# decisiongraph/duckdb-annsearch

Hardware: AMD Instinct MI355X
Metric: queries/sec @ recall@10>=0.95, 10Mx768 fp32, batch=1024 (higher is better)
Workload: dtype f32 results (fp16-image certified filter + exact fp32 rerank); 1 GPU; FAISS IVFFlat nlist=1024 nprobe=32, 10000000x768 fp32 (low-rank gaussian, intrinsic dim 16, noise 0.02), batch=1024, k=10; global_batch=1024, n=10000000, d=768, k=10, parallelism=shard1

## Files before the change

### duckdb-annsearch_amd/csrc/common.hpp

```cpp
#pragma once
#include <hip/hip_runtime.h>
#include <stdint.h>
#include <stdexcept>
#include <string>
#include <cstdio>

namespace hipann {

constexpr int kPlanCopies = 8;
struct IvfPlanHook {
    const int *list_len;
    int nlist, chunk_rows;
    int *ccnt, *slot_off, *qtot;
    bool done;
};

struct HipError : std::runtime_error {
    using std::runtime_error::runtime_error;
};

#define HIPANN_CHECK(expr)                                                                             \
    do {                                                                                               \
        hipError_t _e = (expr);                                                                        \
        if (_e != hipSuccess) {                                                                        \
            throw ::hipann::HipError(std::string(#expr) + " failed: " + hipGetErrorString(_e) + " (" + \
                                     __FILE__ + ":" + std::to_string(__LINE__) + ")");                 \
        }                                                                                              \
    } while (0)

#define HIPANN_REQUIRE(cond, msg)                                        \
    do {                                                                 \
        if (!(cond)) throw ::hipann::HipError(std::string("hipann: ") + (msg)); \
    } while (0)

__host__ __device__ inline int64_t ceil_div(int64_t a, int64_t b) { return (a + b - 1) / b; }

enum Metric : int { kL2 = 0, kIP = 1 };
enum IvfForm : int {
    kFormDecomposed = 0,
    kFormDirect = 1,
    kFormDecomposedValu = 2,
    kFormSplit3 = 3,
    kFormSplit2 = 4,
    kFormSplit2Exact = 5,
    kFormHalfExact = 6,
    kFormI8Exact = 7
};
constexpr int kRerankK = 16, kRerankMaxK = 12;
constexpr int kIvfSubMaxK = 60;
constexpr int kFlatRerankKIP = 32;
enum FlatForm : int {
    kFlatFp32 = 0,
    kFlatSplit3 = 1,
    kFlatSplit2 = 2,
    kFlatSplit2Exact = 3,
    kFlatBf16Exact = 4,
    kFlatI8Exact = 5
};
constexpr float kSplit2Eps = 0x1p-12f;
__host__ __device__ inline bool ivf_form_split(int f) { return f == kFormSplit3 || f == kFormSplit2; }
__host__ __device__ inline int ivf_form_terms(int f) { return f == kFormSplit3 ? 3 : 2; }

__host__ __device__ inline int ivf_group_narrow(int group) { return group & 0xff; }
__host__ __device__ inline int ivf_group_wide(int group) { return (group >> 8) & 0xff; }
__host__ __device__ inline int ivf_ngroups(int c, int group) {
    if (c <= 0) return 0;
    const int n = ivf_group_narrow(group), w = ivf_group_wide(group);
    const int g = w > 0 && c > n ? w : n;
    return (c + g - 1) / g;
}
__host__ __device__ inline int ivf_group_min(int group) {
    return ivf_group_narrow(group) > 0 ? ivf_group_narrow(group) : ivf_group_wide(group);
}

__device__ __forceinline__ int xcd_remap(int bid, int nblocks) {
    const int q = nblocks >> 3, r = nblocks & 7;
    const int xcd = bid & 7, j = bid >> 3;
    return (xcd < r ? xcd * (q + 1) : r * (q + 1) + (xcd - r) * q) + j;
}

}
```

### duckdb-annsearch_amd/csrc/ivf.cpp

```cpp
#include "../../include/hip_ann.h"
#include "ivf.hpp"

#include <algorithm>
#include <chrono>
#include <cstdio>
#include <cstdlib>
#include <cstring>
#include <exception>
#include <numeric>

using namespace hipann;

namespace {

void set_err(char *buf, int len, const char *msg) {
    if (!buf || len <= 0) return;
    std::strncpy(buf, msg, (size_t)len - 1);
    buf[len - 1] = '\0';
}

template <typename F>
int guard_int(char *eb, int el, F &&f) {
    try {
        return f();
// ... 293 lines not shown
    sh.coarse_d.ensure((size_t)nq * np * sizeof(float), sh.device);
    sh.coarse_i.ensure((size_t)nq * np * sizeof(int64_t), sh.device);
    HIPANN_REQUIRE((int64_t)nq * np < (int64_t)0x7fffffff, "nq * nprobe too large");
    sh.slot_off.ensure(sizeof(int) * ((size_t)nq * np + 1), sh.device);
    if (!sh.ccnt.p || !sh.cursor2.p || sh.plan_nlist != nlist) {
        sh.ccnt.ensure(sizeof(int) * 2 * kPlanCopies * (size_t)nlist, sh.device);
        sh.cursor2.ensure(sizeof(int) * 2 * kPlanCopies * (size_t)nlist, sh.device);
        HIPANN_CHECK(hipMemsetAsync(sh.ccnt.p, 0, sizeof(int) * 2 * kPlanCopies * (size_t)nlist, st));
        HIPANN_CHECK(hipMemsetAsync(sh.cursor2.p, 0, sizeof(int) * 2 * kPlanCopies * (size_t)nlist, st));
        sh.plan_nlist = nlist;
        sh.plan_batch = 0;
    }
    const int par = (int)(sh.plan_batch & 1u);
    const size_t pstride = (size_t)kPlanCopies * nlist;
    int *ccnt_cur = sh.ccnt.get<int>() + par * pstride, *ccnt_next = sh.ccnt.get<int>() + (1 - par) * pstride;
    int *cur_cur = sh.cursor2.get<int>() + par * pstride, *cur_next = sh.cursor2.get<int>() + (1 - par) * pstride;
    sh.qtot.ensure(sizeof(int) * (size_t)nq, sh.device);
    struct CcntReset {
        int *p;
        int nlist;
        hipStream_t st;
        bool armed;
        ~CcntReset() {
            if (armed && std::uncaught_exceptions() > 0)
                (void)hipMemsetAsync(p, 0, sizeof(int) * kPlanCopies * (size_t)nlist, st);
        }
    } ccnt_reset{ccnt_cur, nlist, st, true};
    int req = form_override >= 0 ? form_override : ix.form;
    bool as_half = false, probation = false;
    if (form_override < 0 && req == kFormHalfExact && metric == kL2 && kout <= kRerankMaxK && !bigk && !host_fallback() &&
        ivf_mfma_i8_supported(d, kRerankK) && sh.n > 0 && sh.i8_state >= 0) {
        const int mode = filter_image_mode(ix);
        if (mode == 1) {
            as_half = true;
        } else if (mode == 2 && nq >= kAutoI8MinBatch) {
            if (sh.auto8 == 1 && sh.fb_host.p) {
                const uint64_t w = __atomic_load_n(sh.fb_host.get<uint64_t>(), __ATOMIC_RELAXED);
                if (w != sh.fb_seen) {
                    sh.fb_seen = w;
                    sh.auto8_over = auto8_over_rule((int64_t)(w & 0xffffffffu), np, nlist, sh.live, d) ? sh.auto8_over + 1 : 0;
                    if (sh.auto8_over >= 2) sh.auto8 = -1;
                }
            }
            if (sh.auto8 != 0 && sh.live >= sh.auto8_live + sh.auto8_live / 4 + 1) sh.auto8 = 0;
            as_half = sh.auto8 == 1;
            probation = sh.auto8 == 0;
        }
        if (as_half && !ensure_i8_codes(sh, d, nlist, st)) as_half = false;
        if (as_half) req = kFormI8Exact;
    }
    if (form_override < 0) ix.last_filter_image = 0;
    const bool sub_req = (((req == kFormHalfExact || req == kFormSplit2Exact) && kout > kRerankMaxK) ||
                          req == kFormI8Exact) && kout <= kIvfSubMaxK && !bigk;
    bool half = false, i8 = false;
    if (req == kFormHalfExact) {
        half = (kout <= kRerankMaxK || sub_req) && !bigk && ivf_mfma_h_supported(d, kRerankK) &&
               ensure_half_codes(sh, d, nlist, st);
        req = kFormSplit2Exact;
    } else if (req == kFormI8Exact) {
        i8 = sub_req && ivf_mfma_i8_supported(d, kRerankK) && ensure_i8_codes(sh, d, nlist, st);
        req = kFormSplit2Exact;
    }
    const bool img = half || i8;
    const bool want_exact = req == kFormSplit2Exact;
    if (want_exact) req = kout <= kRerankMaxK || sub_req ? kFormSplit2 : kFormSplit3;
    const int k_user = k;
    const int kscan = want_exact && req == kFormSplit2 ? kRerankK : k;
    int form = req != kFormDirect && !bigk && ivf_dot_supported(xq, d, sh.codes) ? req : kFormDirect;
    if (img) form = kFormSplit2;
    if (!img && ivf_form_split(form) && !ivf_mfma_bf_supported(xq, d, sh.codes, kscan, ivf_form_terms(form)))
        form = kFormDecomposed;
    if (form == kFormDecomposed && !ivf_mfma_supported(xq, d, sh.codes, kscan)) form = kFormDecomposedValu;
    const bool exact = want_exact && form == kFormSplit2;
    const bool sub = exact && sub_req;
    k = kscan;
    const int kslot = sub ? ivf_scan_sublists() * k : k;
    const int kfilt = sub ? (i8 ? 64 : std::min(64, std::max(kout + 4, 2 * kout))) : k;
    if (form_override < 0) {
        ix.last_form = exact ? (i8 ? (as_half ? kFormHalfExact : kFormI8Exact) : half ? kFormHalfExact : kFormSplit2Exact) : form;
        ix.last_filter_image = exact && i8 ? 1 : 0;
        ix.last_kfilt = exact ? kfilt : 0;
        ix.last_sublists = sub ? ivf_scan_sublists() : 0;
    }
    const bool tiled = form == kFormDecomposed || ivf_form_split(form);
    const int group = i8 ? ivf_mfma_i8_group(d) : half ? ivf_mfma_h_group(d) : ivf_group_size(form, d);
    float xmax2 = 0.f;
    const bool cert8 = i8 && metric == kL2;
    float rxmax8 = -1.f;
    if (exact) {
        xmax2 = shard_xmax2(sh, d, st);
        if (i8 && !cert8) rxmax8 = shard_i8_rxmax(sh, st);
        sh.nflag.ensure(sizeof(int), sh.device);
        sh.flagged.ensure(sizeof(int) * (size_t)nq, sh.device);
    }
    unsigned *qbound = nullptr;
    if (tiled) {
        sh.qbound.ensure(sizeof(unsigned) * (size_t)nq, sh.device);
        qbound = sh.qbound.get<unsigned>();
    }
    FlatShard &qsh0 = *sh.quant->shards[0];
    if (half) {
        sh.hsplit.ensure((size_t)ivf_half_qsplit_bytes(nq, d), sh.device);
        sh.hits.ensure(sizeof(float) * (size_t)nq, sh.device);
        sh.hres.ensure(sizeof(float) * 2 * (size_t)nq, sh.device);
        float *qn_out = nullptr;
        if (metric == kL2) {
            qsh0.qn.ensure(sizeof(float) * (size_t)nq, sh.device);
            qn_out = qsh0.qn.get<float>();
        }
        RoctxRange rr("hipann.ivf.prepare");
        launch_ivf_split_queries_h(xq, nq, d, sh.half_es, sh.hsplit.p, sh.hits.get<float>(), sh.hres.get<float>(), qn_out,
                                   st);
        qsh0.qn_given = qn_out ? xq : nullptr;
        qsh0.qn_given_nq = nq;
    } else if (i8) {
        sh.qi8.ensure((size_t)ivf_i8_qimg_bytes(nq, d), sh.device);
        sh.qs8.ensure(sizeof(float) * (size_t)nq, sh.device);
        sh.qres8.ensure(sizeof(float) * (size_t)nq, sh.device);
        sh.qhn2.ensure(sizeof(float) * (size_t)nq, sh.device);
        sh.qhn.ensure(sizeof(float) * (size_t)nq, sh.device);
        float *qn_out = nullptr;
        if (metric == kL2) {
            qsh0.qn.ensure(sizeof(float) * (size_t)nq, sh.device);
            qn_out = qsh0.qn.get<float>();
            launch_row_norms(xq, nq, d, qn_out, st);
        }
        RoctxRange rr("hipann.ivf.prepare");
        launch_ivf_split_queries_i8(xq, nq, d, sh.qi8.p, sh.qs8.get<float>(), sh.qres8.get<float>(),
                                    sh.qhn2.get<float>(), sh.qhn.get<float>(), st);
        qsh0.qn_given = qn_out ? xq : nullptr;
        qsh0.qn_given_nq = nq;
    }
    IvfPlanHook hook{sh.list_len.get<int>(), nlist, ivf_chunk_rows(), ccnt_cur, sh.slot_off.get<int>(),
                     sh.qtot.get<int>(), false};
    FlatShard &qsh = *sh.quant->shards[0];
    static const bool hook_env = [] { const char *e = std::getenv("HIPANN_IVF_SELECT_HOOK"); return !e || std::atoi(e); }();
    if (probes_in) {
        HIPANN_CHECK(hipMemcpyAsync(sh.coarse_i.p, probes_in, sizeof(int64_t) * (size_t)nq * np, hipMemcpyDeviceToDevice,
                                    st));
    } else {
        RoctxRange rr("hipann.ivf.coarse");
        qsh.plan_hook = ivf_plan_query_major() && hook_env ? &hook : nullptr;
        CoarseKeysScope ck(qsh);
        try {
            flat_shard_search(*sh.quant, qsh, nq, xq, np, np, sh.coarse_d.get<float>(), sh.coarse_i.get<int64_t>(), st);
        } catch (...) {
            qsh.plan_hook = nullptr;
            qsh.qn_given = nullptr;
            throw;
        }
    }
    qsh.plan_hook = nullptr;
    qsh.qn_given = nullptr;
    sh.cnt.ensure(sizeof(int) * (nlist + 1), sh.device);
    sh.bucket_off.ensure(sizeof(int) * (nlist + 1), sh.device);
    sh.item_off.ensure(sizeof(int) * (nlist + 1), sh.device);
    sh.bucket.ensure(sizeof(int) * (size_t)nq * np, sh.device);
    HIPANN_REQUIRE((int64_t)nq * np < (int64_t)0x7fffffff, "nq * nprobe too large");
    sh.slot_off.ensure(sizeof(int) * ((size_t)nq * np + 1), sh.device);
    {
    RoctxRange rr("hipann.ivf.plan");
    launch_ivf_plan(sh.coarse_i.get<int64_t>(), nq, np, sh.list_len.get<int>(), nlist, group, sh.cnt.get<int>(),
                    sh.bucket_off.get<int>(), sh.item_off.get<int>(), cur_cur, sh.bucket.get<int>(),
                    sh.slot_off.get<int>(), st, exact ? sh.nflag.get<int>() : nullptr, qbound, ccnt_cur,
                    sh.qtot.get<int>(), hook.done, ccnt_next, cur_next);
    }
    sh.plan_batch++;
    ccnt_reset.armed = false;
    const size_t parts = (size_t)np * nq * sh.max_nch * kslot;
    HIPANN_REQUIRE((int64_t)np * nq * sh.max_nch < (int64_t)0x7fffffff, "too many partial lists");
    sh.part_d.ensure(parts * sizeof(float), sh.device);
    sh.part_i.ensure(parts * sizeof(int), sh.device);
    const int64_t max_items = ivf_max_items(nq, np, nlist, sh.max_nch, sh.n, group);
    const float *qn = nullptr;
    if (form != kFormDirect && metric == kL2) {
        const FlatShard &qs = *sh.quant->shards[0];
        if (probes_in && img) {
            qn = qsh0.qn.get<float>();
        } else if (!probes_in && qs.qn_of == xq && qs.qn_nq == nq) {
            qn = qs.qn.get<float>();
        } else {
            sh.qn.ensure(sizeof(float) * (size_t)nq, sh.device);
            launch_row_norms(xq, nq, d, sh.qn.get<float>(), st);
            qn = sh.qn.get<float>();
        }
    }
    if (tiled && !img) ensure_tiled_codes(sh, d, nlist, st);
    if (img) {
    } else if (ivf_form_split(form)) {
        sh.qsplit.ensure((size_t)ivf_mfma_bf_qsplit_bytes(nq, d, ivf_form_terms(form)), sh.device);
    }
    {
        RoctxRange rr("hipann.ivf.scan");
        ScopedTiming t(ix.timer_main, st);
        if (img) {
            launch_ivf_scan_mfma_h(nq, i8 ? sh.qi8.p : sh.hsplit.p, i8 ? sh.qs8.get<float>() : sh.hits.get<float>(),
                                   i8 ? sh.qres8.get<float>() : sh.hres.get<float>(), cert8 ? sh.qhn2.get<float>() : qn, d,
                                   metric, i8 ? sh.codes_i8.p : sh.codes_h.p, sh.tpass_off.get<int64_t>(), sh.xnorm.get<float>(),
                                   sh.list_off.get<int64_t>(), sh.list_len.get<int>(), sh.cnt.get<int>(), sh.bucket_off.get<int>(),
                                   sh.item_off.get<int>(), sh.bucket.get<int>(), sh.slot_off.get<int>(), nlist, np, k,
                                   max_items, qbound, sh.part_d.get<float>(), sh.part_i.get<int>(), st, sub ? 1 : 0,
                                   i8 ? 1 : 0, i8 ? sh.xs8.get<float>() : nullptr,
                                   cert8 ? sh.xr8.get<float>() : nullptr, cert8 ? sh.qhn.get<float>() : nullptr);
        }
        else if (bigk)
            launch_ivf_scan_bigk(xq, d, metric, sh.codes, sh.list_off.get<int64_t>(), sh.list_len.get<int>(),
                                 sh.coarse_i.get<int64_t>(),
                                 nq * np, np, sh.slot_off.get<int>(), nq * np * std::max(sh.max_nch, 1), k,
                                 sh.part_d.get<float>(), sh.part_i.get<int>(), st);
        else if (ivf_form_split(form))
            launch_ivf_scan_mfma_bf(ivf_form_terms(form), xq, nq, sh.qsplit.p, qn, d, metric, sh.codes_t.get<float>(),
                                    sh.tpass_off.get<int64_t>(), sh.xnorm.get<float>(), sh.list_off.get<int64_t>(),
                                    sh.list_len.get<int>(), sh.cnt.get<int>(), sh.bucket_off.get<int>(), sh.item_off.get<int>(),
                                    sh.bucket.get<int>(), sh.slot_off.get<int>(), nlist, np, k, max_items, qbound,
                                    sh.part_d.get<float>(), sh.part_i.get<int>(), st, sub ? 1 : 0);
        else if (form == kFormDecomposed)
            launch_ivf_scan_mfma(xq, qn, d, metric, sh.codes_t.get<float>(), sh.tpass_off.get<int64_t>(),
                                 sh.xnorm.get<float>(), sh.list_off.get<int64_t>(), sh.list_len.get<int>(),
                                 sh.cnt.get<int>(),
                                 sh.bucket_off.get<int>(), sh.item_off.get<int>(), sh.bucket.get<int>(),
                                 sh.slot_off.get<int>(), nlist, np, k, max_items, qbound, sh.part_d.get<float>(),
                                 sh.part_i.get<int>(), st);
        else
            launch_ivf_scan(xq, qn, d, metric, form, sh.codes, sh.xnorm.get<float>(), sh.list_off.get<int64_t>(),
                            sh.list_len.get<int>(), sh.cnt.get<int>(), sh.bucket_off.get<int>(), sh.item_off.get<int>(), sh.bucket.get<int>(),
                            sh.slot_off.get<int>(), nlist, np, nq, k, max_items, qbound, sh.part_d.get<float>(),
                            sh.part_i.get<int>(), st);
    }
    if (!exact) {
        ScopedTiming t(ix.timer_merge, st);
        launch_ivf_merge(sh.part_d.get<float>(), sh.part_i.get<int>(), sh.ids, sh.n, sh.slot_off.get<int>(), np, nq, k,
                         kout, out_sign, D, I, st);
        return;
    }
    const bool inline_fb = !host_fallback() && !sh.count_only;
    int fb_cap = 0, fb_maxch = 1;
    if (inline_fb) {
        if (!sh.fb_total.p) {
            sh.fb_total.ensure(sizeof(unsigned long long), sh.device);
            HIPANN_CHECK(hipMemsetAsync(sh.fb_total.p, 0, sizeof(unsigned long long), st));
        }
        sh.fpd.ensure(sizeof(float) * (size_t)nq * np * kout, sh.device);
        sh.fpi.ensure(sizeof(long long) * (size_t)nq * np * kout, sh.device);
        fb_maxch = sh.max_nch;
        const size_t per_f = (size_t)np * fb_maxch * kout * (sizeof(float) + sizeof(long long));
        fb_cap = (int)std::min<int64_t>({nq, 64, std::max<int64_t>(1, (int64_t)(((size_t)64 << 20) / per_f))});
        sh.fbc_d.ensure(sizeof(float) * (size_t)fb_cap * np * fb_maxch * kout, sh.device);
        sh.fbc_i.ensure(sizeof(long long) * (size_t)fb_cap * np * fb_maxch * kout, sh.device);
        if (sh.fbc_cap < fb_cap || !sh.fbc_done.p) {
            sh.fbc_done.ensure(sizeof(unsigned) * (size_t)std::max(fb_cap, 64), sh.device);
            HIPANN_CHECK(hipMemsetAsync(sh.fbc_done.p, 0, sh.fbc_done.bytes, st));
            sh.fbc_cap = (int)(sh.fbc_done.bytes / sizeof(unsigned));
        }
    }
    {
        RoctxRange rr("hipann.ivf.rerank");
        ScopedTiming t(ix.timer_merge, st);
        launch_ivf_rerank(sh.part_d.get<float>(), sh.part_i.get<int>(), sh.slot_off.get<int>(), np, nq, kfilt, kout,
                          metric, xq, sh.codes, d, sh.ids, sh.n, 0, xmax2, D, I, sh.nflag.get<int>(),
                          sh.flagged.get<int>(), st, kSplit2Eps, i8 ? rxmax8 : half ? sh.half_rxmax : -1.f,
                          i8 ? sh.qres8.get<float>() : half ? sh.hres.get<float>() : nullptr, sh.coarse_i.get<int64_t>(),
                          sh.list_off.get<int64_t>(), nlist, qbound, img && metric == kL2 ? qn : nullptr, kslot,
                          sub ? 1 : 0, inline_fb ? sh.list_len.get<int>() : nullptr,
                          inline_fb ? sh.fpd.get<float>() : nullptr, inline_fb ? sh.fpi.get<long long>() : nullptr,
                          inline_fb ? sh.fb_total.get<unsigned long long>() : nullptr, fb_cap, cert8 ? 1 : 0);
        if (fb_cap > 0)
            launch_ivf_fallback_chunks(sh.nflag.get<int>(), sh.flagged.get<int>(), fb_cap, np, fb_maxch, ivf_chunk_rows(),
                                       kout, metric, xq, sh.codes, d, sh.ids, 0, sh.coarse_i.get<int64_t>(),
                                       sh.list_off.get<int64_t>(), sh.list_len.get<int>(), nlist, sh.fbc_d.get<float>(),
                                       sh.fbc_i.get<long long>(), sh.fbc_done.get<unsigned>(), D, I,
                                       sh.fb_total.get<unsigned long long>(), st,
                                       as_half && !probation ? auto8_host_word(sh) : nullptr, (unsigned)++sh.fb_seq);
    }
    if (sh.count_only) return;
    if (probation) auto8_probation(ix, sh, nq, xq, k_user, kout, st, probes_in);
    if (inline_fb) return;
    int nf = 0;
    HIPANN_CHECK(hipMemcpyAsync(&nf, sh.nflag.p, sizeof(int), hipMemcpyDeviceToHost, st));
    HIPANN_CHECK(hipStreamSynchronize(st));
    if (nf <= 0) return;
    ix.rerank_fallbacks += nf;
    const size_t pbytes = sizeof(int64_t) * (size_t)nq * np;
    sh.coarse_save.ensure(pbytes, sh.device);
    HIPANN_CHECK(hipMemcpyAsync(sh.coarse_save.p, sh.coarse_i.p, pbytes, hipMemcpyDeviceToDevice, st));
    sh.fq.ensure(sizeof(float) * (size_t)nf * d, sh.device);
    sh.fD.ensure(sizeof(float) * (size_t)nf * kout, sh.device);
    sh.fI.ensure(sizeof(int64_t) * (size_t)nf * kout, sh.device);
    launch_ivf_gather_queries(xq, sh.flagged.get<int>(), nf, d, sh.fq.get<float>(), st);
    {
        TimerPause p0(ix.timer_main), p1(ix.timer_merge);
        ivf_shard_search(ix, sh, nf, sh.fq.get<float>(), k_user, kout, sh.fD.get<float>(), sh.fI.get<int64_t>(), st,
                         kFormSplit3);
    }
    launch_ivf_scatter_results(sh.fD.get<float>(), sh.fI.get<int64_t>(), sh.flagged.get<int>(), nf, kout, D, I, st);
    HIPANN_CHECK(hipMemcpyAsync(sh.coarse_i.p, sh.coarse_save.p, pbytes, hipMemcpyDeviceToDevice, st));
}


static void ivf_relayout(IvfIndex &ix, IvfShard &sh, const std::vector<int64_t> &add) {
    const int nlist = ix.nlist, d = ix.d;
    hipStream_t st = sh.stream;
    std::vector<int64_t> off(nlist + 1, 0);
    for (int l = 0; l < nlist; ++l) {
        const int64_t cap = sh.h_off[l + 1] - sh.h_off[l], need = sh.h_len[l] + add[l];
        const int64_t ncap = std::max(cap, need + std::max<int64_t>(need / 4, 64));
        off[l + 1] = off[l] + ncap;
    }
    const int64_t N = off[nlist];
    std::vector<int64_t> tp_old(nlist + 1, 0), tp(nlist + 1, 0);
    for (int l = 0; l < nlist; ++l) {
        tp_old[l + 1] = tp_old[l] + ceil_div(sh.h_off[l + 1] - sh.h_off[l], 32);
        tp[l + 1] = tp[l] + ceil_div(off[l + 1] - off[l], 32);
    }
    auto take = [](DevBuf &dst, DevBuf &src) {
        std::swap(dst.p, src.p);
        std::swap(dst.bytes, src.bytes);
        std::swap(dst.device, src.device);
    };
    auto move_array = [&](DevBuf &cur, const void *src_base, size_t unit, bool pass, size_t count) {
        auto nb = std::make_unique<DevBuf>();
        nb->ensure(unit * std::max<size_t>(count, 1), sh.device);
        HIPANN_CHECK(hipMemsetAsync(nb->p, 0, nb->bytes, st));
        for (int l = 0; l < nlist; ++l) {
            const int64_t len = sh.h_len[l];
            if (!len) continue;
            const int64_t o0 = pass ? tp_old[l] : sh.h_off[l], o1 = pass ? tp[l] : off[l];
            const int64_t cnt = pass ? ceil_div(len, 32) : len;
            HIPANN_CHECK(hipMemcpyAsync(static_cast<char *>(nb->p) + unit * (size_t)o1,
                                        static_cast<const char *>(src_base) + unit * (size_t)o0, unit * (size_t)cnt,
                                        hipMemcpyDeviceToDevice, st));
        }
        HIPANN_CHECK(hipStreamSynchronize(st));
        take(cur, *nb);
    };
    move_array(sh.codes_buf, sh.codes, sizeof(float) * (size_t)d, false, (size_t)N);
    sh.codes = sh.codes_buf.get<float>();
    move_array(sh.ids_buf, sh.ids, sizeof(int64_t), false, (size_t)N);
    sh.ids = sh.ids_buf.get<int64_t>();
    sh.owns_codes = true;
    if (ix.metric == kL2) {
        if (sh.xnorm.p) {
            move_array(sh.xnorm, sh.xnorm.p, sizeof(float), false, (size_t)N);
        } else {
            sh.xnorm.ensure(sizeof(float) * (size_t)std::max<int64_t>(N, 1), sh.device);
            HIPANN_CHECK(hipMemsetAsync(sh.xnorm.p, 0, sh.xnorm.bytes, st));
        }
    }
    const bool img_h = sh.half_state > 0 && sh.codes_h.p, img_t = sh.codes_t.p != nullptr;
// ... 664 lines not shown
}

int hipann_ivf_last_probes(void *h, int64_t *probes, int64_t cap, char *eb, int el) {
    return guard_int(eb, el, [&]() -> int {
        HIPANN_REQUIRE(h && probes, "null argument");
        auto *ix = static_cast<IndexBase *>(h);
        HIPANN_REQUIRE(ix->kind == Kind::IVF, "not an IVFFlat index");
        auto *vx = static_cast<IvfIndex *>(ix);
        std::lock_guard<std::mutex> lk(vx->mu);
        const int64_t m = vx->last_nq * vx->last_np;
        HIPANN_REQUIRE(cap >= m, "probe buffer too small");
        if (m == 0) return 0;
        IvfShard &sh = *vx->shards[0];
        DeviceGuard g(sh.device);
        HIPANN_CHECK(hipStreamSynchronize(sh.stream));
        HIPANN_CHECK(hipDeviceSynchronize());
        HIPANN_CHECK(hipMemcpy(probes, sh.coarse_i.p, sizeof(int64_t) * (size_t)m, hipMemcpyDeviceToHost));
        return 0;
    });
}

int hipann_ivf_set_nprobe(void *h, int nprobe) {
    if (!h || nprobe < 1) return -1;
    auto *ix = static_cast<IndexBase *>(h);
    if (ix->kind != Kind::IVF) return -1;
    auto *vx = static_cast<IvfIndex *>(ix);
    std::lock_guard<std::mutex> lk(vx->mu);
    vx->nprobe = nprobe;
    return 0;
}

int hipann_ivf_set_form(void *h, int form) {
    if (!h || form < kFormDecomposed || form > kFormI8Exact) return -1;
    auto *ix = static_cast<IndexBase *>(h);
    if (ix->kind != Kind::IVF) return -1;
    auto *vx = static_cast<IvfIndex *>(ix);
    std::lock_guard<std::mutex> lk(vx->mu);
    vx->form = form;
    return 0;
}

int64_t hipann_ivf_rerank_fallbacks(void *h) {
    if (!h) return -1;
    auto *ix = static_cast<IndexBase *>(h);
    if (ix->kind != Kind::IVF) return -1;
    auto *vx = static_cast<IvfIndex *>(ix);
    std::lock_guard<std::mutex> lk(vx->mu);
    int64_t t = vx->rerank_fallbacks;
    for (auto &sh : vx->shards) {
        if (!sh->fb_total.p) continue;
        DeviceGuard g(sh->device);
        unsigned long long v = 0;
        if (hipDeviceSynchronize() != hipSuccess) return -1;
        if (hipMemcpy(&v, sh->fb_total.p, sizeof(v), hipMemcpyDeviceToHost) != hipSuccess) return -1;
        t += (int64_t)v;
    }
    return t;
}

int hipann_ivf_set_filter_image(void *h, int mode) {
    if (!h || mode < 0 || mode > 2) return -1;
    auto *ix = static_cast<IndexBase *>(h);
    if (ix->kind != Kind::IVF) return -1;
    auto *vx = static_cast<IvfIndex *>(ix);
    std::lock_guard<std::mutex> lk(vx->mu);
    vx->filter_image = mode;
    return 0;
}

int hipann_ivf_get_filter_image(void *h) {
    if (!h) return -1;
    auto *ix = static_cast<IndexBase *>(h);
    if (ix->kind != Kind::IVF) return -1;
    return static_cast<IvfIndex *>(ix)->filter_image;
}

int hipann_ivf_last_filter_image(void *h) {
    if (!h) return -1;
    auto *ix = static_cast<IndexBase *>(h);
    if (ix->kind != Kind::IVF) return -1;
    return static_cast<IvfIndex *>(ix)->last_filter_image;
}

int64_t hipann_ivf_i8_passes_tiled(void *h) {
    if (!h) return -1;
    auto *ix = static_cast<IndexBase *>(h);
    if (ix->kind != Kind::IVF) return -1;
    auto *vx = static_cast<IvfIndex *>(ix);
    std::lock_guard<std::mutex> lk(vx->mu);
    int64_t t = 0;
    for (auto &sh : vx->shards) t += sh->i8_tiled;
    return t;
}

int hipann_ivf_get_form(void *h) {
    if (!h) return -1;
    auto *ix = static_cast<IndexBase *>(h);
    if (ix->kind != Kind::IVF) return -1;
    return static_cast<IvfIndex *>(ix)->form;
}

}
```

### duckdb-annsearch_amd/csrc/ivf_kernels.hip

```cpp
#include "common.hpp"
#include "wave_topk.hpp"

#include <algorithm>
#include <cstdlib>
#include <utility>

namespace hipann {

constexpr int IVF_WAVES = 8;
constexpr int IVF_THREADS = 64 * IVF_WAVES;
constexpr int IVF_G = 32;
constexpr int IVF_QW = IVF_G / IVF_WAVES;
constexpr int IVF_TR = 256;
constexpr int IVF_BK = 24;
constexpr int IVF_LD = IVF_BK + 4;
#ifndef HIPANN_IVF_CH
#define HIPANN_IVF_CH 2048
#endif
constexpr int IVF_CH = HIPANN_IVF_CH;

__device__ __forceinline__ int ivf_nch(int len) { return (len + IVF_CH - 1) / IVF_CH; }

__global__ void ivf_count(const int64_t *__restrict__ probes, int64_t npairs, const int *__restrict__ list_len,
                          int nlist, int *__restrict__ cnt) {
    const int64_t i = (int64_t)blockIdx.x * blockDim.x + threadIdx.x;
    if (i >= npairs) return;
    const int64_t l = probes[i];
    if (l < 0 || l >= nlist) return;
    if (list_len[l] <= 0) return;
    atomicAdd(cnt + l, 1);
}

__global__ void __launch_bounds__(1024) ivf_plan(const int *__restrict__ cnt, const int *__restrict__ list_len,
                                                 int nlist, int group, int *__restrict__ bucket_off,
                                                 int *__restrict__ item_off, int *__restrict__ cursor) {
    __shared__ int sb[1024], si[1024];
    __shared__ int carry_b, carry_i;
    if (threadIdx.x == 0) { carry_b = 0; carry_i = 0; }
    __syncthreads();
    for (int base = 0; base < nlist; base += 1024) {
        const int l = base + threadIdx.x;
        const int c = l < nlist ? cnt[l] : 0;
        const int items = l < nlist ? ivf_ngroups(c, group) * ivf_nch(list_len[l]) : 0;
        sb[threadIdx.x] = c;
        si[threadIdx.x] = items;
        __syncthreads();
        for (int o = 1; o < 1024; o <<= 1) {
            int vb = 0, vi = 0;
            if ((int)threadIdx.x >= o) { vb = sb[threadIdx.x - o]; vi = si[threadIdx.x - o]; }
            __syncthreads();
            sb[threadIdx.x] += vb;
            si[threadIdx.x] += vi;
            __syncthreads();
        }
        if (l < nlist) {
            bucket_off[l] = carry_b + sb[threadIdx.x] - c;
            item_off[l] = carry_i + si[threadIdx.x] - items;
            cursor[l] = 0;
        }
        __syncthreads();
        if (threadIdx.x == 1023) { carry_b += sb[1023]; carry_i += si[1023]; }
        __syncthreads();
    }
    if (threadIdx.x == 0) { bucket_off[nlist] = carry_b; item_off[nlist] = carry_i; }
}

__global__ void ivf_fill(const int64_t *__restrict__ probes, int64_t npairs, const int *__restrict__ list_len,
                         int nlist, const int *__restrict__ bucket_off, int *__restrict__ cursor,
                         int *__restrict__ bucket) {
    const int64_t i = (int64_t)blockIdx.x * blockDim.x + threadIdx.x;
    if (i >= npairs) return;
    const int64_t l = probes[i];
    if (l < 0 || l >= nlist) return;
    if (list_len[l] <= 0) return;
    const int pos = atomicAdd(cursor + l, 1);
    bucket[bucket_off[l] + pos] = (int)i;
}

__device__ __forceinline__ void slot_scan_block(const int64_t *__restrict__ probes, int64_t npairs,
                                                const int *__restrict__ list_len, int nlist, int *__restrict__ slot_off,
                                                int *wsum) {
    constexpr int J = 16;
    const int lane = threadIdx.x & 63, wave = threadIdx.x >> 6;
    int carry = 0;
    for (int64_t base = 0; base < npairs; base += 16 * 64 * J) {
        const int64_t seg = base + (int64_t)wave * 64 * J;
        int l[J];
#pragma unroll
        for (int j = 0; j < J; ++j) {
            const int64_t i = seg + 64 * j + lane;
            const int64_t pv = i < npairs ? probes[i] : -1;
            l[j] = pv >= 0 && pv < nlist ? (int)pv : -1;
        }
        int v[J];
#pragma unroll
        for (int j = 0; j < J; ++j) v[j] = l[j] >= 0 ? ivf_nch(list_len[l[j]]) : 0;
        int run = 0;
#pragma unroll
        for (int j = 0; j < J; ++j) {
            int x = v[j];
#pragma unroll
            for (int o = 1; o < 64; o <<= 1) {
                const int t = __shfl_up(x, o);
                if (lane >= o) x += t;
            }
            const int tot = __shfl(x, 63);
            v[j] = run + x - v[j];
            run += tot;
        }
        if (lane == 0) wsum[wave] = run;
        __syncthreads();
        int off = carry, total = 0;
        for (int w2 = 0; w2 < 16; ++w2) {
            const int t = wsum[w2];
            off += w2 < wave ? t : 0;
            total += t;
        }
#pragma unroll
        for (int j = 0; j < J; ++j) {
            const int64_t i = seg + 64 * j + lane;
            if (i < npairs) slot_off[i] = off + v[j];
        }
        carry += total;
        __syncthreads();
    }
    if (threadIdx.x == 0) slot_off[npairs] = carry;
}

__global__ void __launch_bounds__(1024) ivf_slot_scan(const int64_t *__restrict__ probes, int64_t npairs,
                                                      const int *__restrict__ list_len, int nlist,
                                                      int *__restrict__ slot_off) {
    __shared__ int wsum[16];
    slot_scan_block(probes, npairs, list_len, nlist, slot_off, wsum);
}

__global__ void __launch_bounds__(256) ivf_count_q(const int64_t *__restrict__ probes, int64_t nq, int nprobe,
                                                   const int *__restrict__ list_len, int nlist, int *__restrict__ ccnt,
                                                   int *__restrict__ slot_off, int *__restrict__ qtot) {
    const int64_t q = (int64_t)blockIdx.x * 4 + (threadIdx.x >> 6);
    if (q >= nq) return;
    const int lane = threadIdx.x & 63;
    int carry = 0;
    for (int p0 = 0; p0 < nprobe; p0 += 64) {
        const int p = p0 + lane;
        const int64_t i = q * nprobe + p;
        const int64_t l = p < nprobe ? probes[i] : -1;
        const bool ok = l >= 0 && l < nlist;
        const int len = ok ? list_len[l] : 0;
        if (len > 0) atomicAdd(ccnt + (int64_t)(q % kPlanCopies) * nlist + l, 1);
        const int v = len > 0 ? ivf_nch(len) : 0;
        int x = v;
#pragma unroll
        for (int o = 1; o < 64; o <<= 1) {
            const int t = __shfl_up(x, o);
            if (lane >= o) x += t;
        }
        if (p < nprobe) slot_off[i] = carry + x - v;
        carry += __shfl(x, 63);
    }
    if (lane == 0) qtot[q] = carry;
}

__global__ void __launch_bounds__(1024) ivf_plan_q(int *__restrict__ ccnt, const int *__restrict__ list_len, int nlist,
                                                   int group, int *__restrict__ cnt, int *__restrict__ bucket_off,
                                                   int *__restrict__ item_off, int *__restrict__ cursor,
                                                   int *__restrict__ qtot, int64_t nq, int64_t npairs,
                                                   int *__restrict__ slot_off, int *__restrict__ nflag_reset,
                                                   unsigned *__restrict__ qbound) {
    __shared__ int sb[1024], si[1024];
    __shared__ int carry_b, carry_i;
    const int tid = threadIdx.x;
    if (tid == 0) { carry_b = 0; carry_i = 0; }
    if (nflag_reset && tid == 0) *nflag_reset = 0;
    if (qbound)
        for (int64_t q = tid; q < nq; q += 1024) qbound[q] = 0xff800000u;
    __syncthreads();
    for (int base = 0; base < nlist; base += 1024) {
        const int l = base + tid;
        int c = 0;
        if (l < nlist)
            for (int cp = 0; cp < kPlanCopies; ++cp) c += ccnt[(int64_t)cp * nlist + l];
        const int items = l < nlist ? ivf_ngroups(c, group) * ivf_nch(list_len[l]) : 0;
        sb[tid] = c;
        si[tid] = items;
        __syncthreads();
        for (int o = 1; o < 1024; o <<= 1) {
            int vb = 0, vi = 0;
            if (tid >= o) { vb = sb[tid - o]; vi = si[tid - o]; }
            __syncthreads();
            sb[tid] += vb;
            si[tid] += vi;
            __syncthreads();
        }
        if (l < nlist) {
            cnt[l] = c;
            bucket_off[l] = carry_b + sb[tid] - c;
            item_off[l] = carry_i + si[tid] - items;
            int pre = 0;
            for (int cp = 0; cp < kPlanCopies; ++cp) {
                const int64_t e = (int64_t)cp * nlist + l;
                const int n = ccnt[e];
                cursor[e] = pre;
                ccnt[e] = 0;
                pre += n;
            }
        }
        __syncthreads();
        if (tid == 1023) { carry_b += sb[1023]; carry_i += si[1023]; }
        __syncthreads();
    }
    if (tid == 0) { bucket_off[nlist] = carry_b; item_off[nlist] = carry_i; }
    __syncthreads();
    if (tid == 0) carry_b = 0;
    __syncthreads();
    for (int64_t base = 0; base < nq; base += 1024) {
        const int64_t q = base + tid;
        const int t = q < nq ? qtot[q] : 0;
        sb[tid] = t;
        __syncthreads();
        for (int o = 1; o < 1024; o <<= 1) {
            int v = 0;
            if (tid >= o) v = sb[tid - o];
            __syncthreads();
            sb[tid] += v;
            __syncthreads();
        }
        if (q < nq) qtot[q] = carry_b + sb[tid] - t;
        __syncthreads();
        if (tid == 1023) carry_b += sb[1023];
        __syncthreads();
    }
    if (tid == 0) slot_off[npairs] = carry_b;
}

__global__ void __launch_bounds__(256) ivf_fill_q(const int64_t *__restrict__ probes, int64_t nq, int nprobe,
                                                  const int *__restrict__ list_len, int nlist,
                                                  const int *__restrict__ qbase, const int *__restrict__ bucket_off,
                                                  int *__restrict__ cursor, int *__restrict__ bucket,
                                                  int *__restrict__ slot_off) {
    const int64_t q = (int64_t)blockIdx.x * 4 + (threadIdx.x >> 6);
    if (q >= nq) return;
    const int lane = threadIdx.x & 63;
    const int b = qbase[q];
    for (int p = lane; p < nprobe; p += 64) {
        const int64_t i = q * nprobe + p;
        slot_off[i] += b;
        const int64_t l = probes[i];
        if (l < 0 || l >= nlist || list_len[l] <= 0) continue;
        const int pos = atomicAdd(cursor + (int64_t)(q % kPlanCopies) * nlist + l, 1);
        bucket[bucket_off[l] + pos] = (int)i;
    }
}

constexpr int kPlanFillMaxList = 8192;
__device__ __forceinline__ int block_excl_scan256(int v, int *s_w) {
    const int lane = threadIdx.x & 63, wave = threadIdx.x >> 6;
    int x = v;
#pragma unroll
    for (int o = 1; o < 64; o <<= 1) {
        const int t = __shfl_up(x, o);
        if (lane >= o) x += t;
    }
    if (lane == 63) s_w[wave] = x;
    __syncthreads();
    int base = 0;
#pragma unroll
    for (int w = 0; w < 4; ++w) base += w < wave ? s_w[w] : 0;
    __syncthreads();
    return base + x - v;
}
__global__ void __launch_bounds__(256) ivf_planfill_q(const int64_t *__restrict__ probes, int64_t nq, int nprobe,
                                                      const int *__restrict__ list_len, int nlist, int group,
                                                      const int *__restrict__ ccnt, int *__restrict__ ccnt_next,
                                                      int *__restrict__ cursor, int *__restrict__ cursor_next,
                                                      const int *__restrict__ qtot, int *__restrict__ slot_off,
                                                      int64_t npairs, int *__restrict__ cnt, int *__restrict__ bucket_off,
                                                      int *__restrict__ item_off, int *__restrict__ bucket,
                                                      int *__restrict__ nflag_reset, unsigned *__restrict__ qbound) {
    __shared__ int s_boff[kPlanFillMaxList];
    __shared__ int s_w[4], s_qb[4];
    const int tid = threadIdx.x, lane = tid & 63, wave = tid >> 6;
    const int64_t q0 = (int64_t)blockIdx.x * 4;
    const int per = (nlist + 255) / 256;
    int sum = 0, isum = 0;
    for (int j = 0; j < per; ++j) {
        const int l = tid * per + j;
        if (l < nlist) {
            int c = 0;
            for (int cp = 0; cp < kPlanCopies; ++cp) c += ccnt[(int64_t)cp * nlist + l];
            sum += c;
            if (blockIdx.x == 0) isum += ivf_ngroups(c, group) * ivf_nch(list_len[l]);
        }
    }
    int b = block_excl_scan256(sum, s_w);
    int ib = blockIdx.x == 0 ? block_excl_scan256(isum, s_w) : 0;
    for (int j = 0; j < per; ++j) {
        const int l = tid * per + j;
        if (l < nlist) {
            int c = 0;
            for (int cp = 0; cp < kPlanCopies; ++cp) c += ccnt[(int64_t)cp * nlist + l];
            s_boff[l] = b;
            if (blockIdx.x == 0) {
                cnt[l] = c;
                bucket_off[l] = b;
                item_off[l] = ib;
                ib += ivf_ngroups(c, group) * ivf_nch(list_len[l]);
            }
            b += c;
        }
    }
    if (blockIdx.x == 0 && tid == 255) {
        bucket_off[nlist] = b;
        item_off[nlist] = ib;
    }
    for (int64_t l = (int64_t)blockIdx.x * 256 + tid; l < (int64_t)kPlanCopies * nlist; l += (int64_t)gridDim.x * 256) {
        ccnt_next[l] = 0;
        cursor_next[l] = 0;
    }
    int qs = 0;
    for (int64_t q = tid; q < q0; q += 256) qs += qtot[q];
    const int qb0 = block_excl_scan256(qs, s_w) + qs;
    if (tid == 255) s_qb[0] = qb0;
    __syncthreads();
    if (tid == 0) {
        int acc = s_qb[0];
        for (int i = 0; i < 4; ++i) {
            s_qb[i] = acc;
            acc += q0 + i < nq ? qtot[q0 + i] : 0;
        }
        if (q0 + 4 >= nq) slot_off[npairs] = acc;
        if (blockIdx.x == 0 && nflag_reset) *nflag_reset = 0;
    }
    __syncthreads();
    const int64_t q = q0 + wave;
    if (q >= nq) return;
    if (qbound && lane == 0) qbound[q] = 0xff800000u;
    const int base = s_qb[wave];
    for (int p = lane; p < nprobe; p += 64) {
        const int64_t i = q * nprobe + p;
        slot_off[i] += base;
        const int64_t l = probes[i];
        if (l < 0 || l >= nlist || list_len[l] <= 0) continue;
        const int cp = (int)(q % kPlanCopies);
        int pre = 0;
        for (int c2 = 0; c2 < cp; ++c2) pre += ccnt[(int64_t)c2 * nlist + l];
        const int pos = atomicAdd(cursor + (int64_t)cp * nlist + l, 1);
        bucket[s_boff[l] + pre + pos] = (int)i;
    }
}

constexpr int IVF_F4 = IVF_BK / 4;
constexpr int IVF_SP = IVF_TR * IVF_F4 / IVF_THREADS;

template <bool VEC4>
__device__ __forceinline__ float4 ivf_ld4(const float *__restrict__ src, int kk, int d) {
    float4 v = make_float4(0.f, 0.f, 0.f, 0.f);
    if (VEC4) {
        if (kk < d) v = *reinterpret_cast<const float4 *>(src);
    } else {
        if (kk + 0 < d) v.x = src[0];
        if (kk + 1 < d) v.y = src[1];
        if (kk + 2 < d) v.z = src[2];
        if (kk + 3 < d) v.w = src[3];
    }
    return v;
}

template <bool VEC4>
__device__ __forceinline__ void ivf_stage_load(const float *__restrict__ codes, int64_t r0, int64_t rlast, int d,
                                               int k0, float4 (&st)[IVF_SP]) {
#pragma unroll
    for (int p = 0; p < IVF_SP; ++p) {
        const int f = threadIdx.x + IVF_THREADS * p;
        const int row = f / IVF_F4, c4 = f - (f / IVF_F4) * IVF_F4;
        const int64_t gr = r0 + row < rlast ? r0 + row : rlast;
        const int kk = k0 + 4 * c4;
        st[p] = ivf_ld4<VEC4>(codes + gr * (int64_t)d + kk, kk, d);
    }
}

__device__ __forceinline__ void ivf_stage_store(float *__restrict__ lds, const float4 (&st)[IVF_SP]) {
#pragma unroll
    for (int p = 0; p < IVF_SP; ++p) {
        const int f = threadIdx.x + IVF_THREADS * p;
        const int row = f / IVF_F4, c4 = f - (f / IVF_F4) * IVF_F4;
        *reinterpret_cast<float4 *>(lds + row * IVF_LD + 4 * c4) = st[p];
    }
}

typedef float ivf_f2 __attribute__((ext_vector_type(2)));
typedef float ivf_f4 __attribute__((ext_vector_type(4)));

__device__ __forceinline__ ivf_f2 ivf_pk_sub(ivf_f2 a, ivf_f2 b) {
    ivf_f2 r;
    asm("v_pk_add_f32 %0, %1, %2 neg_lo:[0,1] neg_hi:[0,1]" : "=v"(r) : "v"(a), "v"(b));
    return r;
// ... 522 lines not shown
    float *sk = sm;
    int *si = reinterpret_cast<int *>(sm + IVF_CH);
    float *qv = sm + 2 * IVF_CH;
    const int slot = blockIdx.x;
    if (slot >= slot_off[npairs]) return;
    int64_t lo = 0, hi = npairs - 1;
    while (lo < hi) {
        const int64_t mid = (lo + hi + 1) >> 1;
        if (slot_off[mid] <= slot) lo = mid; else hi = mid - 1;
    }
    const int64_t pair = lo;
    const int chunk = slot - slot_off[pair];
    const int64_t l = probes[pair];
    const int64_t lend = list_off[l] + list_len[l];
    const int64_t r0 = list_off[l] + (int64_t)chunk * IVF_CH;
    const int64_t r1 = r0 + IVF_CH < lend ? r0 + IVF_CH : lend;
    const int len = (int)(r1 - r0);
    const float *q = Q + (pair / nprobe) * (int64_t)d;
    for (int j = threadIdx.x; j < d; j += 256) qv[j] = q[j];
    __syncthreads();
    const int lane = threadIdx.x & 63, wave = threadIdx.x >> 6;
    for (int r = wave; r < IVF_CH; r += 4) {
        float acc = 0.f;
        if (r < len) {
            const float *x = codes + (r0 + r) * (int64_t)d;
            for (int j = lane; j < d; j += 64) {
                if (IP) acc = fmaf(qv[j], x[j], acc);
                else { const float t = qv[j] - x[j]; acc = fmaf(t, t, acc); }
            }
#pragma unroll
            for (int o = 32; o > 0; o >>= 1) acc += __shfl_xor(acc, o);
        }
        if (lane == 0) {
            sk[r] = r < len ? (IP ? -acc : acc) : __builtin_inff();
            si[r] = r < len ? (int)(r0 + r) : 0x7fffffff;
        }
    }
    __syncthreads();
    for (int size = 2; size <= IVF_CH; size <<= 1) {
        for (int stride = size >> 1; stride > 0; stride >>= 1) {
            for (int t = threadIdx.x; t < IVF_CH / 2; t += 256) {
                const int a = 2 * t - (t & (stride - 1)), b = a + stride;
                const bool up = (a & size) == 0;
                const float ka = sk[a], kb = sk[b];
                const int ia = si[a], ib = si[b];
                const bool b_less = kb < ka || (kb == ka && ib < ia);
                if (b_less == up) { sk[a] = kb; sk[b] = ka; si[a] = ib; si[b] = ia; }
            }
            __syncthreads();
        }
    }
    const int64_t off = (int64_t)slot * k;
    for (int e = threadIdx.x; e < k; e += 256) {
        part_d[off + e] = e < IVF_CH ? sk[e] : __builtin_inff();
        part_i[off + e] = e < IVF_CH ? si[e] : 0x7fffffff;
    }
}

void launch_ivf_scan_bigk(const float *Q, int d, int metric, const float *codes, const int64_t *list_off,
                          const int *list_len, const int64_t *probes, int64_t npairs, int nprobe, const int *slot_off, int64_t nslots,
                          int k, float *pd, int *pi, hipStream_t st) {
    if (nslots <= 0) return;
    HIPANN_REQUIRE(nslots < (int64_t)0x7fffffff, "too many slots");
    const size_t smem = (size_t)2 * IVF_CH * 4 + (size_t)d * 4;
    HIPANN_REQUIRE(smem <= 64 * 1024, "dimension too large for the k > 64 IVF path");
    dim3 grid((unsigned)nslots), block(256);
    if (metric == kIP)
        hipLaunchKernelGGL(ivf_scan_slot_bigk<true>, grid, block, smem, st, Q, d, codes, list_off, list_len, probes, npairs,
                           nprobe, slot_off, k, pd, pi);
    else
        hipLaunchKernelGGL(ivf_scan_slot_bigk<false>, grid, block, smem, st, Q, d, codes, list_off, list_len, probes, npairs,
                           nprobe, slot_off, k, pd, pi);
    HIPANN_CHECK(hipGetLastError());
}

bool ivf_plan_query_major() {
    static const bool split = [] { const char *e = std::getenv("HIPANN_IVF_PLAN_SPLIT"); return e && std::atoi(e); }();
    return !split;
}

void launch_ivf_plan(const int64_t *probes, int64_t nq, int nprobe, const int *list_len, int nlist, int group,
                     int *cnt, int *bucket_off, int *item_off, int *cursor, int *bucket, int *slot_off,
                     hipStream_t st, int *nflag_reset, unsigned *qbound, int *ccnt, int *qtot, bool counted,
                     int *ccnt_next, int *cursor_next) {
    const int64_t npairs = nq * nprobe;
    if (ivf_plan_query_major() && ccnt && qtot) {
        const unsigned gq = (unsigned)std::max<int64_t>(1, ceil_div(nq, (int64_t)4));
        if (nq > 0 && !counted)
            hipLaunchKernelGGL(ivf_count_q, dim3(gq), dim3(256), 0, st, probes, nq, nprobe, list_len, nlist, ccnt,
                               slot_off, qtot);
        static const bool fused_env = [] { const char *e = std::getenv("HIPANN_IVF_PLANFILL"); return !e || std::atoi(e); }();
        if (fused_env && ccnt_next && cursor_next && nlist <= kPlanFillMaxList && nq > 0) {
            hipLaunchKernelGGL(ivf_planfill_q, dim3(gq), dim3(256), 0, st, probes, nq, nprobe, list_len, nlist, group,
                               ccnt, ccnt_next, cursor, cursor_next, qtot, slot_off, npairs, cnt, bucket_off, item_off,
                               bucket, nflag_reset, qbound);
            HIPANN_CHECK(hipGetLastError());
            return;
        }
        hipLaunchKernelGGL(ivf_plan_q, dim3(1), dim3(1024), 0, st, ccnt, list_len, nlist, group, cnt, bucket_off,
                           item_off, cursor, qtot, nq, npairs, slot_off, nflag_reset, qbound);
        if (nq > 0)
            hipLaunchKernelGGL(ivf_fill_q, dim3(gq), dim3(256), 0, st, probes, nq, nprobe, list_len, nlist, qtot,
                               bucket_off, cursor, bucket, slot_off);
        if (cursor_next)
            HIPANN_CHECK(hipMemsetAsync(cursor_next, 0, sizeof(int) * kPlanCopies * (size_t)nlist, st));
        HIPANN_CHECK(hipGetLastError());
        return;
    }
    if (nflag_reset) HIPANN_CHECK(hipMemsetAsync(nflag_reset, 0, sizeof(int), st));
    if (qbound) HIPANN_CHECK(hipMemsetD32Async((hipDeviceptr_t)qbound, 0xff800000, (size_t)nq, st));
    HIPANN_CHECK(hipMemsetAsync(cnt, 0, sizeof(int) * (size_t)nlist, st));
    if (npairs > 0)
        hipLaunchKernelGGL(ivf_count, dim3((unsigned)ceil_div(npairs, 256)), dim3(256), 0, st, probes, npairs, list_len,
                           nlist, cnt);
    hipLaunchKernelGGL(ivf_plan, dim3(1), dim3(1024), 0, st, cnt, list_len, nlist, group, bucket_off, item_off,
                       cursor);
    hipLaunchKernelGGL(ivf_slot_scan, dim3(1), dim3(1024), 0, st, probes, npairs, list_len, nlist, slot_off);
    if (npairs > 0)
        hipLaunchKernelGGL(ivf_fill, dim3((unsigned)ceil_div(npairs, 256)), dim3(256), 0, st, probes, npairs, list_len,
                           nlist, bucket_off, cursor, bucket);
    HIPANN_CHECK(hipGetLastError());
}

int64_t ivf_max_items(int64_t nq, int nprobe, int nlist, int max_nch, int64_t nrows, int group) {
    const int64_t npairs = nq * nprobe;
    return ceil_div(npairs, (int64_t)ivf_group_min(group)) * std::max(max_nch, 1) + ceil_div(nrows, IVF_CH) + nlist;
}

int ivf_mfma_group(int d);
int ivf_mfma_bf_group(int d, int np);

int ivf_group_size(int form, int d) {
    if (ivf_form_split(form)) return ivf_mfma_bf_group(d, ivf_form_terms(form));
    return form == kFormDecomposed ? ivf_mfma_group(d) : form == kFormDecomposedValu ? DT_G : IVF_G;
}

int ivf_chunk_rows() { return IVF_CH; }

size_t ivf_scan_smem_bytes() { return (size_t)2 * (IVF_TR + IVF_G) * IVF_LD * sizeof(float); }
static size_t ivf_scan_dot_smem_bytes() { return (size_t)DT_STAGES * DT_STAGE_F4 * 16; }

bool ivf_dot_supported(const float *Q, int d, const float *codes) {
    return (d % 4 == 0) && ((uintptr_t)Q % 16 == 0) && ((uintptr_t)codes % 16 == 0);
}

void launch_ivf_scan(const float *Q, const float *qn, int d, int metric, int form, const float *codes,
                     const float *xn, const int64_t *list_off, const int *list_len, const int *cnt,
                     const int *bucket_off, const int *item_off, const int *bucket, const int *slot_off, int nlist,
                     int nprobe, int64_t nq,
                     int k, int64_t max_items, unsigned *qbound, float *pd, int *pi, hipStream_t st) {
    if (max_items <= 0) return;
    HIPANN_REQUIRE(max_items < (int64_t)0x7fffffff, "too many IVF work items");
    HIPANN_REQUIRE(form != kFormDecomposed, "the MFMA scan is launched with its tiled codes (launch_ivf_scan_mfma)");
    if (form == kFormDecomposedValu) {
        HIPANN_REQUIRE(ivf_dot_supported(Q, d, codes), "decomposed IVF scan needs d % 4 == 0 and 16-B aligned data");
        HIPANN_REQUIRE(metric == kIP || (qn && xn), "decomposed L2 scan needs query and row norms");
        dim3 grid((unsigned)max_items), block(DT_THREADS);
        const size_t smem = ivf_scan_dot_smem_bytes();
#define HIPANN_DOT_ARGS Q, qn, d, codes, xn, list_off, list_len, cnt, bucket_off, item_off, bucket, slot_off, nlist, nprobe, k, pd, pi
        if (metric == kIP) hipLaunchKernelGGL((ivf_scan_dot<true>), grid, block, smem, st, HIPANN_DOT_ARGS);
        else hipLaunchKernelGGL((ivf_scan_dot<false>), grid, block, smem, st, HIPANN_DOT_ARGS);
#undef HIPANN_DOT_ARGS
    } else {
        const bool vec4 = ivf_dot_supported(Q, d, codes);
        dim3 grid((unsigned)max_items), block(IVF_THREADS);
        const size_t smem = ivf_scan_smem_bytes();
#define HIPANN_IVF_ARGS Q, d, codes, list_off, list_len, cnt, bucket_off, item_off, bucket, slot_off, nlist, nprobe, nq, k, pd, pi
        if (vec4) {
            if (metric == kIP) hipLaunchKernelGGL((ivf_scan_topk<true, true>), grid, block, smem, st, HIPANN_IVF_ARGS);
            else hipLaunchKernelGGL((ivf_scan_topk<true, false>), grid, block, smem, st, HIPANN_IVF_ARGS);
        } else {
            if (metric == kIP) hipLaunchKernelGGL((ivf_scan_topk<false, true>), grid, block, smem, st, HIPANN_IVF_ARGS);
            else hipLaunchKernelGGL((ivf_scan_topk<false, false>), grid, block, smem, st, HIPANN_IVF_ARGS);
        }
#undef HIPANN_IVF_ARGS
    }
    HIPANN_CHECK(hipGetLastError());
}

void launch_ivf_merge(const float *pd, const int *pi, const int64_t *ids, int64_t nrows, const int *slot_off, int nprobe, int64_t nq,
                      int k, int kout, float out_sign, float *D, int64_t *I, hipStream_t st) {
    if (nq <= 0) return;
    dim3 grid((unsigned)ceil_div(nq, 4)), block(256);
    const int S = (kout + 63) / 64;
#define HIPANN_IVF_MERGE(s)                                                                                           \
    if (S <= s) {                                                                                                     \
        hipLaunchKernelGGL(ivf_merge_topk<s>, grid, block, 0, st, pd, pi, ids, nrows, slot_off, nprobe, nq, k, kout, \
                           out_sign, D, I);                                                                           \
        HIPANN_CHECK(hipGetLastError());                                                                              \
        return;                                                                                                       \
    }
    HIPANN_IVF_MERGE(1) HIPANN_IVF_MERGE(2) HIPANN_IVF_MERGE(4) HIPANN_IVF_MERGE(8) HIPANN_IVF_MERGE(16)
    HIPANN_IVF_MERGE(32)
#undef HIPANN_IVF_MERGE
    throw HipError("ivf merge: k too large");
}

}

// ... 204 lines not shown
    }
    unsigned T = 0;
    for (int bit = 31; bit >= 0; --bit) {
        const unsigned cand = T | (1u << bit);
        int cnt = 0;
#pragma unroll
        for (int j = 0; j < J; ++j)
            if (j < nj) cnt += __popcll(__ballot(u[j] < cand));
        if (cnt < k) T = cand;
    }
    (void)n_lt_out;
    return T;
}
__device__ __forceinline__ unsigned rws_bits(float f) {
    f = f == 0.f ? 0.f : f;
    const unsigned b = __float_as_uint(f);
    return (b >> 31) ? ~b : (b | 0x80000000u);
}
template <int J>
__device__ __forceinline__ int rws_take(const float *__restrict__ mk, const int *__restrict__ mp, int m, int k, unsigned T,
                                        float *__restrict__ ok, int *__restrict__ op) {
    const int lane = threadIdx.x & 63;
    const unsigned long long lt = (1ull << lane) - 1ull;
    const int nj = (m + 63) >> 6;
    int base = 0;
#pragma unroll
    for (int j = 0; j < J; ++j) {
        const int e = j * 64 + lane;
        const bool a = j < nj && e < m && rws_bits(mk[e]) < T;
        const unsigned long long ma = __ballot(a);
        if (a) { const int p = base + __popcll(ma & lt); ok[p] = mk[e]; op[p] = mp[e]; }
        base += __popcll(ma);
    }
#pragma unroll
    for (int j = 0; j < J; ++j) {
        const int e = j * 64 + lane;
        const bool b = j < nj && e < m && rws_bits(mk[e]) == T;
        const unsigned long long mb = __ballot(b);
        if (b) { const int p = base + __popcll(mb & lt); if (p < k) { ok[p] = mk[e]; op[p] = mp[e]; } }
        base += __popcll(mb);
    }
    return base < k ? base : k;
}
template <int J>
__device__ __forceinline__ int rws_select_narrow(const float *mk, const int *mp, int m, int k, float *tk, int *tp,
                                                 float *ok, int *op) {
    const int lane = threadIdx.x & 63;
    const unsigned long long lt = (1ull << lane) - 1ull;
    const int nj = (m + 63) >> 6;
    unsigned u[J];
    unsigned mn = 0xffffffffu;
#pragma unroll
    for (int j = 0; j < J; ++j) {
        const int e = j * 64 + lane;
        u[j] = j < nj && e < m ? rws_bits(mk[e]) : 0xffffffffu;
        mn = min(mn, u[j]);
    }
    unsigned th = 0;
    for (int bit = 31; bit >= 0; --bit) {
        const unsigned cand = th | (1u << bit);
        if ((int)__popcll(__ballot(mn < cand)) < k) th = cand;
    }
    int c = 0;
#pragma unroll
    for (int j = 0; j < J; ++j) {
        const bool a = u[j] <= th && u[j] != 0xffffffffu;
        const unsigned long long ma = __ballot(a);
        const int p = c + (int)__popcll(ma & lt);
        if (a && p < 64) { tk[p] = mk[j * 64 + lane]; tp[p] = mp[j * 64 + lane]; }
        c += (int)__popcll(ma);
    }
    if (c > 64) return -1;
    __builtin_amdgcn_fence(__ATOMIC_SEQ_CST, "wavefront");
    unsigned dummy = 0;
    const unsigned T = rws_kth_bits<1>(tk, c, k, dummy);
    return rws_take<1>(tk, tp, c, k, T, ok, op);
}

template <int WV, int J>
__device__ __forceinline__ void rerank_wave_select(const float *__restrict__ pd, const int *__restrict__ pi,
                                                   int64_t total, int k, int64_t nrows, float bound,
                                                   float *wk, int *wp, float *sk, int *sp, int *scnt,
                                                   WaveList<1, int> &L, bool &bad, long long &rr_t, int64_t rr_q,
                                                   float *ntk, int *ntp) {
    (void)rr_t;
    (void)rr_q;
    const int lane = threadIdx.x & 63, wv = threadIdx.x >> 6;
    const unsigned long long lt = (1ull << lane) - 1ull;
    float v[J];
    int r[J];
#pragma unroll
    for (int j = 0; j < J; ++j) {
        const int64_t c = ((int64_t)j * WV + wv) * 64 + lane;
        v[j] = c < total ? pd[c] : __builtin_inff();
        r[j] = c < total ? pi[c] : -1;
    }
    RR_MARK(1);
    float *mk = wk + wv * 64 * J;
    int *mp = wp + wv * 64 * J;
    int m = 0;
#pragma unroll
    for (int j = 0; j < J; ++j) {
        const bool a = v[j] <= bound && !(v[j] == __builtin_inff()) && r[j] >= 0 && r[j] < nrows;
        const unsigned long long ma = __ballot(a);
        if (a) { const int p = m + __popcll(ma & lt); mk[p] = v[j]; mp[p] = r[j]; }
        m += __popcll(ma);
    }
    __builtin_amdgcn_fence(__ATOMIC_SEQ_CST, "wavefront");
    if constexpr (HIPANN_RR_STAMP != 0) { if (m >= 0) RR_STAMP_Q(rr_q, 6); }
    int kw;
    if (m <= k) {
        kw = m;
        for (int e = lane; e < m; e += 64) { sk[wv * 64 + e] = mk[e]; sp[wv * 64 + e] = mp[e]; }
    } else if (m <= 64) {
        unsigned dummy = 0;
        const unsigned T = rws_kth_bits<1>(mk, m, k, dummy);
        kw = rws_take<1>(mk, mp, m, k, T, sk + wv * 64, sp + wv * 64);
    } else {
        kw = ntk ? rws_select_narrow<J>(mk, mp, m, k, ntk + wv * 64, ntp + wv * 64, sk + wv * 64, sp + wv * 64) : -1;
        if (kw < 0) {
            unsigned dummy = 0;
            const unsigned T = rws_kth_bits<J>(mk, m, k, dummy);
            kw = rws_take<J>(mk, mp, m, k, T, sk + wv * 64, sp + wv * 64);
        }
    }
    if (lane == 0) scnt[wv] = kw;
    RR_MARK(5);
    RR_STAMP_Q(rr_q, 7);
    __syncthreads();
    if (wv != 0) return;
    int m0 = 0;
#pragma unroll
    for (int w = 0; w < WV; ++w) {
        const int n = scnt[w];
        const bool a = lane < n;
        float kk = a ? sk[w * 64 + lane] : 0.f;
        int pp = a ? sp[w * 64 + lane] : 0;
        if (a) { mk[m0 + lane] = kk; mp[m0 + lane] = pp; }
        m0 += n;
    }
    __builtin_amdgcn_fence(__ATOMIC_SEQ_CST, "wavefront");
    int nsel = m0;
    if (m0 > k && m0 <= 64) {
        unsigned dummy = 0;
        const unsigned T = rws_kth_bits<1>(mk, m0, k, dummy);
        nsel = rws_take<1>(mk, mp, m0, k, T, sk, sp);
        __builtin_amdgcn_fence(__ATOMIC_SEQ_CST, "wavefront");
    } else if (m0 > k) {
        unsigned dummy = 0;
        const unsigned T = rws_kth_bits<WV>(mk, m0, k, dummy);
        nsel = rws_take<WV>(mk, mp, m0, k, T, sk, sp);
        __builtin_amdgcn_fence(__ATOMIC_SEQ_CST, "wavefront");
    } else {
        for (int e = lane; e < m0; e += 64) { sk[e] = mk[e]; sp[e] = mp[e]; }
        __builtin_amdgcn_fence(__ATOMIC_SEQ_CST, "wavefront");
    }
    float kk = lane < nsel ? sk[lane] : __builtin_inff();
    int row = lane < nsel ? sp[lane] : IdTraits<int>::pad();
    wave_rank_sort(kk, row, nsel);
    bad = false;
    L.d[0] = lane < k ? kk : __builtin_inff();
    L.id[0] = lane < k ? row : IdTraits<int>::pad();
    RR_MARK(2);
}

struct ScanCand {
    float key;
    long long pos, label;
};

template <typename Gen>
__device__ __forceinline__ void ivf_scan_order_topk(int64_t n, int kout, Gen gen, WaveList<1, long long> &R) {
    const int lane = threadIdx.x & 63;
    const long long PAD = IdTraits<long long>::pad();
    WaveList<1, long long> A;
    A.init();
    for (int64_t c0 = 0; c0 < n; c0 += 64) {
        const ScanCand x = c0 + lane < n ? gen(c0 + lane) : ScanCand{__builtin_inff(), PAD, PAD};
// ... 201 lines not shown
        asm volatile("s_waitcnt vmcnt(0)" ::: "memory");
        unsigned old = 0;
        if (lane == 0) old = __hip_atomic_fetch_add(done + f, 1u, __ATOMIC_RELAXED, __HIP_MEMORY_SCOPE_AGENT);
        old = (unsigned)__shfl((int)old, 0);
        int64_t need = 0;
        for (int pp = lane; pp < nprobe; pp += 64) {
            int64_t ll, ln;
            plist(q, pp, ll, ln);
            need += (ln + chunk_rows - 1) / chunk_rows;
        }
#pragma unroll
        for (int o = 32; o > 0; o >>= 1) need += __shfl_xor(need, o);
        if ((int64_t)old + 1 != need) continue;
        __builtin_amdgcn_fence(__ATOMIC_ACQUIRE, "agent");
        asm volatile("s_waitcnt vmcnt(0)" ::: "memory");
        const float *pd = cpd + (int64_t)f * per_q * kout;
        const long long *pr = cpi + (int64_t)f * per_q * kout;
        int64_t lenv = 0;
        if (lane < nprobe) {
            int64_t ll;
            plist(q, lane, ll, lenv);
        }
        WaveList<1, long long> R;
        ivf_scan_order_topk(per_q * kout, kout, [&](int64_t cc) {
            const int64_t slot = cc / kout;
            const int pp = (int)(slot / maxch);
            int64_t ll, ln;
            if (nprobe <= 64) ln = __shfl(lenv, pp);
            else plist(q, pp, ll, ln);
            const bool live = (slot % maxch) * (int64_t)chunk_rows < ln;
            const float key = live ? pd[cc] : __builtin_inff();
            const long long row = live ? pr[cc] : PAD;
            const bool ok = !(key == __builtin_inff()) && row != PAD;
            return ScanCand{ok ? key : __builtin_inff(), ok ? ((long long)pp << 32) | row : PAD,
                            ok ? (long long)(ids ? ids[row] : label_offset + row) : PAD};
        }, R);
        const float pad_d = IP ? -__builtin_inff() : __builtin_inff();
        if (lane < kout) {
            const bool pad = R.id[0] == PAD || R.d[0] == __builtin_inff();
            D[q * kout + lane] = pad ? pad_d : (IP ? -R.d[0] : R.d[0]);
            I[q * kout + lane] = pad ? -1 : (int64_t)R.id[0];
        }
        if (lane == 0) {
            __hip_atomic_store(done + f, 0u, __ATOMIC_RELAXED, __HIP_MEMORY_SCOPE_AGENT);
            atomicAdd(total, 1ull);
        }
    }
}

void launch_ivf_fallback_chunks(const int *nflag, const int *flagged, int fb_cap, int nprobe, int maxch, int chunk_rows,
                                int kout, int metric, const float *Q, const float *codes, int d, const int64_t *ids,
                                int64_t label_offset, const int64_t *probes, const int64_t *list_off,
                                const int *list_len, int nlist, float *cpd, long long *cpi, unsigned *done, float *D,
                                int64_t *I, unsigned long long *total, hipStream_t st, unsigned long long *host_word,
                                unsigned host_seq) {
    if (fb_cap <= 0) return;
    HIPANN_REQUIRE(kout >= 1 && kout <= 64 && maxch >= 1 && chunk_rows >= 64, "ivf fallback: arguments out of range");
    dim3 grid(256), block(256);
    if (metric == kIP)
        hipLaunchKernelGGL(ivf_fallback_chunks<true>, grid, block, 0, st, nflag, flagged, fb_cap, nprobe, maxch,
                           chunk_rows, kout, Q, codes, d, ids, label_offset, probes, list_off, list_len, nlist, cpd, cpi,
                           done, D, I, total, host_word, host_seq);
    else
        hipLaunchKernelGGL(ivf_fallback_chunks<false>, grid, block, 0, st, nflag, flagged, fb_cap, nprobe, maxch,
                           chunk_rows, kout, Q, codes, d, ids, label_offset, probes, list_off, list_len, nlist, cpd, cpi,
                           done, D, I, total, host_word, host_seq);
    HIPANN_CHECK(hipGetLastError());
}

#ifndef HIPANN_RR_MINB
#define HIPANN_RR_MINB 4
#endif
template <bool IP, int WV>
__global__ void __launch_bounds__(WV == 1 ? 256 : 64 * WV, WV == 4 ? HIPANN_RR_MINB : 1)
ivf_rerank_topk(const float *__restrict__ pd, const int *__restrict__ pi, const int *__restrict__ slot_off,
                int nprobe, int64_t nq, int k, int kout, const float *__restrict__ Q,
                const float *__restrict__ codes, int d, const int64_t *__restrict__ ids, int64_t nrows,
                int64_t label_offset, float xmax2, float *__restrict__ D, int64_t *__restrict__ I,
                int *__restrict__ nflag, int *__restrict__ flagged, float eps, float rxmax,
                const float *__restrict__ qres, const int64_t *__restrict__ probes,
                const int64_t *__restrict__ list_off, int nlist, const unsigned *__restrict__ qbound,
                const float *__restrict__ qnorm, int kslot, int sub, const int *__restrict__ list_len,
                float *__restrict__ fpd, long long *__restrict__ fpi, unsigned long long *__restrict__ fb_total,
                int fb_cap, int i8_l2) {
    const int64_t q = WV == 1 ? (int64_t)blockIdx.x * 4 + (threadIdx.x >> 6) : (int64_t)blockIdx.x;
    if (q >= nq) return;
    const int lane = threadIdx.x & 63;
    const int wv = WV == 1 ? 0 : (int)(threadIdx.x >> 6);
    RR_STAMP(0);
    long long rr_t = HIPANN_RR_PROF ? clock64() : 0;
    WaveList<1, int> L;
    L.init();
    const int64_t s0 = slot_off ? slot_off[q * nprobe] : q * nprobe;
    const int64_t s1 = slot_off ? slot_off[(q + 1) * nprobe] : (q + 1) * nprobe;
    const int64_t total = (s1 - s0) * kslot;
    if constexpr (HIPANN_RR_STAMP != 0) { if (total >= 0) RR_STAMP(1); }
    pd += s0 * kslot;
    pi += s0 * kslot;
    float tsub = __builtin_inff();
    if (sub && qbound) {
        const unsigned b = qbound[q];
        const float t = __uint_as_float((b & 0x80000000u) ? (b & 0x7fffffffu) : ~b);
        tsub = t == t ? t : __builtin_inff();
    }
    constexpr int RS_J = 16;
    const bool bsel = WV > 1 && total <= (int64_t)64 * WV * RS_J && !rerank_lists();
    if (WV > 1 && !bsel) RR_COUNT(9);
    constexpr int MU = 4;
    for (int64_t cb = (int64_t)wv * 64; !bsel && cb < total; cb += 64 * WV * MU) {
        float vv[MU];
        int rr[MU];
#pragma unroll
        for (int u = 0; u < MU; ++u) {
            const int64_t c = cb + (int64_t)u * 64 * WV + lane;
            vv[u] = c < total ? pd[c] : __builtin_inff();
            rr[u] = c < total ? pi[c] : -1;
        }
#pragma unroll
        for (int u = 0; u < MU; ++u) {
            const bool ok = rr[u] >= 0 && rr[u] < nrows && !(vv[u] == __builtin_inff()) && vv[u] < tsub;
            L.offer(ok ? vv[u] : __builtin_inff(), ok ? rr[u] : IdTraits<int>::pad(), k - 1);
        }
    }
    const float *qp = Q + q * (int64_t)d;
    float mine = __builtin_inff();
    int myrow, ncand;
    float k16;
    bool sel_bad = false;
    const float qn_pre = qres && qnorm ? qnorm[q] : 0.f;
    const float qres_pre = qres ? qres[q] : 0.f;
    if constexpr (WV > 1) {
        __shared__ float sd[WV * 64], sdist[64];
        __shared__ int si[WV * 64], srow[64];
        __shared__ int scnt[2][WV];
        if (bsel) {
            float bound = __builtin_inff();
            if (sub) {
                bound = tsub;
            } else if (qbound) {
                const unsigned qb = qbound[q];
                const float t = __uint_as_float((qb & 0x80000000u) ? (qb & 0x7fffffffu) : ~qb);
                bound = t == t ? t : __builtin_inff();
            }
            RR_MARK(0);
#if HIPANN_RR_OLDSEL
            rerank_block_select<WV, RS_J>(pd, pi, total, k, nrows, sd, si, scnt, L, bound, rr_t);
#else
            __shared__ float wk[WV * 64 * RS_J];
            __shared__ int wp[WV * 64 * RS_J];
            __shared__ float ntk[WV * 64];
            __shared__ int ntp[WV * 64];
            rerank_wave_select<WV, RS_J>(pd, pi, total, k, nrows, bound, wk, wp, sd, si, scnt[0], L, sel_bad, rr_t, q,
                                         ntk, ntp);
#endif
            if (wv == 0) srow[lane] = lane < k ? L.id[0] : IdTraits<int>::pad();
            RR_STAMP(2);
        } else {
            sd[wv * 64 + lane] = lane < k ? L.d[0] : __builtin_inff();
            si[wv * 64 + lane] = lane < k ? L.id[0] : IdTraits<int>::pad();
            __syncthreads();
            if (wv == 0) {
                L.init();
#pragma unroll
                for (int w = 0; w < WV; ++w) L.offer(sd[w * 64 + lane], si[w * 64 + lane], k - 1);
                srow[lane] = lane < k ? L.id[0] : IdTraits<int>::pad();
            }
        }
        __syncthreads();
        for (int r0 = wv * 4; r0 < k; r0 += 4 * WV) {
            float acc[4] = {0.f, 0.f, 0.f, 0.f};
            const float *xr[4];
            bool ok[4];
#pragma unroll
            for (int u = 0; u < 4; ++u) {
                const int r = r0 + u < k ? r0 + u : k - 1;
                const int row = srow[r];
                ok[u] = r0 + u < k && row != IdTraits<int>::pad();
                xr[u] = codes + (int64_t)(ok[u] ? row : 0) * d;
            }
            rerank_rows4<IP>(qp, xr, d, lane, acc);
#pragma unroll
// ... 221 lines not shown
        const float r = qp[e] - (float)(__bf16)qp[e];
        rq2 = fmaf(r, r, rq2);
    }
#pragma unroll
    for (int o = 32; o > 0; o >>= 1) {
        qq += __shfl_xor(qq, o);
        rq2 += __shfl_xor(rq2, o);
    }
    const float qn = sqrtf(qq), rq = qres ? qres[q] : sqrtf(rq2), xh = sqrtf(xmax2) + rxmax;
    const float g = (float)(qres ? 2 * d : d) * 0x1p-24f;
    const float eip = qn * rxmax + rq * xh + g * (qn + rq) * xh;
    const float T = bound[q];
    const float E = 1.01f * ((IP ? 1.f : 2.f) * eip + (float)(d + 8) * 0x1p-24f * 2.f * (qq + xmax2)) +
                    0x1p-20f * (qq + xmax2 + fabsf(T));
    const float dk = readlane_f(L.d[0], kout - 1);
    const bool ok = !over && E <= 3.4e38f && dk < __builtin_inff() && (T == __builtin_inff() || dk < T - E);
    if (dbg && lane == 0) {
        dbg[4 * f + 0] = over ? 1.f : 0.f;
        dbg[4 * f + 1] = dk;
        dbg[4 * f + 2] = T;
        dbg[4 * f + 3] = E;
    }
    if (!ok) {
        if (lane == 0) flagged2[atomicAdd(nflag2, 1)] = (int)q;
        return;
    }
    if (lane < kout) {
        D[q * kout + lane] = IP ? -L.d[0] : L.d[0];
        I[q * kout + lane] = (int64_t)L.id[0];
    }
}

void launch_flat_cand_rerank(const int *flagged, int nf, const float *cand_d, const int *cand_i, const int *cand_n,
                             int nsplit, int cap, const float *bound, const float *Q, const float *X, int d,
                             int64_t nrows, int64_t label_offset, float xmax2, float rxmax, int metric, int kout,
                             float *part_d, long long *part_i, int *ovf, float *D, int64_t *I, int *nflag2,
                             int *flagged2, hipStream_t st, float *dbg, const float *qres) {
    if (nf <= 0) return;
    HIPANN_REQUIRE(kout >= 1 && kout <= 64 && nsplit >= 1 && cap >= 1, "flat cand rerank: bad arguments");
    const int P = std::min(kCandRerankParts, nsplit);
    dim3 g1((unsigned)nf, (unsigned)P);
    if (metric == kIP) {
        hipLaunchKernelGGL(flat_cand_rerank_part<true>, g1, dim3(256), 0, st, flagged, cand_d, cand_i, cand_n, nsplit,
                           cap, Q, X, d, nrows, label_offset, kout, part_d, part_i, ovf);
        hipLaunchKernelGGL(flat_cand_rerank_final<true>, dim3((unsigned)nf), dim3(64), 0, st, flagged, P, bound, Q, d,
                           xmax2, rxmax, kout, part_d, part_i, ovf, D, I, nflag2, flagged2, dbg, qres);
    } else {
        hipLaunchKernelGGL(flat_cand_rerank_part<false>, g1, dim3(256), 0, st, flagged, cand_d, cand_i, cand_n, nsplit,
                           cap, Q, X, d, nrows, label_offset, kout, part_d, part_i, ovf);
        hipLaunchKernelGGL(flat_cand_rerank_final<false>, dim3((unsigned)nf), dim3(64), 0, st, flagged, P, bound, Q, d,
                           xmax2, rxmax, kout, part_d, part_i, ovf, D, I, nflag2, flagged2, dbg, qres);
    }
    HIPANN_CHECK(hipGetLastError());
}

int flat_cand_rerank_parts(int nsplit) { return std::min(kCandRerankParts, nsplit); }

__global__ void __launch_bounds__(256) ivf_max_norm(const float *__restrict__ xn, int64_t n, unsigned *__restrict__ out) {
    float m = 0.f;
    for (int64_t i = (int64_t)blockIdx.x * 256 + threadIdx.x; i < n; i += (int64_t)gridDim.x * 256) m = fmaxf(m, xn[i]);
#pragma unroll
    for (int o = 32; o > 0; o >>= 1) m = fmaxf(m, __shfl_xor(m, o));
    if ((threadIdx.x & 63) == 0) atomicMax(out, __float_as_uint(m));
}

__global__ void __launch_bounds__(256) ivf_gather_queries(const float *__restrict__ Q, const int *__restrict__ idx, int nf,
                                                          int d, float *__restrict__ out) {
    const int64_t t = (int64_t)blockIdx.x * 256 + threadIdx.x;
    if (t >= (int64_t)nf * d) return;
    const int j = (int)(t / d), e = (int)(t - (int64_t)j * d);
    out[t] = Q[(int64_t)idx[j] * d + e];
}

__global__ void __launch_bounds__(256) ivf_scatter_results(const float *__restrict__ Df, const int64_t *__restrict__ If,
                                                           const int *__restrict__ idx, int nf, int kout,
                                                           float *__restrict__ D, int64_t *__restrict__ I) {
    const int64_t t = (int64_t)blockIdx.x * 256 + threadIdx.x;
    if (t >= (int64_t)nf * kout) return;
    const int j = (int)(t / kout), e = (int)(t - (int64_t)j * kout);
    D[(int64_t)idx[j] * kout + e] = Df[t];
    I[(int64_t)idx[j] * kout + e] = If[t];
}

#ifndef HIPANN_RR_WIDE
#define HIPANN_RR_WIDE (1 << 30)
#endif

void launch_ivf_rerank(const float *pd, const int *pi, const int *slot_off, int nprobe, int64_t nq, int k, int kout,
                       int metric, const float *Q, const float *codes, int d, const int64_t *ids, int64_t nrows,
                       int64_t label_offset, float xmax2, float *D, int64_t *I, int *nflag, int *flagged,
                       hipStream_t st, float eps, float rxmax, const float *qres, const int64_t *probes,
                       const int64_t *list_off, int nlist, const unsigned *qbound, const float *qnorm, int kslot,
                       int sub, const int *list_len, float *fpd, long long *fpi, unsigned long long *fb_total,
                       int fb_cap, int i8_l2) {
    if (nq <= 0) return;
    if (kslot <= 0) kslot = k;
    HIPANN_REQUIRE(!i8_l2 || (metric == kL2 && qres && qnorm), "ivf rerank: the int8 L2 certificate needs ‖q − q̂‖ and ‖q‖²");
    HIPANN_REQUIRE(k >= kRerankK && k <= 64 && kout >= 1 && kout <= k && kslot >= 1 && (!sub || qbound),
                   "ivf rerank: k / kout out of range");
    HIPANN_REQUIRE(!fpd || (fpi && list_len && probes && list_off && fb_total), "ivf rerank: inline re-run buffers");
    const bool wide = nq < HIPANN_RR_WIDE;
    dim3 grid((unsigned)(wide ? nq : ceil_div(nq, 4))), block(256);
#define RR_ARGS pd, pi, slot_off, nprobe, nq, k, kout, Q, codes, d, ids, nrows, label_offset, xmax2, D, I, nflag, flagged, \
                eps, rxmax, qres, probes, list_off, nlist, qbound, qnorm, kslot, sub, list_len, fpd, fpi, fb_total, \
                fpd ? fb_cap : 0, i8_l2
    if (metric == kIP) {
        if (wide) hipLaunchKernelGGL((ivf_rerank_topk<true, 4>), grid, block, 0, st, RR_ARGS);
        else hipLaunchKernelGGL((ivf_rerank_topk<true, 1>), grid, block, 0, st, RR_ARGS);
    } else {
        if (wide) hipLaunchKernelGGL((ivf_rerank_topk<false, 4>), grid, block, 0, st, RR_ARGS);
        else hipLaunchKernelGGL((ivf_rerank_topk<false, 1>), grid, block, 0, st, RR_ARGS);
    }
#undef RR_ARGS
    HIPANN_CHECK(hipGetLastError());
}

extern "C" int hipann_debug_rr_stamps(long long *out, int n) {
#if HIPANN_RR_STAMP
    if (n > 4096 * 8 || hipDeviceSynchronize() != hipSuccess) return -1;
    return hipMemcpyFromSymbol(out, HIP_SYMBOL(rr_stamp), sizeof(long long) * (size_t)n) == hipSuccess ? 0 : -1;
#else
    (void)out;
    (void)n;
    return -1;
#endif
}

extern "C" int hipann_debug_rr_prof(unsigned long long *out16) {
#if HIPANN_RR_PROF
    if (hipDeviceSynchronize() != hipSuccess) return -1;
    if (hipMemcpyFromSymbol(out16, HIP_SYMBOL(rr_prof), sizeof(unsigned long long) * 16) != hipSuccess) return -1;
    unsigned long long z[16] = {0};
    if (hipMemcpyToSymbol(HIP_SYMBOL(rr_prof), z, sizeof z) != hipSuccess) return -1;
    return 0;
#else
    (void)out16;
    return -1;
#endif
}

void launch_ivf_max_norm(const float *xn, int64_t n, unsigned *out, hipStream_t st) {
    HIPANN_CHECK(hipMemsetAsync(out, 0, sizeof(unsigned), st));
    if (n <= 0) return;
    const unsigned blocks = (unsigned)std::min<int64_t>(1024, ceil_div(n, 256));
    hipLaunchKernelGGL(ivf_max_norm, dim3(blocks), dim3(256), 0, st, xn, n, out);
    HIPANN_CHECK(hipGetLastError());
}

void launch_ivf_gather_queries(const float *Q, const int *idx, int nf, int d, float *out, hipStream_t st) {
    if (nf <= 0) return;
    hipLaunchKernelGGL(ivf_gather_queries, dim3((unsigned)ceil_div((int64_t)nf * d, 256)), dim3(256), 0, st, Q, idx, nf,
                       d, out);
    HIPANN_CHECK(hipGetLastError());
}

void launch_ivf_scatter_results(const float *Df, const int64_t *If, const int *idx, int nf, int kout, float *D,
                                int64_t *I, hipStream_t st) {
    if (nf <= 0) return;
    hipLaunchKernelGGL(ivf_scatter_results, dim3((unsigned)ceil_div((int64_t)nf * kout, 256)), dim3(256), 0, st, Df, If,
                       idx, nf, kout, D, I);
    HIPANN_CHECK(hipGetLastError());
}

}
```

### duckdb-annsearch_amd/csrc/ivf_mfma.hip

```cpp
#include "common.hpp"
#include "wave_topk.hpp"

#include <algorithm>
#include <cstdio>
#include <cstdlib>
#include <cstring>

namespace hipann {

typedef float mf_f32x4 __attribute__((ext_vector_type(4)));

#ifndef HIPANN_MF_EXPERIMENT
#define HIPANN_MF_EXPERIMENT 0
#endif

#ifndef HIPANN_MF_WAVES
#define HIPANN_MF_WAVES 8
#endif
#ifndef HIPANN_MF_P
#define HIPANN_MF_P 6
#endif
#ifndef HIPANN_MF_QPF
#define HIPANN_MF_QPF 0
#endif
// ... 66 lines not shown
    row_cx<15>(p, m & 8);
    row_cx<4>(p, m & 4);
    row_cx<2>(p, m & 2);
    row_cx<1>(p, m & 1);
}
__device__ __forceinline__ void row_merge16(uint64_t &l, uint64_t c, int m) {
    const uint64_t r = row_xor<15>(c);
    l = r < l ? r : l;
    row_cx<8>(l, m & 8);
    row_cx<4>(l, m & 4);
    row_cx<2>(l, m & 2);
    row_cx<1>(l, m & 1);
}
__device__ __forceinline__ void row_insert1(uint64_t &l, uint64_t c) {
    c &= row_xor<1>(c);
    c &= row_xor<2>(c);
    c &= row_xor<7>(c);
    c &= row_xor<15>(c);
    const unsigned plo = (unsigned)__builtin_amdgcn_update_dpp(0, (int)(unsigned)l, 0x111, 0xF, 0xF, true);
    const unsigned phi = (unsigned)__builtin_amdgcn_update_dpp(0, (int)(unsigned)(l >> 32), 0x111, 0xF, 0xF, true);
    const uint64_t prev = ((uint64_t)phi << 32) | plo;
    l = l <= c ? l : (prev <= c ? c : prev);
}
__device__ __forceinline__ uint64_t row_kth(uint64_t l, int kth, int g) {
    const unsigned lo = (unsigned)l, hi = (unsigned)(l >> 32);
    unsigned rl[4], rh[4];
#pragma unroll
    for (int r = 0; r < 4; ++r) {
        rl[r] = (unsigned)__builtin_amdgcn_readlane((int)lo, 16 * r + kth);
        rh[r] = (unsigned)__builtin_amdgcn_readlane((int)hi, 16 * r + kth);
    }
    const unsigned sl = g == 0 ? rl[0] : g == 1 ? rl[1] : g == 2 ? rl[2] : rl[3];
    const unsigned sh = g == 0 ? rh[0] : g == 1 ? rh[1] : g == 2 ? rh[2] : rh[3];
    return ((uint64_t)sh << 32) | sl;
}

__device__ __forceinline__ unsigned row_kth_key(uint64_t l, int kth, int g) {
    const unsigned hi = (unsigned)(l >> 32);
    unsigned rh[4];
#pragma unroll
    for (int r = 0; r < 4; ++r) rh[r] = (unsigned)__builtin_amdgcn_readlane((int)hi, 16 * r + kth);
    return g == 0 ? rh[0] : g == 1 ? rh[1] : g == 2 ? rh[2] : rh[3];
}

template <int QT>
__device__ __forceinline__ void mf_finish_item(uint64_t (&lst)[QT][4], float *smem, int nqi,
                                               const int *__restrict__ bucket, int boff, int nprobe,
                                               const int *__restrict__ slot_off, int chunk, int k, int sub,
                                               unsigned *__restrict__ qbound, float *__restrict__ part_d,
                                               int *__restrict__ part_i) {
    const int lane = threadIdx.x & 63;
    const int wave = __builtin_amdgcn_readfirstlane(threadIdx.x >> 6);
    const int m = lane & 15, g = lane >> 4;
    if (!sub) {
        uint64_t *scratch = reinterpret_cast<uint64_t *>(smem);
#pragma unroll 1
        for (int half = MF_WAVES / 2; half > 0; half >>= 1) {
            __syncthreads();
            if (wave >= half && wave < 2 * half) {
                uint64_t *dst = scratch + (size_t)(wave - half) * QT * 4 * 64;
#pragma unroll
                for (int qt = 0; qt < QT; ++qt)
#pragma unroll
                    for (int v = 0; v < 4; ++v) dst[(qt * 4 + v) * 64 + lane] = lst[qt][v];
            }
            __syncthreads();
            if (wave < half) {
                const uint64_t *src = scratch + (size_t)wave * QT * 4 * 64;
#pragma unroll
                for (int qt = 0; qt < QT; ++qt)
#pragma unroll
                    for (int v = 0; v < 4; ++v) row_merge16(lst[qt][v], src[(qt * 4 + v) * 64 + lane], m);
            }
        }
    }
    if ((sub || wave == 0) && m < k) {
#pragma unroll
        for (int qt = 0; qt < QT; ++qt)
#pragma unroll
            for (int v = 0; v < 4; ++v) {
                const int q = qt * 16 + 4 * g + v;
                if (q < nqi) {
                    const int pr = bucket[boff + q];
                    const int64_t slot = (int64_t)slot_off[pr] + chunk;
                    const int64_t off = (sub ? slot * MF_WAVES + wave : slot) * k + m;
                    const uint64_t e = lst[qt][v];
                    const unsigned id = (unsigned)e;
                    const bool real = e != MF_EMPTY && id != MF_PAD_ID;
                    part_d[off] = real ? mf_unsortable((unsigned)(e >> 32)) : __builtin_inff();
                    part_i[off] = real ? (int)id : (int)MF_PAD_ID;
                    if (m == k - 1 && real) atomicMin(qbound + pr / nprobe, (unsigned)(e >> 32));
                }
            }
    }
}

template <int QT, bool IP>
__device__ __forceinline__ void mf_item(int d, const float *__restrict__ codes_t, int64_t tp0,
                                        const float *__restrict__ xn,
                                        int64_t r0, int64_t r1, int nqi, const float *__restrict__ qs, int stride,
                                        const float (&qn)[QT][4], const unsigned (&qb)[QT][4],
                                        const int *__restrict__ bucket, int boff, int nprobe,
                                        const int *__restrict__ slot_off, int chunk, int k, int sub, float *smem,
                                        unsigned *__restrict__ qbound, float *__restrict__ part_d,
                                        int *__restrict__ part_i) {
    const int lane = threadIdx.x & 63;
    const int wave = __builtin_amdgcn_readfirstlane(threadIdx.x >> 6);
    const int m = lane & 15, g = lane >> 4;
    const int nsub = mf_nsub(d);
    const int npass_all = (int)ceil_div(r1 - r0, MF_PASS);
    const int npass = npass_all > wave ? (npass_all - wave + MF_WAVES - 1) / MF_WAVES : 0;


    bool qv[QT][4];
#pragma unroll
    for (int qt = 0; qt < QT; ++qt)
#pragma unroll
        for (int v = 0; v < 4; ++v) qv[qt][v] = qt * 16 + 4 * g + v < nqi;

    uint64_t lst[QT][4], thr[QT][4];
#pragma unroll
    for (int qt = 0; qt < QT; ++qt)
#pragma unroll
        for (int v = 0; v < 4; ++v) {
            const uint64_t b = ((uint64_t)qb[qt][v] << 32) | MF_PAD_ID;
            lst[qt][v] = m < k ? b : MF_EMPTY;
            thr[qt][v] = b;
        }

    auto row_of = [&](int i, int r) -> int64_t {
        const int64_t row = r0 + (int64_t)(wave + MF_WAVES * i) * MF_PASS + 16 * r + m;
        return row < r1 ? row : r1 - 1;
    };
    const int ilast = npass > 0 ? npass - 1 : 0;
    const float *rp;
    int ld_i = 0, ld_s = 0;
    auto set_pass = [&](int i) {
        rp = codes_t + ((tp0 + wave + MF_WAVES * i) * nsub) * (MF_RT * 256) + 4 * lane;
    };
    auto next_load = [&](mf_f32x4 (&dst)[MF_RT]) {
        const int s = ld_i <= ilast ? ld_s : nsub - 1;
#pragma unroll
        for (int r = 0; r < MF_RT; ++r)
            dst[r] = *reinterpret_cast<const mf_f32x4 *>(rp + (int64_t)s * (MF_RT * 256) + r * 256);
        if (++ld_s == nsub) {
            ld_s = 0;
            ++ld_i;
            set_pass(ld_i <= ilast ? ld_i : ilast);
        }
    };

    mf_f32x4 ring[MF_P][MF_RT];
    float xnr[MF_RT] = {0.f, 0.f};
    if (npass > 0) {
        set_pass(0);
#pragma unroll
        for (int p = 0; p < MF_P; ++p) next_load(ring[p]);
        if (!IP) {
#pragma unroll
            for (int r = 0; r < MF_RT; ++r) xnr[r] = xn[row_of(0, r)];
        }
    }

    mf_f32x4 acc[QT][MF_RT];
    uint64_t sink = 0;
    mf_f32x4 qnext[QT];
    if (MF_QPF) {
// ... 489 lines not shown
        MB_QN(3)
        mb_item<3, IP, NP, NH>(MB_ARGS);
    }
#undef MB_QN
#undef MB_ARGS
}

template <int NP>
__global__ void __launch_bounds__(256) ivf_split_queries(const float *__restrict__ Q, int64_t nq, int d, int nsup,
                                                         uint4 *__restrict__ out) {
    const int64_t t = (int64_t)blockIdx.x * 256 + threadIdx.x;
    if (t >= nq * nsup * 4) return;
    const int64_t q = t / (nsup * 4);
    const int rr = (int)(t - q * (nsup * 4));
    const int S = rr >> 2, gg = rr & 3;
    const float *src = Q + q * d;
    const int d0 = 32 * S + 4 * gg, d1 = d0 + 16;
    mf_f32x4 a = mf_f32x4{0.f, 0.f, 0.f, 0.f}, b = a;
    if (d0 < d) a = *reinterpret_cast<const mf_f32x4 *>(src + d0);
    if (d1 < d) b = *reinterpret_cast<const mf_f32x4 *>(src + d1);
    const MbTerms<NP> sp = mb_split<NP>(a, b);
#pragma unroll
    for (int j = 0; j < NP; ++j) out[((q * NP + j) * nsup + S) * 4 + gg] = sp.t[j];
}

int ivf_mfma_bf_group(int d, int np) { return mb_group(d, np); }

int64_t ivf_mfma_bf_qsplit_bytes(int64_t nq, int d, int np) { return nq * np * mb_nsuper(d) * 64; }

bool ivf_mfma_bf_supported(const float *Q, int d, const float *codes, int k, int np) {
    return ivf_mfma_supported(Q, d, codes, k) && mb_group(d, np) >= 16;
}

void launch_ivf_scan_mfma_bf(int np, const float *Q, int64_t nq, void *qsplit, const float *qn, int d, int metric,
                             const float *codes_t, const int64_t *tpass_off, const float *xn, const int64_t *list_off,
                             const int *list_len, const int *cnt, const int *bucket_off, const int *item_off, const int *bucket,
                             const int *slot_off, int nlist, int nprobe, int k, int64_t max_items, unsigned *qbound,
                             float *pd, int *pi, hipStream_t st, int sub) {
    if (max_items <= 0 || nq <= 0) return;
    HIPANN_REQUIRE(np == 2 || np == 3, "split-bf16 scan: 2 or 3 terms");
    HIPANN_REQUIRE(max_items < (int64_t)0x7fffffff, "too many IVF work items");
    HIPANN_REQUIRE(qsplit, "split-bf16 scan: no query image buffer");
    HIPANN_REQUIRE(ivf_mfma_bf_supported(Q, d, codes_t, k, np), "split-bf16 IVF scan needs d % 4 == 0, 16-B aligned data, k <= 16");
    HIPANN_REQUIRE(metric == kIP || (qn && xn), "decomposed L2 scan needs query and row norms");
    const int nsup = mb_nsuper(d);
    const int64_t nthr = nq * nsup * 4;
    uint4 *qs = static_cast<uint4 *>(qsplit);
    if (np == 3) hipLaunchKernelGGL(ivf_split_queries<3>, dim3((unsigned)ceil_div(nthr, 256)), dim3(256), 0, st, Q, nq, d, nsup, qs);
    else hipLaunchKernelGGL(ivf_split_queries<2>, dim3((unsigned)ceil_div(nthr, 256)), dim3(256), 0, st, Q, nq, d, nsup, qs);
    const int nh = mb_phases(d, np);
    const int group = mb_group(d, np);
    const size_t merge = (size_t)(MF_WAVES / 2) * MF_QTMAX * 4 * 64 * sizeof(float2);
    const size_t smem = std::max((size_t)group * mb_stride(d, np, nh) * 4, merge);
    dim3 grid((unsigned)max_items), block(MF_THREADS);
#define MB_LAUNCH_ARGS qs, qn, d, codes_t, tpass_off, xn, list_off, list_len, cnt, bucket_off, item_off, bucket, slot_off, nlist, nprobe, \
                       group, k, sub, qbound, pd, pi
#define MB_LAUNCH(NP_, NH_)                                                                                         \
    do {                                                                                                            \
        if (metric == kIP) hipLaunchKernelGGL((ivf_scan_mfma_bf<true, NP_, NH_>), grid, block, smem, st, MB_LAUNCH_ARGS); \
        else hipLaunchKernelGGL((ivf_scan_mfma_bf<false, NP_, NH_>), grid, block, smem, st, MB_LAUNCH_ARGS);       \
    } while (0)
    if (np == 3) {
        if (nh == 2) MB_LAUNCH(3, 2); else MB_LAUNCH(3, 1);
    } else {
        if (nh == 2) MB_LAUNCH(2, 2); else MB_LAUNCH(2, 1);
    }
#undef MB_LAUNCH
#undef MB_LAUNCH_ARGS
    HIPANN_CHECK(hipGetLastError());
}


typedef _Float16 mh_f16x8 __attribute__((ext_vector_type(8)));
#ifndef HIPANN_MH_P
#define HIPANN_MH_P 6
#endif
#ifndef HIPANN_MH_INSERT
#define HIPANN_MH_INSERT 3
#endif
#ifndef HIPANN_MH_STATS
#define HIPANN_MH_STATS 0
#endif
#if HIPANN_MH_STATS
__device__ unsigned long long mh_stats_dev[2][2][5];
#endif
constexpr int MH_P = HIPANN_MH_P;
__host__ __device__ inline int mh_nsup(int d) { return (int)ceil_div(ceil_div(d, 32), MH_P) * MH_P; }
__host__ __device__ inline int mh_stride(int d) { return mh_nsup(d) * 16 + 8; }
inline bool mh_two_term_fits(int d) { return MF_LDS_MAX / ((size_t)(2 * mh_nsup(d) * 16 + 8) * 4) >= 16; }
constexpr int MH_QTW = 6;
inline int mh_group_wide(int d) {
    const int g = (int)(MF_LDS_MAX / ((size_t)mh_stride(d) * 4 + 8)) / 16 * 16;
    return g < 16 * MH_QTW ? g : 16 * MH_QTW;
}
inline int mh_group_packed(int d) { return mh_two_term_fits(d) ? mh_group_wide(d) << 8 : 0; }

__device__ __forceinline__ unsigned short mh_half_bits(float v) {
    const _Float16 h = (_Float16)v;
    return __builtin_fabsf((float)h) < 0x1p-14f ? (unsigned short)0 : __builtin_bit_cast(unsigned short, h);
}
__device__ __forceinline__ float mh_val(unsigned short b) { return (float)__builtin_bit_cast(_Float16, b); }
__device__ __forceinline__ unsigned mh_pack(float a, float b) {
    return (unsigned)mh_half_bits(a) | ((unsigned)mh_half_bits(b) << 16);
}

__device__ __forceinline__ mf_f32x4 mh_mfma(const uint4 &a, const uint4 &b, const mf_f32x4 &c) {
    return __builtin_amdgcn_mfma_f32_16x16x32_f16(__builtin_bit_cast(mh_f16x8, a), __builtin_bit_cast(mh_f16x8, b), c,
                                                  0, 0, 0);
}

typedef int mf_i32x4 __attribute__((ext_vector_type(4)));
__host__ __device__ inline int mi_nsup(int d) { return (int)ceil_div(ceil_div(d, 64), MH_P) * MH_P; }
__device__ __forceinline__ int mi_quant(float x, float s) {
    return s > 0.f ? (int)fminf(fmaxf(rintf(x / s), -127.f), 127.f) : 0;
}
__device__ __forceinline__ uint4 mi_units(const float *x, int dim0, int d, float s) {
    unsigned w[4] = {0u, 0u, 0u, 0u};
#pragma unroll
    for (int i = 0; i < 16; ++i) {
        const int v = dim0 + i < d ? mi_quant(x[dim0 + i], s) : 0;
        w[i >> 2] |= ((unsigned)v & 0xffu) << (8 * (i & 3));
    }
    return make_uint4(w[0], w[1], w[2], w[3]);
}
__device__ __forceinline__ float mi_row_scale(const float *x, int d, int lane) {
    float mx = 0.f;
    for (int e = lane; e < d; e += 64) mx = fmaxf(mx, fabsf(x[e]));
#pragma unroll
    for (int o = 32; o > 0; o >>= 1) mx = fmaxf(mx, __shfl_xor(mx, o));
    return mx > 0.f && mx < 3.0e38f ? mx / 127.f : (mx == 0.f ? 0.f : -1.f);
}

__global__ void __launch_bounds__(256)
ivf_tile_i8(const float *__restrict__ codes, const int64_t *__restrict__ list_off, const int *__restrict__ list_len,
            const int64_t *__restrict__ tpass_off, int nlist, int d, int nsup, uint4 *__restrict__ dst,
            float *__restrict__ xs8, float *__restrict__ xr8, unsigned *__restrict__ nonfin,
            const int64_t *__restrict__ pass_ids) {
    const int64_t pass = pass_ids ? pass_ids[blockIdx.x] : (int64_t)blockIdx.x;
    int lo = 0, hi = nlist - 1;
    while (lo < hi) {
        const int mid = (lo + hi + 1) >> 1;
        if (tpass_off[mid] <= pass) lo = mid; else hi = mid - 1;
    }
    const int l = lo;
    const int64_t r0 = list_off[l] + (pass - tpass_off[l]) * 32, rend = list_off[l] + list_len[l];
    __shared__ float sc[32];
    const int wave = threadIdx.x >> 6, lane = threadIdx.x & 63;
    for (int rr = wave; rr < 32; rr += 4) {
        const int64_t row = r0 + rr;
        float s = 0.f, res = 0.f;
        if (row < rend) {
            const float *x = codes + row * (int64_t)d;
            s = mi_row_scale(x, d, lane);
            if (s < 0.f) {
                s = 0.f;
                res = __builtin_inff();
            } else {
                float r2 = 0.f;
                for (int e = lane; e < d; e += 64) {
                    const float t = x[e] - s * (float)mi_quant(x[e], s);
                    r2 = fmaf(t, t, r2);
                }
#pragma unroll
                for (int o = 32; o > 0; o >>= 1) r2 += __shfl_xor(r2, o);
                res = sqrtf(r2) * 1.0001f;
            }
        }
// ... 444 lines not shown
                    const float sc = I8 ? qiv * xsr[r] : qiv;
                    if (IP) {
                        key = -av * sc;
                    } else {
                        key = fmaf(-2.f * sc, av, qnv + xnr[r]);
                        if constexpr (I8) key = fmaf(-qrv, xrr[r], key);
                        key = key < 0.f ? 0.f : key;
                    }
                    const bool ok = rok && qt * 16 + 4 * g + v < nqi;
                    const unsigned ks = mf_sortable(key);
                    uint64_t cp = ok ? (((uint64_t)ks << 32) | rid) : MF_EMPTY;
                    if (HIPANN_MH_STATS) ++st_step;
                    if (HIPANN_MF_EXPERIMENT == 1) {
                        sink ^= cp;
                    } else if (const uint64_t hit = __ballot(ok && ks <= thr[qt][v])) {
                        int most = 0;
#pragma unroll
                        for (int f = 0; f < 4; ++f) {
                            const int c = __popc((unsigned)(hit >> (16 * f)) & 0xffffu);
                            most = c > most ? c : most;
                        }
                        if (HIPANN_MH_STATS) { ++st_hit; st_rows += __popcll(hit); st_ins += most <= HIPANN_MH_INSERT; }
                        if (most <= HIPANN_MH_INSERT) {
                            uint64_t pend = hit;
                            do {
                                uint64_t first = 0;
#pragma unroll
                                for (int f = 0; f < 4; ++f) {
                                    const unsigned x = (unsigned)(pend >> (16 * f)) & 0xffffu;
                                    first |= (uint64_t)(x & (0u - x)) << (16 * f);
                                }
                                row_insert1(lst[qt][v], (first >> lane) & 1 ? cp : MF_EMPTY);
                                pend &= ~first;
                            } while (HIPANN_MH_INSERT > 1 && pend);
                        } else {
                            row_sort16(cp, m);
                            row_merge16(lst[qt][v], cp, m);
                        }
                        thr[qt][v] = row_kth_key(lst[qt][v], k - 1, g);
                    }
                }
        }
#pragma unroll
        for (int r = 0; r < MF_RT; ++r) {
            xnr[r] = xnr_next[r];
            xsr[r] = xsr_next[r];
            xrr[r] = xrr_next[r];
        }
    }

    if (HIPANN_MF_EXPERIMENT == 1 && sink == 1) part_d[0] = 0.f;
#if HIPANN_MH_STATS
    if (lane == 0) {
        unsigned long long *st = mh_stats_dev[I8][stat_part];
        atomicAdd(st + 0, (unsigned long long)npass);
        atomicAdd(st + 1, (unsigned long long)st_step);
        atomicAdd(st + 2, (unsigned long long)st_hit);
        atomicAdd(st + 3, (unsigned long long)st_rows);
        atomicAdd(st + 4, (unsigned long long)st_ins);
    }
#endif
    mf_finish_item<QT>(lst, smem, nqi, bucket, boff, nprobe, slot_off, chunk, k, sub, qbound, part_d, part_i);
}

template <int TS>
__device__ __forceinline__ void mh_fill(unsigned *qs, const uint4 *__restrict__ qsplit, int nsup, int stride, int nqi,
                                        const int *__restrict__ bucket, int boff, int nprobe) {
    const int per_q = nsup * 4;
    for (int t = threadIdx.x; t < nqi * per_q; t += MF_THREADS) {
        const int q = t / per_q, r2 = t - q * per_q;
        const int gq = bucket[boff + q] / nprobe;
        *reinterpret_cast<uint4 *>(qs + q * stride + r2 * 4) = qsplit[(int64_t)gq * TS * nsup * 4 + r2];
    }
}

template <bool IP, bool I8>
__global__ void __launch_bounds__(MF_THREADS, MF_WAVES / 4)
ivf_scan_mfma_h(const uint4 *__restrict__ qsplit, const float *__restrict__ qnorm, const float *__restrict__ its, int d,
                const uint4 *__restrict__ codes_h, const int64_t *__restrict__ tpass_off, const float *__restrict__ xn,
                const int64_t *__restrict__ list_off, const int *__restrict__ list_len, const int *__restrict__ cnt, const int *__restrict__ bucket_off,
                const int *__restrict__ item_off, const int *__restrict__ bucket, const int *__restrict__ slot_off,
                int nlist, int nprobe, int group, int k, int sub, unsigned *__restrict__ qbound, float *__restrict__ part_d,
                int *__restrict__ part_i, float *__restrict__ qres, int nq, int remap, const float *__restrict__ xs8,
                const float *__restrict__ xr8, const float *__restrict__ qhn) {
    extern __shared__ __attribute__((aligned(16))) float smem[];
    const int total = item_off[nlist];
    if ((int)blockIdx.x >= total) return;
    const int item = remap ? xcd_remap((int)blockIdx.x, total) : (int)blockIdx.x;
    int lo = 0, hi = nlist - 1;
    while (lo < hi) {
        const int mid = (lo + hi + 1) >> 1;
        if (item_off[mid] <= item) lo = mid; else hi = mid - 1;
    }
    const int l = lo;
    const int64_t lr0 = list_off[l], lr1 = lr0 + list_len[l];
    const int c = cnt[l];
    const int ng = ivf_ngroups(c, group);
    const int rem = item - item_off[l];
    const int chunk = rem / ng, grp = rem - chunk * ng;
    const int q_begin = (int)((int64_t)grp * c / ng), q_end = (int)((int64_t)(grp + 1) * c / ng);
    const int nqi = q_end - q_begin;
    const int64_t r0 = lr0 + (int64_t)chunk * MF_CH;
    const int64_t r1 = r0 + MF_CH < lr1 ? r0 + MF_CH : lr1;
    const int boff = bucket_off[l] + q_begin;
    const int nqt = (nqi + 15) >> 4;

    const int64_t tp0 = tpass_off[l] + (int64_t)chunk * (MF_CH / MF_PASS);
    unsigned *qs = reinterpret_cast<unsigned *>(smem);
    const int nsup = I8 ? mi_nsup(d) : mh_nsup(d);
    const int stride = I8 ? mi_nsup(d) * 16 + 8 : mh_stride(d);
    float *qpar = reinterpret_cast<float *>(qs + nqi * stride);
    mh_fill<I8 ? 1 : 2>(qs, qsplit, nsup, stride, nqi, bucket, boff, nprobe);
    for (int t = threadIdx.x; t < nqi; t += MF_THREADS) {
        const int qi = bucket[boff + t] / nprobe;
        if constexpr (I8)
            reinterpret_cast<float4 *>(qpar)[t] =
                make_float4(IP ? 0.f : qnorm[qi], its[qi], IP ? 0.f : 2.f * qhn[qi], 0.f);
        else reinterpret_cast<float2 *>(qpar)[t] = make_float2(IP ? 0.f : qnorm[qi], its[qi]);
        if (!I8) qres[qi] = qres[nq + qi];
    }

    const int lane = threadIdx.x & 63, g = lane >> 4;
    const int stat_part = (int64_t)blockIdx.x * 5 < (int64_t)total ? 0 : 1;
#define MH_CASE(QTV)                                                                                        \
    {                                                                                                       \
        unsigned qb[QTV][4];                                                                                \
        _Pragma("unroll") for (int qt = 0; qt < QTV; ++qt) _Pragma("unroll") for (int v = 0; v < 4; ++v) {  \
            const int q = qt * 16 + 4 * g + v;                                                              \
            const int qi = q < nqi ? bucket[boff + q] / nprobe : 0;                                         \
            qb[qt][v] = q < nqi ? __atomic_load_n(qbound + qi, __ATOMIC_RELAXED) : 0xffffffffu;             \
        }                                                                                                   \
        mh_item<QTV, IP, I8>(d, codes_h, tp0, xn, r0, r1, nqi, qs, stride, qb, qpar, bucket, boff, nprobe, slot_off, \
                             chunk, k, sub, smem, qbound, part_d, part_i, xs8, xr8, stat_part);             \
    }
    switch (nqt) {
    case 0: case 1: MH_CASE(1) break;
    case 2: MH_CASE(2) break;
    case 3: MH_CASE(3) break;
    case 4: MH_CASE(4) break;
    case 5: MH_CASE(5) break;
    default: MH_CASE(6) break;
    }
#undef MH_CASE
}

void ivf_mh_stats_report() {
#if HIPANN_MH_STATS
    unsigned long long h[2][2][5];
    if (hipMemcpyFromSymbol(h, HIP_SYMBOL(mh_stats_dev), sizeof(h)) != hipSuccess) return;
    for (int i8 = 0; i8 < 2; ++i8)
        for (int part = 0; part < 2; ++part)
            std::fprintf(stderr, "HIPANN_MH_STATS image=%s blocks=%s passes=%llu steps=%llu hit_steps=%llu admitted_rows=%llu "
                                 "insert_steps=%llu\n", i8 ? "int8" : "fp16", part ? "rest" : "first_fifth", h[i8][part][0],
                         h[i8][part][1], h[i8][part][2], h[i8][part][3], h[i8][part][4]);
    std::memset(h, 0, sizeof(h));
    (void)hipMemcpyToSymbol(HIP_SYMBOL(mh_stats_dev), h, sizeof(h));
#endif
}

int ivf_mfma_h_group(int d) { return mh_group_packed(d); }
int ivf_scan_sublists() { return MF_WAVES; }
int64_t ivf_half_pass_bytes(int d) { return (int64_t)mh_nsup(d) * MF_RT * 64 * 16; }
int64_t ivf_half_qsplit_bytes(int64_t nq, int d) { return nq * 2 * mh_nsup(d) * 64; }
bool ivf_mfma_h_supported(int d, int k) { return d >= 1 && k >= 1 && k <= MF_KMAX && mh_two_term_fits(d); }
int ivf_mfma_i8_group(int d) {
    const int g = (int)(MF_LDS_MAX / ((size_t)(mi_nsup(d) * 16 + 8) * 4 + 16)) / 16 * 16;
    return (g < 16 * MH_QTW ? g : 16 * MH_QTW) << 8;
}
int64_t ivf_i8_pass_bytes(int d) { return (int64_t)mi_nsup(d) * MF_RT * 64 * 16; }
int64_t ivf_i8_qimg_bytes(int64_t nq, int d) { return nq * mi_nsup(d) * 64; }
bool ivf_mfma_i8_supported(int d, int k) {
    return d >= 1 && k >= 1 && k <= MF_KMAX && ivf_group_wide(ivf_mfma_i8_group(d)) >= 16;
}
void launch_ivf_tile_i8(const float *codes, const int64_t *list_off, const int *list_len, const int64_t *tpass_off,
                        int nlist, int64_t total_pass, int d, void *dst, float *xs8, float *xr8, unsigned *nonfin,
                        hipStream_t st, const int64_t *pass_ids) {
    if (nonfin) HIPANN_CHECK(hipMemsetAsync(nonfin, 0, sizeof(unsigned), st));
    if (total_pass <= 0) return;
    HIPANN_REQUIRE(total_pass < (int64_t)0x7fffffff, "too many passes");
    HIPANN_REQUIRE(xs8 && xr8, "int8 image: missing scale / residual planes");
    hipLaunchKernelGGL(ivf_tile_i8, dim3((unsigned)total_pass), dim3(256), 0, st, codes, list_off, list_len, tpass_off,
                       nlist, d, mi_nsup(d), static_cast<uint4 *>(dst), xs8, xr8, nonfin, pass_ids);
    HIPANN_CHECK(hipGetLastError());
}
void launch_ivf_split_queries_i8(const float *Q, int64_t nq, int d, void *qi8, float *qs8, float *qres8,
                                 float *qhn2, float *qhn, hipStream_t st) {
    if (nq <= 0) return;
    HIPANN_REQUIRE(ceil_div(nq, 4) < (int64_t)0x7fffffff, "too many queries");
    hipLaunchKernelGGL(ivf_split_queries_i8, dim3((unsigned)ceil_div(nq, 4)), dim3(256), 0, st, Q, nq, d, mi_nsup(d),
                       static_cast<uint4 *>(qi8), qs8, qres8, qhn2, qhn);
    HIPANN_CHECK(hipGetLastError());
}

void launch_ivf_max_abs(const float *x, int64_t cnt, unsigned *out, hipStream_t st) {
    HIPANN_CHECK(hipMemsetAsync(out, 0, sizeof(unsigned), st));
    if (cnt <= 0) return;
    const unsigned blocks = (unsigned)std::min<int64_t>(4096, ceil_div(cnt, 256));
    hipLaunchKernelGGL(ivf_max_abs, dim3(blocks), dim3(256), 0, st, x, cnt, out);
    HIPANN_CHECK(hipGetLastError());
}

void launch_ivf_tile_half(const float *codes, const int64_t *list_off, const int *list_len, const int64_t *tpass_off,
                          int nlist, int64_t total_pass, int d, float scale, void *dst, hipStream_t st,
                          const int64_t *pass_ids) {
    if (total_pass <= 0) return;
    HIPANN_REQUIRE(total_pass < (int64_t)0x7fffffff, "too many passes");
    hipLaunchKernelGGL(ivf_tile_half, dim3((unsigned)total_pass), dim3(256), 0, st, codes, list_off, list_len, tpass_off,
                       nlist, d, mh_nsup(d), scale, static_cast<uint4 *>(dst), pass_ids);
    HIPANN_CHECK(hipGetLastError());
}

void launch_ivf_half_residual(const float *codes, int64_t n, int d, float scale, unsigned *out, hipStream_t st) {
    HIPANN_CHECK(hipMemsetAsync(out, 0, sizeof(unsigned), st));
    if (n <= 0) return;
    HIPANN_REQUIRE(ceil_div(n, 4) < (int64_t)0x7fffffff, "too many rows");
    hipLaunchKernelGGL(ivf_half_residual, dim3((unsigned)ceil_div(n, 4)), dim3(256), 0, st, codes, n, d, scale,
                       1.f / scale, out);
    HIPANN_CHECK(hipGetLastError());
}

void launch_ivf_append_rows(const float *rows, const float *norms, const int64_t *dst, const int64_t *ids_in, int64_t n,
                            int d, float *codes, int64_t *ids, float *xnorm, const int *newlen, int *list_len, int nlist,
                            float hscale, unsigned *stat, hipStream_t st) {
    int64_t blocks = std::max(ceil_div(n, (int64_t)4), ceil_div((int64_t)nlist, (int64_t)256));
    if (!dst) blocks = std::min<int64_t>(blocks, 64);
    HIPANN_REQUIRE(blocks < (int64_t)0x7fffffff, "append block too large");
    if (stat) HIPANN_CHECK(hipMemsetAsync(stat, 0, sizeof(unsigned) * 4, st));
    hipLaunchKernelGGL(ivf_append_rows, dim3((unsigned)blocks), dim3(256), 0, st, rows, norms, dst, ids_in, n, d, codes,
                       ids, xnorm, newlen, list_len, nlist, hscale, stat);
    HIPANN_CHECK(hipGetLastError());
}

void launch_ivf_split_queries_h(const float *Q, int64_t nq, int d, int es, void *qsplit, float *its, float *qres,
                                float *qn, hipStream_t st) {
    if (nq <= 0) return;
    const int vec4 = (d % 4 == 0) && ((uintptr_t)Q % 16 == 0);
    hipLaunchKernelGGL(ivf_split_queries_h, dim3((unsigned)ceil_div(nq, 4)), dim3(256), 0, st, Q, nq, d, mh_nsup(d), es,
                       static_cast<uint4 *>(qsplit), its, qres, qn, vec4);
    HIPANN_CHECK(hipGetLastError());
}

void launch_ivf_scan_mfma_h(int64_t nq, const void *qsplit, const float *its, float *qres, const float *qn, int d,
                            int metric, const void *codes_h, const int64_t *tpass_off, const float *xn,
                            const int64_t *list_off, const int *list_len, const int *cnt, const int *bucket_off,
                            const int *item_off, const int *bucket, const int *slot_off, int nlist, int nprobe, int k,
                            int64_t max_items, unsigned *qbound, float *pd, int *pi, hipStream_t st, int sub, int i8mode,
                            const float *xs8, const float *xr8, const float *qhn) {
    if (max_items <= 0 || nq <= 0) return;
    HIPANN_REQUIRE(max_items < (int64_t)0x7fffffff, "too many IVF work items");
    HIPANN_REQUIRE(qsplit && its && qres && codes_h, "fp16 IVF scan: missing buffers");
    HIPANN_REQUIRE(i8mode ? ivf_mfma_i8_supported(d, k) && xs8 : ivf_mfma_h_supported(d, k),
                   "fp16 / int8 IVF scan needs k <= 16 (int8: scales and prepared queries)");
    HIPANN_REQUIRE(metric == kIP || (qn && xn), "decomposed L2 scan needs query and row norms");
    HIPANN_REQUIRE(!i8mode || metric == kIP || (xr8 && qhn), "int8 L2 scan needs the rows' residuals and the queries' norms");
    const uint4 *qs = static_cast<const uint4 *>(qsplit);
    const int group = i8mode ? ivf_mfma_i8_group(d) : mh_group_packed(d);
    const size_t merge = (size_t)(MF_WAVES / 2) * MH_QTW * 4 * 64 * sizeof(float2);
    const size_t per_q = i8mode ? (size_t)(mi_nsup(d) * 16 + 8) * 4 + 16 : (size_t)mh_stride(d) * 4 + 8;
    const size_t smem = std::max((size_t)ivf_group_wide(group) * per_q, merge);
    HIPANN_REQUIRE(smem <= MF_LDS_MAX, "fp16 IVF scan: LDS image too large");
    HIPANN_REQUIRE(nq < (int64_t)0x7fffffff, "fp16 IVF scan: batch too large");
    dim3 grid((unsigned)max_items), block(MF_THREADS);
    const uint4 *ch = static_cast<const uint4 *>(codes_h);
    static const int remap = [] { const char *e = std::getenv("HIPANN_IVF_REMAP"); return !e || std::atoi(e) ? 1 : 0; }();
#define MH_LAUNCH_ARGS qs, qn, its, d, ch, tpass_off, xn, list_off, list_len, cnt, bucket_off, item_off, bucket, slot_off, nlist, nprobe, \
                       group, k, sub, qbound, pd, pi, qres, (int)nq, remap, xs8, xr8, qhn
    if (i8mode) {
        if (metric == kIP) hipLaunchKernelGGL((ivf_scan_mfma_h<true, true>), grid, block, smem, st, MH_LAUNCH_ARGS);
        else hipLaunchKernelGGL((ivf_scan_mfma_h<false, true>), grid, block, smem, st, MH_LAUNCH_ARGS);
    } else {
        if (metric == kIP) hipLaunchKernelGGL((ivf_scan_mfma_h<true, false>), grid, block, smem, st, MH_LAUNCH_ARGS);
        else hipLaunchKernelGGL((ivf_scan_mfma_h<false, false>), grid, block, smem, st, MH_LAUNCH_ARGS);
    }
#undef MH_LAUNCH_ARGS
    HIPANN_CHECK(hipGetLastError());
}

}
```

### duckdb-annsearch_amd/csrc/runtime.hpp

```cpp
#pragma once
#include "common.hpp"
#include <cstdlib>
#include <ctime>
#include <memory>
#include <mutex>
#include <vector>

namespace hipann {

struct DeviceGuard {
    int prev = 0;
    explicit DeviceGuard(int dev) {
        HIPANN_CHECK(hipGetDevice(&prev));
        if (prev != dev) HIPANN_CHECK(hipSetDevice(dev));
    }
    ~DeviceGuard() { (void)hipSetDevice(prev); }
};

struct DevBuf {
    void *p = nullptr;
    size_t bytes = 0;
    int device = 0;
    DevBuf() = default;
    DevBuf(const DevBuf &) = delete;
// ... 222 lines not shown
    DevBuf xb16, qimg, seed;
    DevBuf cand;
    bool xb16_ok = false;
    bool keys_bf3 = false;
    float bf16_rxmax = 0.f;
    DevBuf xi8, xscale, qscale, qres;
    bool xi8_ok = false;
    float i8_rxmax = 0.f;
    StreamFence fence;
    HostBuf h_nflag;
    unsigned flag_seq = 0;
    DevBuf app_stat;
    hipEvent_t done = nullptr;
};

struct FlatPending {
    enum Kind { kNone = 0, kSmallI8 = 1, kExact = 2 };
    int kind = kNone;
    int64_t nq = 0;
    const float *xq = nullptr;
    int k = 0, kout = 0;
    float *D = nullptr;
    int64_t *I = nullptr;
    const float *cr_d = nullptr, *cr_bound = nullptr;
    const int *cr_i = nullptr, *cr_n = nullptr;
    int cr_nsplit = 0, cr_cap = 0;
    float xmax2 = 0.f, rxmax = 0.f;
    bool i8 = false;
};

struct IndexBase {
    Kind kind;
    int d = 0;
    int metric = kL2;
    std::mutex mu;
    KernelTimer timer_main, timer_merge;
    int last_form = -1, last_kfilt = 0, last_sublists = 0;
    std::vector<int> peer;
    explicit IndexBase(Kind k) : kind(k) {}
    virtual ~IndexBase() = default;
    virtual int64_t ntotal() const = 0;
    virtual int64_t memory_bytes() const = 0;
};

struct FlatIndex : IndexBase {
    std::vector<std::unique_ptr<FlatShard>> shards;
    int form = kFlatI8Exact;
    int64_t rerank_fallbacks = 0;
    int64_t cand_reranked = 0;
    int64_t host_syncs = 0;
    HostBuf h_q, h_d, h_i;
    DevBuf gather_d, gather_i, merged_d, merged_i;
    FlatIndex() : IndexBase(Kind::Flat) {}
    ~FlatIndex() override;
    int64_t ntotal() const override {
        int64_t t = 0;
        for (auto &s : shards) t += s->n;
        return t;
    }
    int64_t memory_bytes() const override {
        int64_t b = 0;
        for (auto &s : shards)
            b += s->n * (int64_t)d * 4 + (metric == kL2 ? s->n * 4 : 0) + (int64_t)s->xb16.bytes +
                 (int64_t)s->xi8.bytes + (int64_t)s->xscale.bytes;
        return b;
    }
};

struct IvfShard {
    int device = 0;
    int64_t n = 0;
    int64_t live = 0;
    const float *centroids = nullptr;
    const float *codes = nullptr;
    const int64_t *ids = nullptr;
    DevBuf centroids_buf, codes_buf, ids_buf;
    DevBuf list_off;
    DevBuf list_len;
    DevBuf xnorm;
    std::unique_ptr<FlatIndex> quant;
    hipStream_t stream = nullptr;
    DevBuf q, qn, coarse_d, coarse_i, cnt, bucket_off, item_off, cursor, bucket, slot_off, part_d, part_i, out_d, out_i;
    DevBuf qbound;
    DevBuf qsplit;
    float xmax2 = -1.f;
    DevBuf nflag, flagged, fq, fD, fI, coarse_save, tmpnorm;
    DevBuf ccnt, qtot;
    DevBuf cursor2;
    uint64_t plan_batch = 0;
    int plan_nlist = 0;
    DevBuf fpd, fpi;
    DevBuf fb_total;
    DevBuf fbc_d, fbc_i, fbc_done;
    int fbc_cap = 0;
    std::vector<int64_t> h_off;
    std::vector<int64_t> h_len;
    bool owns_codes = false;
    DevBuf codes_t, tpass_off;
    int half_state = 0, half_es = 0;
    float half_rxmax = 0.f;
    DevBuf codes_h, hsplit, hits, hres;
    int i8_state = 0;
    float i8_rxmax = -1.f;
    int64_t i8_tiled = 0;
    DevBuf codes_i8, xs8, xr8, qi8, qs8, qres8, qhn2, qhn;
    int auto8 = 0, auto8_over = 0;
    int64_t auto8_live = 0;
    HostBuf fb_host;
    uint64_t fb_seq = 0, fb_seen = 0;
    bool count_only = false;
    DevBuf probe_D, probe_I;
    DevBuf app_rows, app_norm, app_assign, app_up, app_stat;
    DevBuf app_cd;
    HostBuf app_hassign, app_hup[2];
    hipEvent_t app_ev[2] = {nullptr, nullptr};
    hipEvent_t app_sync = nullptr;
    int app_buf = 0;
    int max_nch = 1;
    StreamFence fence;
    hipEvent_t done = nullptr;
};

struct IvfIndex : IndexBase {
    int nlist = 0, nprobe = 1;
    std::vector<int> owner;
    int form = kFormHalfExact;
    int filter_image = 2, last_filter_image = 0;
    int64_t rerank_fallbacks = 0;
    std::vector<std::unique_ptr<IvfShard>> shards;
    int64_t last_nq = 0;
    int last_np = 0;
    HostBuf h_q, h_d, h_i;
    DevBuf gather_d, gather_i, merged_d, merged_i;
    IvfIndex() : IndexBase(Kind::IVF) {}
    ~IvfIndex() override;
    int64_t ntotal() const override {
        int64_t t = 0;
        for (auto &s : shards) t += s->live;
        return t;
    }
    int64_t memory_bytes() const override {
        int64_t b = 0;
        for (auto &s : shards)
            b += s->n * ((int64_t)d * 4 + 8 + (metric == kL2 ? 4 : 0)) + (int64_t)nlist * d * 4 +
                 (int64_t)s->codes_h.bytes + (int64_t)s->codes_t.bytes + (int64_t)s->codes_i8.bytes + (int64_t)s->xs8.bytes +
                 (int64_t)s->xr8.bytes;
        return b;
    }
};

std::vector<int> enable_peer_access(const std::vector<int> &devs);

constexpr size_t kKernelCopyMax = (size_t)64 << 10;
void launch_copy_words(const void *src, void *dst, size_t bytes, hipStream_t st);
void launch_post_words(const void *src, void *host_dst, int words, unsigned token, hipStream_t st);
void *host_device_ptr(void *pinned);
void launch_row_norms(const float *x, int64_t n, int d, float *out, hipStream_t st);
size_t gemm_smem_bytes();
void launch_flat_gemm_topk(const float *Q, const float *qn, int64_t nq, const float *X, const float *xn, int64_t N,
                           int d, int metric, int k, int nsplit, int64_t tiles_per_split, float *pd, int *pi,
                           hipStream_t st);
size_t flat_bf_qsplit_bytes(int64_t nq, int d, int np);
void launch_flat_gemm_topk_bf(int np, const float *Q, const float *qn, int64_t nq, void *qsplit, const float *X,
                              const float *xn, int64_t N, int d, int metric, int k, int nsplit, int64_t tiles_per_split,
                              float *pd, int *pi, int qmajor, hipStream_t st);
size_t scan_smem_bytes(int nq, int d);
void launch_flat_gemm_keys(const float *Q, const float *qn, int64_t nq, const float *X, const float *xn, int64_t N,
                           int d, int metric, float *keys, int64_t ldk, hipStream_t st, bool bf3 = false);
void launch_flat_scan_keys(const float *Q, int nq, const float *X, int64_t N, int d, int metric, float *keys,
                           int64_t ldk, hipStream_t st);
void launch_rows_topk(const float *keys, int64_t ldk, int64_t ncols, int64_t nq, int64_t seg_len, int nseg, int k,
                      int id0, float *pd, int *pi, hipStream_t st);
bool launch_rows_select_out(const float *keys, int64_t ldk, int64_t ncols, int64_t nq, int k, int kout,
                            int64_t label_offset, float out_sign, float *D, int64_t *I, hipStream_t st,
                            IvfPlanHook *hook = nullptr);
void launch_merge_raw(const float *pd, const int *pi, int nparts, int64_t nq, int k, float *od, int *oi,
                      hipStream_t st);
void launch_flat_scan_topk(const float *Q, int nq, const float *X, int64_t N, int d, int metric, int k, int nwaves,
                           int64_t rows_per_wave, float *pd, int *pi, hipStream_t st);
void launch_ivf_plan(const int64_t *probes, int64_t nq, int nprobe, const int *list_len, int nlist, int group,
                     int *cnt, int *bucket_off, int *item_off, int *cursor, int *bucket, int *slot_off,
                     hipStream_t st, int *nflag_reset = nullptr, unsigned *qbound = nullptr, int *ccnt = nullptr,
                     int *qtot = nullptr, bool counted = false, int *ccnt_next = nullptr, int *cursor_next = nullptr);
int64_t ivf_max_items(int64_t nq, int nprobe, int nlist, int max_nch, int64_t nrows, int group);
int ivf_mfma_bf_group(int d, int np);
bool ivf_mfma_bf_supported(const float *Q, int d, const float *codes, int k, int np);
int64_t ivf_mfma_bf_qsplit_bytes(int64_t nq, int d, int np);
void launch_flat_cand_rerank(const int *flagged, int nf, const float *cand_d, const int *cand_i, const int *cand_n,
                             int nsplit, int cap, const float *bound, const float *Q, const float *X, int d,
                             int64_t nrows, int64_t label_offset, float xmax2, float rxmax, int metric, int kout,
                             float *part_d, long long *part_i, int *ovf, float *D, int64_t *I, int *nflag2,
                             int *flagged2, hipStream_t st, float *dbg = nullptr, const float *qres = nullptr);
int flat_cand_rerank_parts(int nsplit);
void launch_ivf_rerank(const float *pd, const int *pi, const int *slot_off, int nprobe, int64_t nq, int k, int kout,
                       int metric, const float *Q, const float *codes, int d, const int64_t *ids, int64_t nrows,
                       int64_t label_offset, float xmax2, float *D, int64_t *I, int *nflag, int *flagged,
                       hipStream_t st, float eps = kSplit2Eps, float rxmax = -1.f, const float *qres = nullptr,
                       const int64_t *probes = nullptr, const int64_t *list_off = nullptr, int nlist = 0,
                       const unsigned *qbound = nullptr, const float *qnorm = nullptr, int kslot = 0, int sub = 0,
                       const int *list_len = nullptr, float *fpd = nullptr, long long *fpi = nullptr,
                       unsigned long long *fb_total = nullptr,
                       int fb_cap = 0,
                       int i8_l2 = 0);
void launch_ivf_fallback_chunks(const int *nflag, const int *flagged, int fb_cap, int nprobe, int maxch, int chunk_rows,
                                int kout, int metric, const float *Q, const float *codes, int d, const int64_t *ids,
                                int64_t label_offset, const int64_t *probes, const int64_t *list_off,
                                const int *list_len, int nlist, float *cpd, long long *cpi, unsigned *done, float *D,
                                int64_t *I, unsigned long long *total, hipStream_t st,
                                unsigned long long *host_word = nullptr, unsigned host_seq = 0);
int ivf_mfma_h_group(int d);
void ivf_mh_stats_report();
int ivf_scan_sublists();
int64_t ivf_half_pass_bytes(int d);
int64_t ivf_half_qsplit_bytes(int64_t nq, int d);
bool ivf_mfma_h_supported(int d, int k);
void launch_ivf_max_abs(const float *x, int64_t cnt, unsigned *out, hipStream_t st);
void launch_ivf_tile_half(const float *codes, const int64_t *list_off, const int *list_len, const int64_t *tpass_off,
                          int nlist, int64_t total_pass, int d, float scale, void *dst, hipStream_t st,
                          const int64_t *pass_ids = nullptr);
void launch_ivf_half_residual(const float *codes, int64_t n, int d, float scale, unsigned *out, hipStream_t st);
void launch_ivf_scan_mfma_h(int64_t nq, const void *qsplit, const float *its, float *qres, const float *qn, int d,
                            int metric, const void *codes_h, const int64_t *tpass_off, const float *xn,
                            const int64_t *list_off, const int *list_len, const int *cnt, const int *bucket_off,
                            const int *item_off, const int *bucket, const int *slot_off, int nlist, int nprobe, int k,
                            int64_t max_items, unsigned *qbound, float *pd, int *pi, hipStream_t st, int sub = 0,
                            int i8mode = 0, const float *xs8 = nullptr, const float *xr8 = nullptr,
                            const float *qhn = nullptr);
int ivf_mfma_i8_group(int d);
int64_t ivf_i8_pass_bytes(int d);
int64_t ivf_i8_qimg_bytes(int64_t nq, int d);
bool ivf_mfma_i8_supported(int d, int k);
void launch_ivf_tile_i8(const float *codes, const int64_t *list_off, const int *list_len, const int64_t *tpass_off,
                        int nlist, int64_t total_pass, int d, void *dst, float *xs8, float *xr8, unsigned *nonfin,
                        hipStream_t st, const int64_t *pass_ids = nullptr);
void launch_ivf_split_queries_i8(const float *Q, int64_t nq, int d, void *qi8, float *qs8, float *qres8,
                                 float *qhn2, float *qhn, hipStream_t st);
void launch_ivf_split_queries_h(const float *Q, int64_t nq, int d, int es, void *qsplit, float *its, float *qres,
                                float *qn, hipStream_t st);
int flat_bf16_waves(int64_t nq);
int flat_bf16_tile_rows();
int flat_bf16_topk_kmax(int64_t nq);
int flat_gemm_topk_bf_kmax(int np);
size_t flat_bf16_img_bytes(int64_t n, int d, int R);
void launch_b16_tile_rows(const float *X, int64_t n, int d, int R, void *out, hipStream_t st);
void launch_b16_row_residual2(const float *X, int64_t n, int d, float *out, hipStream_t st);
void launch_flat_bf16_topk(const float *Q, const float *qn, int64_t nq, void *qimg, const void *ximg, const float *xn,
                           int64_t N, int d, int metric, int k, int nsplit, int64_t tiles_per_split, float *pd, int *pi,
                           const float *seed, bool image_ready, hipStream_t st);
bool flat_bf16_resumable(int64_t nq, int d, int k);
void launch_flat_bf16_k64(const void *qimg, const float *qn, int64_t nq, const void *ximg, const float *xn, int64_t N,
                          int nk, int metric, int nqt, int nsplit, int64_t tiles_per_split, int64_t tile_begin,
                          int64_t tile_end, const float *bound, float *cand_d, int *cand_i, int *cand_n, int cap,
                          bool resume, bool keys, hipStream_t st, const float *qscale = nullptr,
                          const float *xscale = nullptr);
int flat_i8_nk(int d);
size_t flat_i8_img_bytes(int64_t n, int d, int R);
void launch_i8_row_scale(const float *X, int64_t n, int d, float *scale, float *resid, hipStream_t st);
void launch_i8_tile_rows(const float *X, const float *scale, int64_t n, int d, int R, void *out, hipStream_t st);
void launch_i8_query_prep(const float *X, int64_t n, int d, float *qn, float *scale, float *resid, int R, void *out,
                          hipStream_t st);
int flat_i8_scan_k();
int flat_i8_scan_max_nq();
int64_t flat_i8_scan_waves(int64_t n);
void launch_flat_i8_scan(const float *Q, int64_t nq, int d, int metric, const void *ximg, const float *xscale,
                         const float *xnorm, int64_t n, float *qscale, float *qres, const float *qnorm, void *qimg,
                         float *part_d, int *part_i, int64_t nw, hipStream_t st);
void launch_flat_i8_group_merge(const float *pd, const int *pi, int nw, int nq, int ngroup, float *od, int *oi,
                                hipStream_t st);
int flat_keys_kth_max();
void launch_flat_keys_kth(const float *keys, int S, int64_t nq, int k, float *bound, hipStream_t st);
void launch_flat_cand_bound(const float *cand_d, const int *cand_n, int nsplit, int cap, int64_t nq, int k,
                            float *bound, hipStream_t st);
void launch_flat_cand_select(const float *cand_d, const int *cand_i, const int *cand_n, int nsplit, int cap, int64_t nq,
                             int k, float *out_d, int *out_i, int *nflag, int *flagged, hipStream_t st);
void launch_flat_bf16_seed(const float *pd, int nsplit, int64_t nq, int k, float *seed, hipStream_t st);
bool flat_bf16_k64_supported(int nk, int k);
void launch_ivf_max_norm(const float *xn, int64_t n, unsigned *out, hipStream_t st);
void launch_ivf_gather_queries(const float *Q, const int *idx, int nf, int d, float *out, hipStream_t st);
void launch_ivf_append_rows(const float *rows, const float *norms, const int64_t *dst, const int64_t *ids_in, int64_t n,
                            int d, float *codes, int64_t *ids, float *xnorm, const int *newlen, int *list_len, int nlist,
                            float hscale, unsigned *stat, hipStream_t st);
int64_t flat_remove_scan_blocks(int64_t cnt);
void launch_flat_remove_plan(const int64_t *rows, int64_t m, int64_t first, int64_t cnt, unsigned char *keep,
                             int64_t *sums, int64_t *src, hipStream_t st);
void launch_flat_gather_rows(const float *X, const int64_t *idx, int64_t cnt, int d, float *out, hipStream_t st);
void launch_flat_gather_f32(const float *v, const int64_t *idx, int64_t cnt, float *out, hipStream_t st);
void launch_ivf_remove_rows(const int64_t *labels, int64_t m, const int64_t *list_off, int *list_len, int nlist, int d,
                            float *codes, int64_t *ids, float *xnorm, unsigned char *mark, int *plan,
                            const int64_t *tpass_off, int64_t *pass_ids, unsigned long long *npass, int *newlen,
                            hipStream_t st);
void launch_ivf_scatter_results(const float *Df, const int64_t *If, const int *idx, int nf, int kout, float *D,
                                int64_t *I, hipStream_t st);
void launch_ivf_scan_mfma_bf(int np, const float *Q, int64_t nq, void *qsplit, const float *qn, int d, int metric,
                             const float *codes_t, const int64_t *tpass_off, const float *xn, const int64_t *list_off,
                             const int *list_len, const int *cnt, const int *bucket_off, const int *item_off, const int *bucket,
                             const int *slot_off, int nlist, int nprobe, int k, int64_t max_items, unsigned *qbound,
                             float *pd, int *pi, hipStream_t st, int sub = 0);
int ivf_group_size(int form, int d);
int ivf_chunk_rows();
bool ivf_plan_query_major();
void launch_ivf_scan_bigk(const float *Q, int d, int metric, const float *codes, const int64_t *list_off,
                          const int *list_len, const int64_t *probes, int64_t npairs, int nprobe, const int *slot_off, int64_t nslots,
                          int k, float *pd, int *pi, hipStream_t st);
size_t ivf_scan_smem_bytes();
bool ivf_dot_supported(const float *Q, int d, const float *codes);
void launch_ivf_scan(const float *Q, const float *qn, int d, int metric, int form, const float *codes,
                     const float *xn, const int64_t *list_off, const int *list_len, const int *cnt,
                     const int *bucket_off, const int *item_off, const int *bucket, const int *slot_off, int nlist,
                     int nprobe, int64_t nq,
                     int k, int64_t max_items, unsigned *qbound, float *pd, int *pi, hipStream_t st);
// ... 24 lines not shown
```

### duckdb-annsearch_amd/hipann.py

```python
from __future__ import annotations

import ctypes as C
import os
import subprocess
import threading
from pathlib import Path
from typing import Optional, Sequence, Tuple

import numpy as np

HERE = Path(__file__).resolve().parent
LIB_PATH = Path(os.environ["HIPANN_LIB"]) if os.environ.get("HIPANN_LIB") else HERE / "libhipann.so"

METRIC_L2 = 0
METRIC_INNER_PRODUCT = 1
MAX_K = 2048

MIN_GPU_WORK = 786432
MIN_GPU_WORK_ONESHOT = 65536
AUTO_MIN_WORK = 1048576


class HipAnnError(RuntimeError):
    """Raised when libhipann.so reports an error (the C ABI's err_buf text)."""


_lib = None
_lib_lock = threading.Lock()


def build(force: bool = False) -> Path:
    if force or not LIB_PATH.exists():
        subprocess.run(["make", "-s", "-C", str(HERE / "csrc"), "-j8"], check=True)
    return LIB_PATH


def _share_torch_hip_runtime() -> None:
    if os.environ.get("HIPANN_STANDALONE") == "1":
        return
    try:
        import torch
    except Exception:
        pass


def lib() -> C.CDLL:
    global _lib
    with _lib_lock:
        if _lib is not None:
            return _lib
        if not LIB_PATH.exists():
            raise HipAnnError(f"libhipann.so not built ({LIB_PATH}); run hipann.build()")
        _share_torch_hip_runtime()
        L = C.CDLL(str(LIB_PATH))
        vp, f, i64p, i64, i32, cp = C.c_void_p, C.POINTER(C.c_float), C.POINTER(C.c_int64), C.c_int64, C.c_int, C.c_char_p
        u32p = C.POINTER(C.c_uint32)
        sig = {
            "hipann_available": ([], i32),
            "hipann_device_count": ([], i32),
            "hipann_device_info": ([cp, i32], i32),
            "hipann_peer_access": ([vp, C.POINTER(C.c_int), i32, cp, i32], i32),
            "hipann_flat_create": ([i32, i32, f, i64, C.POINTER(C.c_int), i32, cp, i32], vp),
            "hipann_flat_add": ([vp, f, i64, cp, i32], i32),
            "hipann_flat_remove_ids": ([vp, i64p, i64, cp, i32], i64),
            "hipann_flat_search": ([vp, i64, f, i64, f, i64p, cp, i32], i32),
            "hipann_flat_reconstruct": ([vp, i64, f, cp, i32], i32),
            "hipann_flat_create_device": ([i32, i32, vp, i64, i32, i32, i64, cp, i32], vp),
            "hipann_flat_search_device": ([vp, i64, vp, i64, vp, vp, vp, cp, i32], i32),
            "hipann_flat_set_form": ([vp, i32], i32),
            "hipann_flat_get_form": ([vp], i32),
            "hipann_last_search_path": ([vp, C.POINTER(C.c_int), C.POINTER(C.c_int), C.POINTER(C.c_int)], i32),
            "hipann_flat_rerank_fallbacks": ([vp], i64),
            "hipann_flat_host_syncs": ([vp], i64),
            "hipann_merge_topk_device": ([i32, i32, i64, i64, vp, vp, vp, vp, vp, cp, i32], i32),
            "hipann_merge_topk_packed_device": ([i32, i32, i64, i64, vp, i64, vp, vp, vp, cp, i32], i32),
            "hipann_ivf_create": ([i32, i32, i32, i32, f, i64p, i64p, f, C.POINTER(C.c_int), i32, cp, i32], vp),
            "hipann_ivf_create_device": ([i32, i32, i32, i32, vp, i64p, vp, vp, i32, i32, cp, i32], vp),
            "hipann_ivf_search": ([vp, i64, f, i64, f, i64p, cp, i32], i32),
            "hipann_ivf_search_device": ([vp, i64, vp, i64, vp, vp, vp, cp, i32], i32),
            "hipann_ivf_coarse_device": ([vp, i64, vp, vp, vp, cp, i32], i32),
            "hipann_ivf_search_probes_device": ([vp, i64, vp, vp, i64, vp, vp, vp, cp, i32], i32),
            "hipann_ivf_last_probes": ([vp, i64p, i64, cp, i32], i32),
            "hipann_ivf_set_nprobe": ([vp, i32], i32),
            "hipann_ivf_get_nprobe": ([vp], i32),
            "hipann_ivf_nlist": ([vp], i32),
            "hipann_ivf_search_np": ([vp, i32, i64, f, i64, f, i64p, cp, i32], i32),
            "hipann_ivf_add": ([vp, i64, f, i64p, cp, i32], i32),
            "hipann_ivf_remove_ids": ([vp, i64p, i64, cp, i32], i64),
            "hipann_ivf_export": ([vp, f, i64p, i64p, f, cp, i32], i32),
            "hipann_ivf_train": ([i32, i32, i32, i64, f, i64, i32, C.c_uint64, i32, i32, f, i64p, cp, i32], i32),
            "hipann_ivf_train_device": ([i32, i32, i32, i64, vp, i64, i32, C.c_uint64, i32, i32, vp, vp, cp, i32],
                                        i32),
            "hipann_flat_reconstruct_n": ([vp, i64, i64, f, cp, i32], i32),
            "hipann_ivf_set_form": ([vp, i32], i32),
            "hipann_ivf_get_form": ([vp], i32),
            "hipann_ivf_rerank_fallbacks": ([vp], i64),
            "hipann_ivf_i8_passes_tiled": ([vp], i64),
            "hipann_ivf_set_filter_image": ([vp, i32], i32),
            "hipann_ivf_get_filter_image": ([vp], i32),
            "hipann_ivf_last_filter_image": ([vp], i32),
            "hipann_ntotal": ([vp], i64),
            "hipann_dim": ([vp], i32),
            "hipann_metric": ([vp], i32),
            "hipann_memory_bytes": ([vp], i64),
            "hipann_free": ([vp], None),
            "hipann_set_kernel_timing": ([vp, i32], i32),
            "hipann_last_kernel_ms": ([vp, i32], C.c_double),
            "diskann_hip_available": ([], i32),
            "diskann_hip_batch_distances": ([f, f, i32, i32, i32, f], i32),
            "diskann_hip_multi_batch_distances": ([f, f, u32p, i32, i32, i32, i32, f], i32),
            "diskann_metal_available": ([], i32),
            "diskann_metal_batch_distances": ([f, f, i32, i32, i32, f], i32),
            "diskann_metal_multi_batch_distances": ([f, f, u32p, i32, i32, i32, i32, f], i32),
            "diskann_hip_register_db": ([vp, i64, i32, i32, f, f], vp),
            "diskann_hip_multi_batch_distances_ids": ([vp, f, i32, u32p, u32p, i32, i32, f], i32),
            "diskann_hip_multi_batch_distances_ids_device": ([vp, vp, i32, vp, vp, i32, i32, vp, vp], i32),
            "diskann_hip_db_size": ([vp], i64),
            "diskann_hip_release_db": ([vp], None),
            "diskann_hip_set_kernel_timing": ([vp, i32], i32),
            "diskann_hip_register_graph": ([vp, C.POINTER(C.c_uint32), i32], i32),
            "diskann_hip_search_batch_resident": ([vp, C.POINTER(C.c_uint32), i32, f, i32, i32, i32, i32, i64p, f,
                                                   i64p, cp, i32], i32),
            "diskann_hip_search_batch_resident_device": ([vp, C.POINTER(C.c_uint32), i32, vp, i32, i32, i32, i32, vp,
                                                          vp, i64p, vp, cp, i32], i32),
            "diskann_hip_kernel_stats": ([vp, C.POINTER(C.c_double), i64p], i32),
            "diskann_hip_search_batch": ([vp, C.POINTER(C.c_uint32), i32, C.POINTER(C.c_uint32), i32, f, i32, i32,
                                          i32, i32, i64p, f, i64p, cp, i32], i32),
            "diskann_hip_build_graph": ([vp, i32, i32, C.c_float, i32, C.c_uint32, i32, C.POINTER(C.c_uint32), i64p, cp,
                                         i32], i32),
            "diskann_hip_robust_prune": ([vp, C.POINTER(C.c_uint32), i32, C.POINTER(C.c_uint32), i32, i32, C.c_float,
                                          i32, C.POINTER(C.c_uint32), cp, i32], i32),
            "diskann_hip_build_phase_seconds": ([vp, C.POINTER(C.c_double)], i32),
            "diskann_hip_remove_ids": ([vp, i64p, i64, C.c_float, i32, C.POINTER(C.c_uint32), i64,
                                        C.POINTER(C.c_uint32), i64p, cp, i32], i64),
            "diskann_hip_remove_phase_seconds": ([vp, C.POINTER(C.c_double)], i32),
            "diskann_hip_add_rows": ([vp, f, i64, i32, C.c_float, i32, C.c_uint32, i32, i32, C.POINTER(C.c_uint32),
                                      i64p, cp, i32], i64),
            "diskann_hip_batch_mates": ([vp, i64, i32, i32, C.POINTER(C.c_uint32), cp, i32], i32),
            "diskann_hip_add_phase_seconds": ([vp, C.POINTER(C.c_double)], i32),
        }
        missing = [name for name in sig if not hasattr(L, name)]
        if missing:
            raise HipAnnError(f"libhipann.so is missing exports: {missing}")
        for name, (args, res) in sig.items():
            fn = getattr(L, name)
            fn.argtypes = args
            fn.restype = res
        _lib = L
        return L


def _ptr(a: Optional[np.ndarray], t):
    return None if a is None else a.ctypes.data_as(C.POINTER(t))


def _err() -> C.Array:
    return C.create_string_buffer(1024)


def _check(rc, eb) -> None:
    if rc != 0:
        raise HipAnnError(eb.value.decode(errors="replace") or "hipann error")


def _f32_2d(x, d: Optional[int] = None) -> np.ndarray:
    x = np.ascontiguousarray(x, dtype=np.float32)
    if x.ndim == 1:
        x = x.reshape(1, -1) if d is None else x.reshape(-1, d)
    if d is not None and x.shape[1] != d:
        raise ValueError(f"expected dimension {d}, got {x.shape[1]}")
    return x


def is_available() -> bool:
    try:
        return bool(lib().hipann_available())
    except (HipAnnError, OSError):
        return False


def device_count() -> int:
    return int(lib().hipann_device_count())


def device_info() -> str:
    buf = C.create_string_buffer(512)
    lib().hipann_device_info(buf, 512)
    return buf.value.decode()


class _Handle:
    def __init__(self, h, d: int, metric: int):
        if not h:
            raise HipAnnError("null handle")
        self._h = C.c_void_p(h)
        self.d = d
        self.metric_type = metric

    def close(self) -> None:
        if getattr(self, "_h", None):
            lib().hipann_free(self._h)
            self._h = None

    def __del__(self):
        try:
            self.close()
        except Exception:
            pass

    @property
    def ntotal(self) -> int:
        return int(lib().hipann_ntotal(self._h))

    @property
    def memory_bytes(self) -> int:
        return int(lib().hipann_memory_bytes(self._h))

    def set_kernel_timing(self, on: bool) -> None:
        lib().hipann_set_kernel_timing(self._h, 1 if on else 0)

    def last_search_path(self) -> dict:
        f, kf, sl = C.c_int(-1), C.c_int(0), C.c_int(0)
        lib().hipann_last_search_path(self._h, C.byref(f), C.byref(kf), C.byref(sl))
        return {"form": f.value, "filter_k": kf.value, "sublists": sl.value}

    def kernel_ms(self, which: int = 0) -> float:
        return float(lib().hipann_last_kernel_ms(self._h, which))

    PEER_SAME_DEVICE, PEER_ENABLED, PEER_UNAVAILABLE = 2, 1, 0

    def peer_access(self) -> list:
        eb = _err()
        n = lib().hipann_peer_access(self._h, None, 0, eb, 1024)
        _check(min(n, 0), eb)
        st = (C.c_int * max(n, 1))()
        _check(min(lib().hipann_peer_access(self._h, st, n, eb, 1024), 0), eb)
        return [int(st[i]) for i in range(n)]

    @property
    def handle(self) -> C.c_void_p:
        return self._h


class _FlatForm:

    FORM_FP32 = 0
    FORM_SPLIT3 = 1
    FORM_SPLIT2 = 2
    FORM_SPLIT2_EXACT = 3
    FORM_BF16_EXACT = 4
    FORM_I8_EXACT = 5

    @property
    def form(self) -> int:
        return int(lib().hipann_flat_get_form(self._h))

    @form.setter
    def form(self, v: int) -> None:
        if lib().hipann_flat_set_form(self._h, int(v)) != 0:
            raise HipAnnError("form must be 0 (fp32), 1 (split bf16, 3 terms), 2 (split bf16, 2 terms), "
                              "3 (split bf16 + exact rerank), 4 (bf16 + exact rerank) or 5 (int8 + exact rerank)")

    def rerank_fallbacks(self) -> int:
        return int(lib().hipann_flat_rerank_fallbacks(self._h))

    def host_syncs(self) -> int:
        return int(lib().hipann_flat_host_syncs(self._h))


class HipIndexFlat(_FlatForm, _Handle):

    def __init__(self, d: int, metric: int = METRIC_L2, xb=None, devices: Optional[Sequence[int]] = None):
        x = _f32_2d(xb, d) if xb is not None else np.zeros((0, d), np.float32)
        devs = (C.c_int * len(devices))(*devices) if devices else None
        eb = _err()
        h = lib().hipann_flat_create(d, metric, _ptr(x, C.c_float), x.shape[0], devs, len(devices) if devices else 0,
                                     eb, 1024)
        if not h:
            raise HipAnnError(eb.value.decode())
        super().__init__(h, d, metric)

    def add(self, x) -> None:
        x = _f32_2d(x, self.d)
        eb = _err()
        _check(lib().hipann_flat_add(self._h, _ptr(x, C.c_float), x.shape[0], eb, 1024), eb)

    def remove_ids(self, labels) -> int:
        lab = np.ascontiguousarray(labels, dtype=np.int64).reshape(-1)
        eb = _err()
        rc = int(lib().hipann_flat_remove_ids(self._h, _ptr(lab, C.c_int64), lab.size, eb, 1024))
        _check(min(rc, 0), eb)
        return rc

    def search(self, x, k: int) -> Tuple[np.ndarray, np.ndarray]:
        x = _f32_2d(x, self.d)
        n = x.shape[0]
        D = np.empty((n, max(k, 0)), np.float32)
        I = np.empty((n, max(k, 0)), np.int64)
        eb = _err()
        _check(lib().hipann_flat_search(self._h, n, _ptr(x, C.c_float), k, _ptr(D, C.c_float), _ptr(I, C.c_int64),
                                        eb, 1024), eb)
        return D, I

    def reconstruct_n(self, i0: int, n: int) -> np.ndarray:
        out = np.empty((max(n, 0), self.d), np.float32)
        eb = _err()
        _check(lib().hipann_flat_reconstruct_n(self._h, i0, n, _ptr(out, C.c_float), eb, 1024), eb)
# ... 537 lines not shown
```

### include/hip_ann.h

```cpp
#ifndef HIP_ANN_H
#define HIP_ANN_H

#include <stdint.h>

#ifdef __cplusplus
extern "C" {
#endif

#define HIPANN_METRIC_L2 0
#define HIPANN_METRIC_IP 1

#define HIPANN_MAX_K 2048
#define HIPANN_AUTO_MIN_WORK 1048576

int hipann_available(void);

int hipann_device_count(void);

int hipann_device_info(char *buf, int buf_len);

int hipann_peer_access(void *index, int *state, int cap, char *err_buf, int err_len);


void *hipann_flat_create(int d, int metric, const float *xb, int64_t n, const int *devices, int ndev,
// ... 16 lines not shown
#define HIPANN_FLAT_FORM_SPLIT2_EXACT 3
#define HIPANN_FLAT_FORM_BF16_EXACT 4
#define HIPANN_FLAT_FORM_I8_EXACT 5
int hipann_flat_set_form(void *index, int form);
int hipann_flat_get_form(void *index);
int64_t hipann_flat_rerank_fallbacks(void *index);
int64_t hipann_flat_host_syncs(void *index);

int hipann_last_search_path(void *index, int *form, int *filter_k, int *sublists);


void *hipann_flat_create_device(int d, int metric, const float *xb_dev, int64_t n, int device, int copy,
                                int64_t label_offset, char *err_buf, int err_len);

int hipann_flat_search_device(void *index, int64_t nq, const float *xq_dev, int64_t k, float *D_dev,
                              int64_t *I_dev, void *stream, char *err_buf, int err_len);

int hipann_merge_topk_device(int metric, int nparts, int64_t nq, int64_t k, const float *D_parts,
                             const int64_t *I_parts, float *D_out, int64_t *I_out, void *stream,
                             char *err_buf, int err_len);

int hipann_merge_topk_packed_device(int metric, int nparts, int64_t nq, int64_t k, const void *parts,
                                    int64_t part_bytes, float *D_out, int64_t *I_out, void *stream,
                                    char *err_buf, int err_len);


void *hipann_ivf_create(int d, int metric, int nlist, int nprobe, const float *centroids,
                        const int64_t *list_offsets, const int64_t *ids, const float *codes,
                        const int *devices, int ndev, char *err_buf, int err_len);

void *hipann_ivf_create_device(int d, int metric, int nlist, int nprobe, const float *centroids_dev,
                               const int64_t *list_offsets, const int64_t *ids_dev, const float *codes_dev,
                               int device, int copy, char *err_buf, int err_len);

int hipann_ivf_search(void *index, int64_t nq, const float *xq, int64_t k, float *D, int64_t *I,
                      char *err_buf, int err_len);

int hipann_ivf_search_np(void *index, int nprobe, int64_t nq, const float *xq, int64_t k, float *D, int64_t *I,
                         char *err_buf, int err_len);

int hipann_ivf_search_device(void *index, int64_t nq, const float *xq_dev, int64_t k, float *D_dev,
                             int64_t *I_dev, void *stream, char *err_buf, int err_len);

int hipann_ivf_last_probes(void *index, int64_t *probes, int64_t cap, char *err_buf, int err_len);
int hipann_ivf_coarse_device(void *index, int64_t nq, const float *xq_dev, int64_t *probes_dev, void *stream,
                             char *err_buf, int err_len);
int hipann_ivf_search_probes_device(void *index, int64_t nq, const float *xq_dev, const int64_t *probes_dev,
                                    int64_t k, float *D_dev, int64_t *I_dev, void *stream, char *err_buf, int err_len);

int hipann_ivf_set_nprobe(void *index, int nprobe);
int hipann_ivf_get_nprobe(void *index);
int hipann_ivf_nlist(void *index);

int hipann_ivf_add(void *index, int64_t n, const float *xb, const int64_t *ids, char *err_buf, int err_len);

int64_t hipann_ivf_remove_ids(void *index, const int64_t *labels, int64_t n, char *err_buf, int err_len);

#define HIPANN_KMEANS_INIT_RANDOM 0
#define HIPANN_KMEANS_INIT_PLUSPLUS 1
int hipann_ivf_train(int d, int metric, int nlist, int64_t n, const float *x, int64_t train_sample, int niter,
                     uint64_t seed, int init, int device, float *centroids, int64_t *list_sizes, char *err_buf,
                     int err_len);

int hipann_ivf_train_device(int d, int metric, int nlist, int64_t n, const float *x_dev, int64_t train_sample,
                            int niter, uint64_t seed, int init, int device, float *centroids_dev, void *stream,
                            char *err_buf, int err_len);

int hipann_ivf_export(void *index, float *centroids, int64_t *list_offsets, int64_t *ids, float *codes,
                      char *err_buf, int err_len);

#define HIPANN_IVF_FORM_DECOMPOSED 0
#define HIPANN_IVF_FORM_DIRECT 1
#define HIPANN_IVF_FORM_DECOMPOSED_VALU 2
#define HIPANN_IVF_FORM_SPLIT3 3
#define HIPANN_IVF_FORM_SPLIT2 4
#define HIPANN_IVF_FORM_SPLIT2_EXACT 5
#define HIPANN_IVF_FORM_HALF_EXACT 6
#define HIPANN_IVF_FORM_I8_EXACT 7
int hipann_ivf_set_form(void *index, int form);
int hipann_ivf_get_form(void *index);
int hipann_ivf_set_filter_image(void *index, int mode);
int hipann_ivf_get_filter_image(void *index);
int hipann_ivf_last_filter_image(void *index);
int64_t hipann_ivf_i8_passes_tiled(void *index);
int64_t hipann_ivf_rerank_fallbacks(void *index);


int64_t hipann_ntotal(void *index);
int hipann_dim(void *index);
int hipann_metric(void *index);
int64_t hipann_memory_bytes(void *index);
void hipann_free(void *index);

int hipann_set_kernel_timing(void *index, int on);

double hipann_last_kernel_ms(void *index, int which);

#ifdef __cplusplus
}
#endif

#endif
```

Before: 542,800 queries/s.

## Seed per-query bounds with a chunk-0 scan before scanning remaining chunks

Splits the int8-image IVF scan into two phases. The first scans only the first chunk of each probed list, and a new seed-bound kernel merges those partials into per-query candidate lists and tightens the qbound threshold. The second phase scans the remaining chunks with that tighter bound, so more rows are pruned early. This adds an extra kernel launch, a group-offset prefix in the plan kernels, and extra partial-buffer space, and it only helps when lists span more than one chunk.

```diff
diff --git a/duckdb-annsearch_amd/csrc/common.hpp b/duckdb-annsearch_amd/csrc/common.hpp
--- a/duckdb-annsearch_amd/csrc/common.hpp
+++ b/duckdb-annsearch_amd/csrc/common.hpp
@@ -48,6 +48,7 @@
 };
 constexpr int kRerankK = 16, kRerankMaxK = 12;
 constexpr int kIvfSubMaxK = 60;
+constexpr int kSeedK = 64;
 constexpr int kFlatRerankKIP = 32;
 enum FlatForm : int {
     kFlatFp32 = 0,
@@ -73,6 +74,24 @@
     return ivf_group_narrow(group) > 0 ? ivf_group_narrow(group) : ivf_group_wide(group);
 }
 
+__host__ __device__ inline int ivf_phase_first(int phase, int item_off_l, int goff_l) {
+    return phase == 1 ? goff_l : phase == 2 ? item_off_l - goff_l : item_off_l;
+}
+__host__ __device__ inline int ivf_phase_list(int phase, const int *item_off, const int *goff, int nlist, int item) {
+    int lo = 0, hi = nlist - 1;
+    while (lo < hi) {
+        const int mid = (lo + hi + 1) >> 1;
+        if (ivf_phase_first(phase, item_off[mid], phase ? goff[mid] : 0) <= item) lo = mid; else hi = mid - 1;
+    }
+    return lo;
+}
+__host__ __device__ inline void ivf_phase_decode(int phase, int rem, int ng, int &chunk, int &grp) {
+    chunk = phase == 1 ? 0 : rem / ng + (phase == 2 ? 1 : 0);
+    grp = phase == 1 ? rem : rem % ng;
+}
+__host__ __device__ inline int64_t ivf_seed_run_slot(int slot0, int64_t q) { return (int64_t)slot0 + q; }
+__host__ __device__ inline int ivf_seed_pair_slots(int nch) { return nch > 1 ? nch - 1 : 0; }
+
 __device__ __forceinline__ int xcd_remap(int bid, int nblocks) {
     const int q = nblocks >> 3, r = nblocks & 7;
     const int xcd = bid & 7, j = bid >> 3;
diff --git a/duckdb-annsearch_amd/csrc/ivf.cpp b/duckdb-annsearch_amd/csrc/ivf.cpp
--- a/duckdb-annsearch_amd/csrc/ivf.cpp
+++ b/duckdb-annsearch_amd/csrc/ivf.cpp
@@ -399,6 +399,9 @@
         ix.last_kfilt = exact ? kfilt : 0;
         ix.last_sublists = sub ? ivf_scan_sublists() : 0;
     }
+    static const bool seed_env = [] { const char *e = std::getenv("HIPANN_IVF_SEED"); return !e || std::atoi(e) != 0; }();
+    const bool seeded = seed_env && i8 && metric == kL2 && sub && sh.max_nch > 1 && ivf_seed_supported(np, kslot);
+    if (form_override < 0) ix.last_seeded = seeded ? 1 : 0;
     const bool tiled = form == kFormDecomposed || ivf_form_split(form);
     const int group = i8 ? ivf_mfma_i8_group(d) : half ? ivf_mfma_h_group(d) : ivf_group_size(form, d);
     float xmax2 = 0.f;
@@ -472,6 +475,7 @@
     sh.cnt.ensure(sizeof(int) * (nlist + 1), sh.device);
     sh.bucket_off.ensure(sizeof(int) * (nlist + 1), sh.device);
     sh.item_off.ensure(sizeof(int) * (nlist + 1), sh.device);
+    sh.goff.ensure(sizeof(int) * (nlist + 1), sh.device);
     sh.bucket.ensure(sizeof(int) * (size_t)nq * np, sh.device);
     HIPANN_REQUIRE((int64_t)nq * np < (int64_t)0x7fffffff, "nq * nprobe too large");
     sh.slot_off.ensure(sizeof(int) * ((size_t)nq * np + 1), sh.device);
@@ -480,15 +484,17 @@
     launch_ivf_plan(sh.coarse_i.get<int64_t>(), nq, np, sh.list_len.get<int>(), nlist, group, sh.cnt.get<int>(),
                     sh.bucket_off.get<int>(), sh.item_off.get<int>(), cur_cur, sh.bucket.get<int>(),
                     sh.slot_off.get<int>(), st, exact ? sh.nflag.get<int>() : nullptr, qbound, ccnt_cur,
-                    sh.qtot.get<int>(), hook.done, ccnt_next, cur_next);
+                    sh.qtot.get<int>(), hook.done, ccnt_next, cur_next, sh.goff.get<int>());
     }
     sh.plan_batch++;
     ccnt_reset.armed = false;
-    const size_t parts = (size_t)np * nq * sh.max_nch * kslot;
+    const size_t parts = ((size_t)np * nq * sh.max_nch + (seeded ? (size_t)np * nq + (size_t)nq : 0)) * kslot;
     HIPANN_REQUIRE((int64_t)np * nq * sh.max_nch < (int64_t)0x7fffffff, "too many partial lists");
     sh.part_d.ensure(parts * sizeof(float), sh.device);
     sh.part_i.ensure(parts * sizeof(int), sh.device);
     const int64_t max_items = ivf_max_items(nq, np, nlist, sh.max_nch, sh.n, group);
+    float *cand_d = nullptr;
+    int *cand_i = nullptr;
     const float *qn = nullptr;
     if (form != kFormDirect && metric == kL2) {
         const FlatShard &qs = *sh.quant->shards[0];
@@ -511,14 +517,30 @@
         RoctxRange rr("hipann.ivf.scan");
         ScopedTiming t(ix.timer_main, st);
         if (img) {
-            launch_ivf_scan_mfma_h(nq, i8 ? sh.qi8.p : sh.hsplit.p, i8 ? sh.qs8.get<float>() : sh.hits.get<float>(),
-                                   i8 ? sh.qres8.get<float>() : sh.hres.get<float>(), cert8 ? sh.qhn2.get<float>() : qn, d,
-                                   metric, i8 ? sh.codes_i8.p : sh.codes_h.p, sh.tpass_off.get<int64_t>(), sh.xnorm.get<float>(),
-                                   sh.list_off.get<int64_t>(), sh.list_len.get<int>(), sh.cnt.get<int>(), sh.bucket_off.get<int>(),
-                                   sh.item_off.get<int>(), sh.bucket.get<int>(), sh.slot_off.get<int>(), nlist, np, k,
-                                   max_items, qbound, sh.part_d.get<float>(), sh.part_i.get<int>(), st, sub ? 1 : 0,
-                                   i8 ? 1 : 0, i8 ? sh.xs8.get<float>() : nullptr,
-                                   cert8 ? sh.xr8.get<float>() : nullptr, cert8 ? sh.qhn.get<float>() : nullptr);
+            auto scan_h = [&](int phase, const int *slots, int64_t items, float *pd, int *pi, int subl) {
+                launch_ivf_scan_mfma_h(nq, i8 ? sh.qi8.p : sh.hsplit.p, i8 ? sh.qs8.get<float>() : sh.hits.get<float>(),
+                                       i8 ? sh.qres8.get<float>() : sh.hres.get<float>(), cert8 ? sh.qhn2.get<float>() : qn, d,
+                                       metric, i8 ? sh.codes_i8.p : sh.codes_h.p, sh.tpass_off.get<int64_t>(), sh.xnorm.get<float>(),
+                                       sh.list_off.get<int64_t>(), sh.list_len.get<int>(), sh.cnt.get<int>(), sh.bucket_off.get<int>(),
+                                       sh.item_off.get<int>(), sh.bucket.get<int>(), slots, nlist, np, k,
+                                       items, qbound, pd, pi, st, subl,
+                                       i8 ? 1 : 0, i8 ? sh.xs8.get<float>() : nullptr,
+                                       cert8 ? sh.xr8.get<float>() : nullptr, cert8 ? sh.qhn.get<float>() : nullptr, phase,
+                                       sh.goff.get<int>());
+            };
+            if (seeded) {
+                HIPANN_REQUIRE((int64_t)np * nq * sh.max_nch + nq < (int64_t)0x7fffffff, "too many candidate slots");
+                sh.cslot.ensure(sizeof(int) * (size_t)nq * np, sh.device);
+                sh.bcnt.ensure(sizeof(int) * (size_t)nq, sh.device);
+                cand_d = sh.part_d.get<float>() + (size_t)np * nq * kslot;
+                cand_i = sh.part_i.get<int>() + (size_t)np * nq * kslot;
+                scan_h(1, nullptr, ivf_max_items(nq, np, nlist, 1, 0, group), sh.part_d.get<float>(), sh.part_i.get<int>(), 1);
+                launch_ivf_seed_bound(sh.part_d.get<float>(), sh.part_i.get<int>(), sh.slot_off.get<int>(), np, nq, kslot,
+                                      sh.n, qbound, cand_d, cand_i, sh.cslot.get<int>(), sh.bcnt.get<int>(), st);
+                scan_h(2, sh.cslot.get<int>(), ivf_max_items(nq, np, nlist, sh.max_nch - 1, sh.n, group), cand_d, cand_i, 1);
+            } else {
+                scan_h(0, sh.slot_off.get<int>(), max_items, sh.part_d.get<float>(), sh.part_i.get<int>(), sub ? 1 : 0);
+            }
         }
         else if (bigk)
             launch_ivf_scan_bigk(xq, d, metric, sh.codes, sh.list_off.get<int64_t>(), sh.list_len.get<int>(),
@@ -573,14 +595,16 @@
     {
         RoctxRange rr("hipann.ivf.rerank");
         ScopedTiming t(ix.timer_merge, st);
-        launch_ivf_rerank(sh.part_d.get<float>(), sh.part_i.get<int>(), sh.slot_off.get<int>(), np, nq, kfilt, kout,
+        launch_ivf_rerank(seeded ? cand_d : sh.part_d.get<float>(), seeded ? cand_i : sh.part_i.get<int>(),
+                          sh.slot_off.get<int>(), np, nq, kfilt, kout,
                           metric, xq, sh.codes, d, sh.ids, sh.n, 0, xmax2, D, I, sh.nflag.get<int>(),
                           sh.flagged.get<int>(), st, kSplit2Eps, i8 ? rxmax8 : half ? sh.half_rxmax : -1.f,
                           i8 ? sh.qres8.get<float>() : half ? sh.hres.get<float>() : nullptr, sh.coarse_i.get<int64_t>(),
                           sh.list_off.get<int64_t>(), nlist, qbound, img && metric == kL2 ? qn : nullptr, kslot,
                           sub ? 1 : 0, inline_fb ? sh.list_len.get<int>() : nullptr,
                           inline_fb ? sh.fpd.get<float>() : nullptr, inline_fb ? sh.fpi.get<long long>() : nullptr,
-                          inline_fb ? sh.fb_total.get<unsigned long long>() : nullptr, fb_cap, cert8 ? 1 : 0);
+                          inline_fb ? sh.fb_total.get<unsigned long long>() : nullptr, fb_cap, cert8 ? 1 : 0,
+                          seeded ? sh.bcnt.get<int>() : nullptr);
         if (fb_cap > 0)
             launch_ivf_fallback_chunks(sh.nflag.get<int>(), sh.flagged.get<int>(), fb_cap, np, fb_maxch, ivf_chunk_rows(),
                                        kout, metric, xq, sh.codes, d, sh.ids, 0, sh.coarse_i.get<int64_t>(),
@@ -1411,6 +1435,13 @@
     return static_cast<IvfIndex *>(ix)->last_filter_image;
 }
 
+int hipann_ivf_last_seeded(void *h) {
+    if (!h) return -1;
+    auto *ix = static_cast<IndexBase *>(h);
+    if (ix->kind != Kind::IVF) return -1;
+    return static_cast<IvfIndex *>(ix)->last_seeded;
+}
+
 int64_t hipann_ivf_i8_passes_tiled(void *h) {
     if (!h) return -1;
     auto *ix = static_cast<IndexBase *>(h);
diff --git a/duckdb-annsearch_amd/csrc/ivf_kernels.hip b/duckdb-annsearch_amd/csrc/ivf_kernels.hip
--- a/duckdb-annsearch_amd/csrc/ivf_kernels.hip
+++ b/duckdb-annsearch_amd/csrc/ivf_kernels.hip
@@ -33,36 +33,45 @@
 
 __global__ void __launch_bounds__(1024) ivf_plan(const int *__restrict__ cnt, const int *__restrict__ list_len,
                                                  int nlist, int group, int *__restrict__ bucket_off,
-                                                 int *__restrict__ item_off, int *__restrict__ cursor) {
-    __shared__ int sb[1024], si[1024];
-    __shared__ int carry_b, carry_i;
-    if (threadIdx.x == 0) { carry_b = 0; carry_i = 0; }
+                                                 int *__restrict__ item_off, int *__restrict__ cursor,
+                                                 int *__restrict__ goff) {
+    __shared__ int sb[1024], si[1024], sg[1024];
+    __shared__ int carry_b, carry_i, carry_g;
+    if (threadIdx.x == 0) { carry_b = 0; carry_i = 0; carry_g = 0; }
     __syncthreads();
     for (int base = 0; base < nlist; base += 1024) {
         const int l = base + threadIdx.x;
         const int c = l < nlist ? cnt[l] : 0;
-        const int items = l < nlist ? ivf_ngroups(c, group) * ivf_nch(list_len[l]) : 0;
+        const int groups = l < nlist ? ivf_ngroups(c, group) : 0;
+        const int items = l < nlist ? groups * ivf_nch(list_len[l]) : 0;
         sb[threadIdx.x] = c;
         si[threadIdx.x] = items;
+        sg[threadIdx.x] = groups;
         __syncthreads();
         for (int o = 1; o < 1024; o <<= 1) {
-            int vb = 0, vi = 0;
-            if ((int)threadIdx.x >= o) { vb = sb[threadIdx.x - o]; vi = si[threadIdx.x - o]; }
+            int vb = 0, vi = 0, vg = 0;
+            if ((int)threadIdx.x >= o) { vb = sb[threadIdx.x - o]; vi = si[threadIdx.x - o]; vg = sg[threadIdx.x - o]; }
             __syncthreads();
             sb[threadIdx.x] += vb;
             si[threadIdx.x] += vi;
+            sg[threadIdx.x] += vg;
             __syncthreads();
         }
         if (l < nlist) {
             bucket_off[l] = carry_b + sb[threadIdx.x] - c;
             item_off[l] = carry_i + si[threadIdx.x] - items;
+            if (goff) goff[l] = carry_g + sg[threadIdx.x] - groups;
             cursor[l] = 0;
         }
         __syncthreads();
-        if (threadIdx.x == 1023) { carry_b += sb[1023]; carry_i += si[1023]; }
+        if (threadIdx.x == 1023) { carry_b += sb[1023]; carry_i += si[1023]; carry_g += sg[1023]; }
         __syncthreads();
     }
-    if (threadIdx.x == 0) { bucket_off[nlist] = carry_b; item_off[nlist] = carry_i; }
+    if (threadIdx.x == 0) {
+        bucket_off[nlist] = carry_b;
+        item_off[nlist] = carry_i;
+        if (goff) goff[nlist] = carry_g;
+    }
 }
 
 __global__ void ivf_fill(const int64_t *__restrict__ probes, int64_t npairs, const int *__restrict__ list_len,
@@ -166,11 +175,11 @@
                                                    int *__restrict__ item_off, int *__restrict__ cursor,
                                                    int *__restrict__ qtot, int64_t nq, int64_t npairs,
                                                    int *__restrict__ slot_off, int *__restrict__ nflag_reset,
-                                                   unsigned *__restrict__ qbound) {
-    __shared__ int sb[1024], si[1024];
-    __shared__ int carry_b, carry_i;
+                                                   unsigned *__restrict__ qbound, int *__restrict__ goff) {
+    __shared__ int sb[1024], si[1024], sg[1024];
+    __shared__ int carry_b, carry_i, carry_g;
     const int tid = threadIdx.x;
-    if (tid == 0) { carry_b = 0; carry_i = 0; }
+    if (tid == 0) { carry_b = 0; carry_i = 0; carry_g = 0; }
     if (nflag_reset && tid == 0) *nflag_reset = 0;
     if (qbound)
         for (int64_t q = tid; q < nq; q += 1024) qbound[q] = 0xff800000u;
@@ -180,22 +189,26 @@
         int c = 0;
         if (l < nlist)
             for (int cp = 0; cp < kPlanCopies; ++cp) c += ccnt[(int64_t)cp * nlist + l];
-        const int items = l < nlist ? ivf_ngroups(c, group) * ivf_nch(list_len[l]) : 0;
+        const int groups = l < nlist ? ivf_ngroups(c, group) : 0;
+        const int items = l < nlist ? groups * ivf_nch(list_len[l]) : 0;
         sb[tid] = c;
         si[tid] = items;
+        sg[tid] = groups;
         __syncthreads();
         for (int o = 1; o < 1024; o <<= 1) {
-            int vb = 0, vi = 0;
-            if (tid >= o) { vb = sb[tid - o]; vi = si[tid - o]; }
+            int vb = 0, vi = 0, vg = 0;
+            if (tid >= o) { vb = sb[tid - o]; vi = si[tid - o]; vg = sg[tid - o]; }
             __syncthreads();
             sb[tid] += vb;
             si[tid] += vi;
+            sg[tid] += vg;
             __syncthreads();
         }
         if (l < nlist) {
             cnt[l] = c;
             bucket_off[l] = carry_b + sb[tid] - c;
             item_off[l] = carry_i + si[tid] - items;
+            if (goff) goff[l] = carry_g + sg[tid] - groups;
             int pre = 0;
             for (int cp = 0; cp < kPlanCopies; ++cp) {
                 const int64_t e = (int64_t)cp * nlist + l;
@@ -206,10 +219,14 @@
             }
         }
         __syncthreads();
-        if (tid == 1023) { carry_b += sb[1023]; carry_i += si[1023]; }
+        if (tid == 1023) { carry_b += sb[1023]; carry_i += si[1023]; carry_g += sg[1023]; }
         __syncthreads();
     }
-    if (tid == 0) { bucket_off[nlist] = carry_b; item_off[nlist] = carry_i; }
+    if (tid == 0) {
+        bucket_off[nlist] = carry_b;
+        item_off[nlist] = carry_i;
+        if (goff) goff[nlist] = carry_g;
+    }
     __syncthreads();
     if (tid == 0) carry_b = 0;
     __syncthreads();
@@ -276,24 +293,29 @@
                                                       const int *__restrict__ qtot, int *__restrict__ slot_off,
                                                       int64_t npairs, int *__restrict__ cnt, int *__restrict__ bucket_off,
                                                       int *__restrict__ item_off, int *__restrict__ bucket,
-                                                      int *__restrict__ nflag_reset, unsigned *__restrict__ qbound) {
+                                                      int *__restrict__ nflag_reset, unsigned *__restrict__ qbound,
+                                                      int *__restrict__ goff) {
     __shared__ int s_boff[kPlanFillMaxList];
     __shared__ int s_w[4], s_qb[4];
     const int tid = threadIdx.x, lane = tid & 63, wave = tid >> 6;
     const int64_t q0 = (int64_t)blockIdx.x * 4;
     const int per = (nlist + 255) / 256;
-    int sum = 0, isum = 0;
+    int sum = 0, isum = 0, gsum = 0;
     for (int j = 0; j < per; ++j) {
         const int l = tid * per + j;
         if (l < nlist) {
             int c = 0;
             for (int cp = 0; cp < kPlanCopies; ++cp) c += ccnt[(int64_t)cp * nlist + l];
             sum += c;
-            if (blockIdx.x == 0) isum += ivf_ngroups(c, group) * ivf_nch(list_len[l]);
+            if (blockIdx.x == 0) {
+                isum += ivf_ngroups(c, group) * ivf_nch(list_len[l]);
+                gsum += ivf_ngroups(c, group);
+            }
         }
     }
     int b = block_excl_scan256(sum, s_w);
     int ib = blockIdx.x == 0 ? block_excl_scan256(isum, s_w) : 0;
+    int gb = blockIdx.x == 0 && goff ? block_excl_scan256(gsum, s_w) : 0;
     for (int j = 0; j < per; ++j) {
         const int l = tid * per + j;
         if (l < nlist) {
@@ -305,6 +327,8 @@
                 bucket_off[l] = b;
                 item_off[l] = ib;
                 ib += ivf_ngroups(c, group) * ivf_nch(list_len[l]);
+                if (goff) goff[l] = gb;
+                gb += ivf_ngroups(c, group);
             }
             b += c;
         }
@@ -312,6 +336,7 @@
     if (blockIdx.x == 0 && tid == 255) {
         bucket_off[nlist] = b;
         item_off[nlist] = ib;
+        if (goff) goff[nlist] = gb;
     }
     for (int64_t l = (int64_t)blockIdx.x * 256 + tid; l < (int64_t)kPlanCopies * nlist; l += (int64_t)gridDim.x * 256) {
         ccnt_next[l] = 0;
@@ -1000,7 +1025,7 @@
 void launch_ivf_plan(const int64_t *probes, int64_t nq, int nprobe, const int *list_len, int nlist, int group,
                      int *cnt, int *bucket_off, int *item_off, int *cursor, int *bucket, int *slot_off,
                      hipStream_t st, int *nflag_reset, unsigned *qbound, int *ccnt, int *qtot, bool counted,
-                     int *ccnt_next, int *cursor_next) {
+                     int *ccnt_next, int *cursor_next, int *goff) {
     const int64_t npairs = nq * nprobe;
     if (ivf_plan_query_major() && ccnt && qtot) {
         const unsigned gq = (unsigned)std::max<int64_t>(1, ceil_div(nq, (int64_t)4));
@@ -1011,12 +1036,12 @@
         if (fused_env && ccnt_next && cursor_next && nlist <= kPlanFillMaxList && nq > 0) {
             hipLaunchKernelGGL(ivf_planfill_q, dim3(gq), dim3(256), 0, st, probes, nq, nprobe, list_len, nlist, group,
                                ccnt, ccnt_next, cursor, cursor_next, qtot, slot_off, npairs, cnt, bucket_off, item_off,
-                               bucket, nflag_reset, qbound);
+                               bucket, nflag_reset, qbound, goff);
             HIPANN_CHECK(hipGetLastError());
             return;
         }
         hipLaunchKernelGGL(ivf_plan_q, dim3(1), dim3(1024), 0, st, ccnt, list_len, nlist, group, cnt, bucket_off,
-                           item_off, cursor, qtot, nq, npairs, slot_off, nflag_reset, qbound);
+                           item_off, cursor, qtot, nq, npairs, slot_off, nflag_reset, qbound, goff);
         if (nq > 0)
             hipLaunchKernelGGL(ivf_fill_q, dim3(gq), dim3(256), 0, st, probes, nq, nprobe, list_len, nlist, qtot,
                                bucket_off, cursor, bucket, slot_off);
@@ -1032,7 +1057,7 @@
         hipLaunchKernelGGL(ivf_count, dim3((unsigned)ceil_div(npairs, 256)), dim3(256), 0, st, probes, npairs, list_len,
                            nlist, cnt);
     hipLaunchKernelGGL(ivf_plan, dim3(1), dim3(1024), 0, st, cnt, list_len, nlist, group, bucket_off, item_off,
-                       cursor);
+                       cursor, goff);
     hipLaunchKernelGGL(ivf_slot_scan, dim3(1), dim3(1024), 0, st, probes, npairs, list_len, nlist, slot_off);
     if (npairs > 0)
         hipLaunchKernelGGL(ivf_fill, dim3((unsigned)ceil_div(npairs, 256)), dim3(256), 0, st, probes, npairs, list_len,
@@ -1403,7 +1428,8 @@
                                                    int64_t total, int k, int64_t nrows, float bound,
                                                    float *wk, int *wp, float *sk, int *sp, int *scnt,
                                                    WaveList<1, int> &L, bool &bad, long long &rr_t, int64_t rr_q,
-                                                   float *ntk, int *ntp) {
+                                                   float *ntk, int *ntp, const int *__restrict__ pair_slot = nullptr,
+                                                   int kslot = 0) {
     (void)rr_t;
     (void)rr_q;
     const int lane = threadIdx.x & 63, wv = threadIdx.x >> 6;
@@ -1413,8 +1439,10 @@
 #pragma unroll
     for (int j = 0; j < J; ++j) {
         const int64_t c = ((int64_t)j * WV + wv) * 64 + lane;
-        v[j] = c < total ? pd[c] : __builtin_inff();
-        r[j] = c < total ? pi[c] : -1;
+        bool live = c < total;
+        if (pair_slot && live) live = pair_slot[c / kslot + 1] > pair_slot[c / kslot];
+        v[j] = live ? pd[c] : __builtin_inff();
+        r[j] = live ? pi[c] : -1;
     }
     RR_MARK(1);
     float *mk = wk + wv * 64 * J;
@@ -1782,7 +1810,7 @@
                 const int64_t *__restrict__ list_off, int nlist, const unsigned *__restrict__ qbound,
                 const float *__restrict__ qnorm, int kslot, int sub, const int *__restrict__ list_len,
                 float *__restrict__ fpd, long long *__restrict__ fpi, unsigned long long *__restrict__ fb_total,
-                int fb_cap, int i8_l2) {
+                int fb_cap, int i8_l2, const int *__restrict__ seed_cnt) {
     const int64_t q = WV == 1 ? (int64_t)blockIdx.x * 4 + (threadIdx.x >> 6) : (int64_t)blockIdx.x;
     if (q >= nq) return;
     const int lane = threadIdx.x & 63;
@@ -1793,10 +1821,11 @@
     L.init();
     const int64_t s0 = slot_off ? slot_off[q * nprobe] : q * nprobe;
     const int64_t s1 = slot_off ? slot_off[(q + 1) * nprobe] : (q + 1) * nprobe;
-    const int64_t total = (s1 - s0) * kslot;
+    const int64_t total = seed_cnt ? kSeedK + (int64_t)seed_cnt[q] * kslot : (s1 - s0) * kslot;
+    const int64_t first = seed_cnt ? (ivf_seed_run_slot((int)s0, q) + 1) * kslot - kSeedK : s0 * kslot;
     if constexpr (HIPANN_RR_STAMP != 0) { if (total >= 0) RR_STAMP(1); }
-    pd += s0 * kslot;
-    pi += s0 * kslot;
+    pd += first;
+    pi += first;
     float tsub = __builtin_inff();
     if (sub && qbound) {
         const unsigned b = qbound[q];
@@ -2184,6 +2213,106 @@
     I[(int64_t)idx[j] * kout + e] = If[t];
 }
 
+constexpr int kSeedWaves = 4, kSeedJ = 16;
+__global__ void __launch_bounds__(64 * kSeedWaves)
+ivf_seed_bound(const float *__restrict__ pa_d, const int *__restrict__ pa_i, const int *__restrict__ slot_off, int nprobe,
+               int64_t nq, int kslot, int64_t nrows, unsigned *__restrict__ qbound, float *__restrict__ cd,
+               int *__restrict__ ci, int *__restrict__ cslot, int *__restrict__ bcnt) {
+    const int64_t q = blockIdx.x;
+    if (q >= nq) return;
+    const int lane = threadIdx.x & 63, wv = threadIdx.x >> 6;
+    const int64_t p0 = q * nprobe;
+    const int64_t s0 = ivf_seed_run_slot(slot_off[p0], q);
+    if (wv == 0) {
+        int carry = 0;
+        for (int pb = 0; pb < nprobe; pb += 64) {
+            const int p = pb + lane;
+            const int nch = p < nprobe ? slot_off[p0 + p + 1] - slot_off[p0 + p] : 0;
+            const int nb = ivf_seed_pair_slots(nch);
+            int x = nb;
+#pragma unroll
+            for (int o = 1; o < 64; o <<= 1) {
+                const int t = __shfl_up(x, o);
+                if (lane >= o) x += t;
+            }
+            if (p < nprobe) cslot[p0 + p] = (int)(s0 + 1 + carry + x - nb);
+            carry += __shfl(x, 63);
+        }
+        if (lane == 0) bcnt[q] = carry;
+    }
+    const unsigned b = qbound[q];
+    const float t = __uint_as_float((b & 0x80000000u) ? (b & 0x7fffffffu) : ~b);
+    const float bound = t == t ? t : __builtin_inff();
+    __shared__ float wk[kSeedWaves * 64 * kSeedJ], sk[kSeedWaves * 64], ntk[kSeedWaves * 64];
+    __shared__ int wp[kSeedWaves * 64 * kSeedJ], sp[kSeedWaves * 64], ntp[kSeedWaves * 64];
+    __shared__ int scnt[kSeedWaves];
+    WaveList<1, int> L;
+    L.init();
+    bool bad = false;
+    long long rr_t = 0;
+    rerank_wave_select<kSeedWaves, kSeedJ>(pa_d + p0 * kslot, pa_i + p0 * kslot, (int64_t)nprobe * kslot, kSeedK, nrows,
+                                           bound, wk, wp, sk, sp, scnt, L, bad, rr_t, q, ntk, ntp, slot_off + p0, kslot);
+    if (wv != 0) return;
+    const bool real = L.id[0] != IdTraits<int>::pad();
+    cd[(s0 + 1) * kslot - kSeedK + lane] = real ? L.d[0] : __builtin_inff();
+    ci[(s0 + 1) * kslot - kSeedK + lane] = L.id[0];
+    if (lane == kSeedK - 1 && real) {
+        const unsigned u = __float_as_uint(L.d[0]);
+        atomicMin(qbound + q, (u & 0x80000000u) ? ~u : (u | 0x80000000u));
+    }
+}
+
+extern "C" int hipann_debug_ivf_seed_items(const int *list_len, const int *cnt, int nlist, int group, int *item_off,
+                                           int *goff, int cap, int *a_lcg, int *b_lcg) {
+    int io = 0, go = 0;
+    for (int l = 0; l < nlist; ++l) {
+        item_off[l] = io;
+        goff[l] = go;
+        io += ivf_ngroups(cnt[l], group) * (int)ceil_div(list_len[l], IVF_CH);
+        go += ivf_ngroups(cnt[l], group);
+    }
+    item_off[nlist] = io;
+    goff[nlist] = go;
+    for (int phase = 1; phase <= 2; ++phase) {
+        const int total = ivf_phase_first(phase, io, go);
+        if (total > cap) return -1;
+        int *out = phase == 1 ? a_lcg : b_lcg;
+        for (int item = 0; item < total; ++item) {
+            const int l = ivf_phase_list(phase, item_off, goff, nlist, item);
+            int chunk, grp;
+            ivf_phase_decode(phase, item - ivf_phase_first(phase, item_off[l], goff[l]), ivf_ngroups(cnt[l], group), chunk, grp);
+            out[3 * item] = l;
+            out[3 * item + 1] = chunk;
+            out[3 * item + 2] = grp;
+        }
+    }
+    return 0;
+}
+extern "C" void hipann_debug_ivf_seed_slots(const int *slot_off, int nprobe, int64_t nq, int64_t *cslot, int *bcnt) {
+    for (int64_t q = 0; q < nq; ++q) {
+        int64_t s = ivf_seed_run_slot(slot_off[q * nprobe], q) + 1;
+        for (int p = 0; p < nprobe; ++p) {
+            cslot[q * nprobe + p] = s;
+            s += ivf_seed_pair_slots(slot_off[q * nprobe + p + 1] - slot_off[q * nprobe + p]);
+        }
+        bcnt[q] = (int)(s - ivf_seed_run_slot(slot_off[q * nprobe], q) - 1);
+    }
+}
+
+bool ivf_seed_supported(int nprobe, int kslot) {
+    return nprobe >= 1 && kslot >= kSeedK && (int64_t)nprobe * kslot <= (int64_t)64 * kSeedWaves * kSeedJ;
+}
+
+void launch_ivf_seed_bound(const float *pa_d, const int *pa_i, const int *slot_off, int nprobe, int64_t nq, int kslot,
+                           int64_t nrows, unsigned *qbound, float *cd, int *ci, int *cslot, int *bcnt, hipStream_t st) {
+    if (nq <= 0) return;
+    HIPANN_REQUIRE(ivf_seed_supported(nprobe, kslot) && nq < (int64_t)0x7fffffff, "ivf seed bound: too many chunk-0 entries");
+    static_assert(kSeedK == 64, "the seed list is one wave wide");
+    hipLaunchKernelGGL(ivf_seed_bound, dim3((unsigned)nq), dim3(64 * kSeedWaves), 0, st, pa_d, pa_i, slot_off, nprobe, nq,
+                       kslot, nrows, qbound, cd, ci, cslot, bcnt);
+    HIPANN_CHECK(hipGetLastError());
+}
+
 #ifndef HIPANN_RR_WIDE
 #define HIPANN_RR_WIDE (1 << 30)
 #endif
@@ -2194,9 +2323,10 @@
                        hipStream_t st, float eps, float rxmax, const float *qres, const int64_t *probes,
                        const int64_t *list_off, int nlist, const unsigned *qbound, const float *qnorm, int kslot,
                        int sub, const int *list_len, float *fpd, long long *fpi, unsigned long long *fb_total,
-                       int fb_cap, int i8_l2) {
+                       int fb_cap, int i8_l2, const int *seed_cnt) {
     if (nq <= 0) return;
     if (kslot <= 0) kslot = k;
+    HIPANN_REQUIRE(!seed_cnt || (slot_off && sub && qbound), "ivf rerank: candidate runs need the slot table and the bound");
     HIPANN_REQUIRE(!i8_l2 || (metric == kL2 && qres && qnorm), "ivf rerank: the int8 L2 certificate needs ‖q − q̂‖ and ‖q‖²");
     HIPANN_REQUIRE(k >= kRerankK && k <= 64 && kout >= 1 && kout <= k && kslot >= 1 && (!sub || qbound),
                    "ivf rerank: k / kout out of range");
@@ -2205,7 +2335,7 @@
     dim3 grid((unsigned)(wide ? nq : ceil_div(nq, 4))), block(256);
 #define RR_ARGS pd, pi, slot_off, nprobe, nq, k, kout, Q, codes, d, ids, nrows, label_offset, xmax2, D, I, nflag, flagged, \
                 eps, rxmax, qres, probes, list_off, nlist, qbound, qnorm, kslot, sub, list_len, fpd, fpi, fb_total, \
-                fpd ? fb_cap : 0, i8_l2
+                fpd ? fb_cap : 0, i8_l2, seed_cnt
     if (metric == kIP) {
         if (wide) hipLaunchKernelGGL((ivf_rerank_topk<true, 4>), grid, block, 0, st, RR_ARGS);
         else hipLaunchKernelGGL((ivf_rerank_topk<true, 1>), grid, block, 0, st, RR_ARGS);
diff --git a/duckdb-annsearch_amd/csrc/ivf_mfma.hip b/duckdb-annsearch_amd/csrc/ivf_mfma.hip
--- a/duckdb-annsearch_amd/csrc/ivf_mfma.hip
+++ b/duckdb-annsearch_amd/csrc/ivf_mfma.hip
@@ -172,7 +172,7 @@
                 const int q = qt * 16 + 4 * g + v;
                 if (q < nqi) {
                     const int pr = bucket[boff + q];
-                    const int64_t slot = (int64_t)slot_off[pr] + chunk;
+                    const int64_t slot = (slot_off ? (int64_t)slot_off[pr] : (int64_t)pr) + chunk;
                     const int64_t off = (sub ? slot * MF_WAVES + wave : slot) * k + m;
                     const uint64_t e = lst[qt][v];
                     const unsigned id = (unsigned)e;
@@ -828,7 +828,7 @@
 #define HIPANN_MH_STATS 0
 #endif
 #if HIPANN_MH_STATS
-__device__ unsigned long long mh_stats_dev[2][2][5];
+__device__ unsigned long long mh_stats_dev[2][4][5];
 #endif
 constexpr int MH_P = HIPANN_MH_P;
 __host__ __device__ inline int mh_nsup(int d) { return (int)ceil_div(ceil_div(d, 32), MH_P) * MH_P; }
@@ -1439,22 +1439,18 @@
                 const int *__restrict__ item_off, const int *__restrict__ bucket, const int *__restrict__ slot_off,
                 int nlist, int nprobe, int group, int k, int sub, unsigned *__restrict__ qbound, float *__restrict__ part_d,
                 int *__restrict__ part_i, float *__restrict__ qres, int nq, int remap, const float *__restrict__ xs8,
-                const float *__restrict__ xr8, const float *__restrict__ qhn) {
+                const float *__restrict__ xr8, const float *__restrict__ qhn, int phase, const int *__restrict__ goff) {
     extern __shared__ __attribute__((aligned(16))) float smem[];
-    const int total = item_off[nlist];
+    const int total = ivf_phase_first(phase, item_off[nlist], phase ? goff[nlist] : 0);
     if ((int)blockIdx.x >= total) return;
     const int item = remap ? xcd_remap((int)blockIdx.x, total) : (int)blockIdx.x;
-    int lo = 0, hi = nlist - 1;
-    while (lo < hi) {
-        const int mid = (lo + hi + 1) >> 1;
-        if (item_off[mid] <= item) lo = mid; else hi = mid - 1;
-    }
-    const int l = lo;
+    const int l = ivf_phase_list(phase, item_off, goff, nlist, item);
     const int64_t lr0 = list_off[l], lr1 = lr0 + list_len[l];
     const int c = cnt[l];
     const int ng = ivf_ngroups(c, group);
-    const int rem = item - item_off[l];
-    const int chunk = rem / ng, grp = rem - chunk * ng;
+    int chunk, grp;
+    ivf_phase_decode(phase, item - ivf_phase_first(phase, item_off[l], phase ? goff[l] : 0), ng, chunk, grp);
+    const int slot_chunk = phase == 2 ? chunk - 1 : chunk;
     const int q_begin = (int)((int64_t)grp * c / ng), q_end = (int)((int64_t)(grp + 1) * c / ng);
     const int nqi = q_end - q_begin;
     const int64_t r0 = lr0 + (int64_t)chunk * MF_CH;
@@ -1478,7 +1474,7 @@
     }
 
     const int lane = threadIdx.x & 63, g = lane >> 4;
-    const int stat_part = (int64_t)blockIdx.x * 5 < (int64_t)total ? 0 : 1;
+    const int stat_part = phase ? 1 + phase : (int64_t)blockIdx.x * 5 < (int64_t)total ? 0 : 1;
 #define MH_CASE(QTV)                                                                                        \
     {                                                                                                       \
         unsigned qb[QTV][4];                                                                                \
@@ -1488,7 +1484,7 @@
             qb[qt][v] = q < nqi ? __atomic_load_n(qbound + qi, __ATOMIC_RELAXED) : 0xffffffffu;             \
         }                                                                                                   \
         mh_item<QTV, IP, I8>(d, codes_h, tp0, xn, r0, r1, nqi, qs, stride, qb, qpar, bucket, boff, nprobe, slot_off, \
-                             chunk, k, sub, smem, qbound, part_d, part_i, xs8, xr8, stat_part);             \
+                             slot_chunk, k, sub, smem, qbound, part_d, part_i, xs8, xr8, stat_part);        \
     }
     switch (nqt) {
     case 0: case 1: MH_CASE(1) break;
@@ -1503,12 +1499,13 @@
 
 void ivf_mh_stats_report() {
 #if HIPANN_MH_STATS
-    unsigned long long h[2][2][5];
+    unsigned long long h[2][4][5];
+    static const char *const names[4] = {"first_fifth", "rest", "seeded_chunk0", "seeded_rest"};
     if (hipMemcpyFromSymbol(h, HIP_SYMBOL(mh_stats_dev), sizeof(h)) != hipSuccess) return;
     for (int i8 = 0; i8 < 2; ++i8)
-        for (int part = 0; part < 2; ++part)
+        for (int part = 0; part < 4; ++part)
             std::fprintf(stderr, "HIPANN_MH_STATS image=%s blocks=%s passes=%llu steps=%llu hit_steps=%llu admitted_rows=%llu "
-                                 "insert_steps=%llu\n", i8 ? "int8" : "fp16", part ? "rest" : "first_fifth", h[i8][part][0],
+                                 "insert_steps=%llu\n", i8 ? "int8" : "fp16", names[part], h[i8][part][0],
                          h[i8][part][1], h[i8][part][2], h[i8][part][3], h[i8][part][4]);
     std::memset(h, 0, sizeof(h));
     (void)hipMemcpyToSymbol(HIP_SYMBOL(mh_stats_dev), h, sizeof(h));
@@ -1602,8 +1599,10 @@
                             const int64_t *list_off, const int *list_len, const int *cnt, const int *bucket_off,
                             const int *item_off, const int *bucket, const int *slot_off, int nlist, int nprobe, int k,
                             int64_t max_items, unsigned *qbound, float *pd, int *pi, hipStream_t st, int sub, int i8mode,
-                            const float *xs8, const float *xr8, const float *qhn) {
+                            const float *xs8, const float *xr8, const float *qhn, int phase, const int *goff) {
     if (max_items <= 0 || nq <= 0) return;
+    HIPANN_REQUIRE(phase == 0 ? slot_off != nullptr : goff && (phase == 1) == (slot_off == nullptr),
+                   "fp16 / int8 IVF scan: phase 1 writes pair slots, phase 2 needs the pairs' chunk-1 slots");
     HIPANN_REQUIRE(max_items < (int64_t)0x7fffffff, "too many IVF work items");
     HIPANN_REQUIRE(qsplit && its && qres && codes_h, "fp16 IVF scan: missing buffers");
     HIPANN_REQUIRE(i8mode ? ivf_mfma_i8_supported(d, k) && xs8 : ivf_mfma_h_supported(d, k),
@@ -1621,7 +1620,7 @@
     const uint4 *ch = static_cast<const uint4 *>(codes_h);
     static const int remap = [] { const char *e = std::getenv("HIPANN_IVF_REMAP"); return !e || std::atoi(e) ? 1 : 0; }();
 #define MH_LAUNCH_ARGS qs, qn, its, d, ch, tpass_off, xn, list_off, list_len, cnt, bucket_off, item_off, bucket, slot_off, nlist, nprobe, \
-                       group, k, sub, qbound, pd, pi, qres, (int)nq, remap, xs8, xr8, qhn
+                       group, k, sub, qbound, pd, pi, qres, (int)nq, remap, xs8, xr8, qhn, phase, goff
     if (i8mode) {
         if (metric == kIP) hipLaunchKernelGGL((ivf_scan_mfma_h<true, true>), grid, block, smem, st, MH_LAUNCH_ARGS);
         else hipLaunchKernelGGL((ivf_scan_mfma_h<false, true>), grid, block, smem, st, MH_LAUNCH_ARGS);
diff --git a/duckdb-annsearch_amd/csrc/runtime.hpp b/duckdb-annsearch_amd/csrc/runtime.hpp
--- a/duckdb-annsearch_amd/csrc/runtime.hpp
+++ b/duckdb-annsearch_amd/csrc/runtime.hpp
@@ -328,6 +328,7 @@
     hipStream_t stream = nullptr;
     DevBuf q, qn, coarse_d, coarse_i, cnt, bucket_off, item_off, cursor, bucket, slot_off, part_d, part_i, out_d, out_i;
     DevBuf qbound;
+    DevBuf goff, cslot, bcnt;
     DevBuf qsplit;
     float xmax2 = -1.f;
     DevBuf nflag, flagged, fq, fD, fI, coarse_save, tmpnorm;
@@ -372,6 +373,7 @@
     std::vector<int> owner;
     int form = kFormHalfExact;
     int filter_image = 2, last_filter_image = 0;
+    int last_seeded = 0;
     int64_t rerank_fallbacks = 0;
     std::vector<std::unique_ptr<IvfShard>> shards;
     int64_t last_nq = 0;
@@ -427,7 +429,8 @@
 void launch_ivf_plan(const int64_t *probes, int64_t nq, int nprobe, const int *list_len, int nlist, int group,
                      int *cnt, int *bucket_off, int *item_off, int *cursor, int *bucket, int *slot_off,
                      hipStream_t st, int *nflag_reset = nullptr, unsigned *qbound = nullptr, int *ccnt = nullptr,
-                     int *qtot = nullptr, bool counted = false, int *ccnt_next = nullptr, int *cursor_next = nullptr);
+                     int *qtot = nullptr, bool counted = false, int *ccnt_next = nullptr, int *cursor_next = nullptr,
+                     int *goff = nullptr);
 int64_t ivf_max_items(int64_t nq, int nprobe, int nlist, int max_nch, int64_t nrows, int group);
 int ivf_mfma_bf_group(int d, int np);
 bool ivf_mfma_bf_supported(const float *Q, int d, const float *codes, int k, int np);
@@ -447,7 +450,8 @@
                        const int *list_len = nullptr, float *fpd = nullptr, long long *fpi = nullptr,
                        unsigned long long *fb_total = nullptr,
                        int fb_cap = 0,
-                       int i8_l2 = 0);
+                       int i8_l2 = 0,
+                       const int *seed_cnt = nullptr);
 void launch_ivf_fallback_chunks(const int *nflag, const int *flagged, int fb_cap, int nprobe, int maxch, int chunk_rows,
                                 int kout, int metric, const float *Q, const float *codes, int d, const int64_t *ids,
                                 int64_t label_offset, const int64_t *probes, const int64_t *list_off,
@@ -471,7 +475,11 @@
                             const int *item_off, const int *bucket, const int *slot_off, int nlist, int nprobe, int k,
                             int64_t max_items, unsigned *qbound, float *pd, int *pi, hipStream_t st, int sub = 0,
                             int i8mode = 0, const float *xs8 = nullptr, const float *xr8 = nullptr,
-                            const float *qhn = nullptr);
+                            const float *qhn = nullptr,
+                            int phase = 0, const int *goff = nullptr);
+bool ivf_seed_supported(int nprobe, int kslot);
+void launch_ivf_seed_bound(const float *pa_d, const int *pa_i, const int *slot_off, int nprobe, int64_t nq, int kslot,
+                           int64_t nrows, unsigned *qbound, float *cd, int *ci, int *cslot, int *bcnt, hipStream_t st);
 int ivf_mfma_i8_group(int d);
 int64_t ivf_i8_pass_bytes(int d);
 int64_t ivf_i8_qimg_bytes(int64_t nq, int d);
diff --git a/duckdb-annsearch_amd/hipann.py b/duckdb-annsearch_amd/hipann.py
--- a/duckdb-annsearch_amd/hipann.py
+++ b/duckdb-annsearch_amd/hipann.py
@@ -99,6 +99,7 @@
             "hipann_ivf_set_filter_image": ([vp, i32], i32),
             "hipann_ivf_get_filter_image": ([vp], i32),
             "hipann_ivf_last_filter_image": ([vp], i32),
+            "hipann_ivf_last_seeded": ([vp], i32),
             "hipann_ntotal": ([vp], i64),
             "hipann_dim": ([vp], i32),
             "hipann_metric": ([vp], i32),
@@ -219,10 +220,13 @@
     def set_kernel_timing(self, on: bool) -> None:
         lib().hipann_set_kernel_timing(self._h, 1 if on else 0)
 
-    def last_search_path(self) -> dict:
+    def last_search_path(self, seeded: bool = False) -> dict:
         f, kf, sl = C.c_int(-1), C.c_int(0), C.c_int(0)
         lib().hipann_last_search_path(self._h, C.byref(f), C.byref(kf), C.byref(sl))
-        return {"form": f.value, "filter_k": kf.value, "sublists": sl.value}
+        path = {"form": f.value, "filter_k": kf.value, "sublists": sl.value}
+        if seeded:
+            path["seeded"] = int(lib().hipann_ivf_last_seeded(self._h))
+        return path
 
     def kernel_ms(self, which: int = 0) -> float:
         return float(lib().hipann_last_kernel_ms(self._h, which))
diff --git a/include/hip_ann.h b/include/hip_ann.h
--- a/include/hip_ann.h
+++ b/include/hip_ann.h
@@ -122,6 +122,7 @@
 int hipann_ivf_set_filter_image(void *index, int mode);
 int hipann_ivf_get_filter_image(void *index);
 int hipann_ivf_last_filter_image(void *index);
+int hipann_ivf_last_seeded(void *index);
 int64_t hipann_ivf_i8_passes_tiled(void *index);
 int64_t hipann_ivf_rerank_fallbacks(void *index);
 
```

After: 556,600 queries/s, median of 6. +2.5%, better.
